# socom20/speech-cloner

Measured on AMD Instinct MI355X. Metric: mel frames/sec, higher is better.
Workload: dtype bf16; 1 GPU; full: STFT+mel front-end on batch 32 x 4 s @ 16 kHz (configs[1] input) -> 64 windows of 400 frames -> encoder (enc_14 weights) + decoder (hp/decoder_cfg_d.json sizes, random init), 64 windows per launch, independent steps pipelined over 10 HIP streams; batch=32, samples=64000, windows=64, model_dtype=bfloat16, streams=10, parallelism=utterance-sharded x1, no collective

## Files before the change

### include/vc_hip.h

```cpp
#ifndef VC_HIP_H
#define VC_HIP_H

#include <stddef.h>
#include <stdint.h>

#ifdef __cplusplus
extern "C" {
#endif

#define VC_OK 0
#define VC_ERR_INVALID 1
#define VC_ERR_HIP 2
#define VC_ERR_WORKSPACE 3
#define VC_ERR_UNSUPPORTED 4

#define VC_ABI_VERSION 7

int vc_version(void);
const char* vc_last_error(void);
const char* vc_target_arch(void);

int vc_set_option(const char* name, int value);
int vc_get_option(const char* name, int* value);
int vc_ablate_build(void);

typedef struct vc_frontend_cfg {
    int32_t sample_rate;
    int32_t hop_length;
    int32_t win_length;
    int32_t n_fft;
    int32_t n_mels;
    int32_t n_mfcc;
    float pre_emphasis;
    float mean_abs_amp_norm;
    float mfcc_norm_factor;
    float M_dB_norm_factor;
    float P_dB_norm_factor;
    int32_t mfcc_normaleze_first_mfcc;
    int32_t calc_mfcc_derivate;
    int32_t clip_output;
} vc_frontend_cfg;

typedef struct vc_frontend_plan vc_frontend_plan;

int vc_frontend_host_tables(const vc_frontend_cfg* cfg, double* h_mel, double* h_dct);

int vc_frontend_plan_create(const vc_frontend_cfg* cfg, const double* h_window,
                            vc_frontend_plan** out_plan);
void vc_frontend_plan_destroy(vc_frontend_plan* plan);

int32_t vc_frontend_num_frames(const vc_frontend_plan* plan, int32_t n_samples);
int32_t vc_frontend_mfcc_width(const vc_frontend_plan* plan);
int32_t vc_frontend_power_width(const vc_frontend_plan* plan);
int vc_frontend_get_mel(const vc_frontend_plan* plan, double* h_out);
int vc_frontend_get_dct(const vc_frontend_plan* plan, double* h_out);

size_t vc_frontend_workspace_bytes(const vc_frontend_plan* plan, int32_t batch, int32_t max_samples);

int vc_frontend_f32(const vc_frontend_plan* plan, const float* d_wav, const int32_t* d_lens,
                    int32_t batch, int32_t max_samples, int32_t wav_stride, int32_t out_rows,
                    float* d_mfcc, float* d_mel_db, float* d_pow_db,
                    void* d_workspace, size_t workspace_bytes, void* stream);

int vc_frontend_stages_f32(const vc_frontend_plan* plan, const float* d_wav, const int32_t* d_lens,
                           int32_t batch, int32_t max_samples, int32_t wav_stride, int32_t out_rows,
                           float* d_mfcc, float* d_mel_db, float* d_pow_db,
                           void* d_workspace, size_t workspace_bytes, void* stream,
                           int32_t stage_mask);

#define VC_F32 0
#define VC_BF16 1
#define VC_ACT_NONE 0
#define VC_ACT_RELU 1
#define VC_ACT_SIGMOID 2
#define VC_ACT_TANH 3
#define VC_GEMM_PLAIN 0
#define VC_GEMM_HIGHWAY 1
#define VC_GEMM_MAX_GROUPS 32

typedef struct vc_gemm_group {
    const void* d_Bt;
    int32_t K;
    int32_t taps;
    int32_t pad_l;
    int32_t c_off;
} vc_gemm_group;

typedef struct vc_gemm_desc {
    int32_t dtype;
    int32_t mode;
    const void* d_X;
    int32_t M, T, Cin, ldx;
    int32_t N;
    int32_t n_groups;
    vc_gemm_group groups[VC_GEMM_MAX_GROUPS];
    const float* d_pro_scale;
    const float* d_pro_shift;
    int32_t pro_relu, pro_pool;
    const float* d_epi_scale;
    const float* d_epi_shift;
    int32_t act;
    const void* d_R;
    int32_t ldr;
    void* d_C;
    int32_t ldc;
    int32_t out_f32;
    float drop_keep;
    unsigned long long drop_seed;
    int32_t sum_groups;
    int32_t epi_pool;
    void* d_workspace;
    size_t workspace_bytes;
} vc_gemm_desc;

int vc_conv_gemm(const vc_gemm_desc* desc, void* stream);
size_t vc_conv_gemm_workspace_bytes(const vc_gemm_desc* desc);
int vc_conv_gemm_epi_pool_supported(const vc_gemm_desc* desc);

int vc_lstm_bidir(const float* d_xproj, const void* d_Wh_fw, const void* d_Wh_bw, int32_t w_dtype, int32_t n_seq, int32_t T,
                  int32_t H, void* d_out, int32_t out_dtype, void* stream);

int vc_softmax_argmax(const float* d_logits, int32_t M, int32_t N, int32_t ldl,
                      void* d_prob, int32_t ldp, int32_t out_dtype, int32_t* d_class, void* stream);
int vc_softmax_argmax_dual(const float* d_logits, int32_t M, int32_t N, int32_t ldl, float* d_prob, int32_t ldp,
                           void* d_prob_bf16, int32_t ldp_bf16, int32_t* d_class, void* stream);

size_t vc_gru_workspace_bytes(int32_t H, int32_t w_dtype);
int vc_gru_bidir(const float* d_xproj, const void* d_Wh_fw, const void* d_Wh_bw, int32_t w_dtype,
                 int32_t n_seq, int32_t T, int32_t H, void* d_out, int32_t out_dtype,
                 void* d_workspace, size_t workspace_bytes, void* stream);


typedef struct vc_wgrad_group {
    const void* d_dYT;
    void* d_dW;
    int32_t N, taps, shift0;
    int32_t ldw;
} vc_wgrad_group;
typedef struct vc_wgrad_desc {
    const void* d_XT;
    int32_t ldxt, ldyt, Cin, M, T, margin, n_groups;
    int32_t splits_allowed;
    vc_wgrad_group groups[VC_GEMM_MAX_GROUPS];
} vc_wgrad_desc;
int vc_conv_wgrad(const vc_wgrad_desc* desc, void* stream);

int vc_transpose_pad(const float* d_X, int32_t M, int32_t C, int32_t ld, int32_t T, const float* d_scale,
                     const float* d_shift, int32_t relu, int32_t pool, int32_t row_shift, float* d_XT,
                     int32_t ldt, int32_t pad, int32_t slack_row, void* stream);

int vc_split16(const float* d_X, int32_t M, int32_t C, int32_t ldx, int32_t T, const float* d_scale, const float* d_shift,
               int32_t relu, int32_t pool, void* d_out16, float* d_row_scale, void* stream);
typedef struct vc_w16_item {
    const float* src;
    void* dst;
    float* scale_dst;
    int32_t k, cin, cout, mode;
    int32_t row_len, tap_stride, plane_stride, base;
    int32_t group, scale_n;
} vc_w16_item;
int vc_weights16(const vc_w16_item* d_items, int32_t n_items, uint32_t* d_gmax, int32_t n_groups, void* stream);
typedef struct vc_gemm16_pair {
    const void* d_Bt0;
    const void* d_Bt1;
    int32_t taps0, extra, pad_l, c_off0, c_off1;
    int32_t row0;
    int32_t nrows0, nrows1;
    int32_t s_off0, s_off1;
} vc_gemm16_pair;
typedef struct vc_gemm16_desc {
    const void* d_X16;
    const float* d_row_scale;
    int32_t M, T, C, ldx;
    int32_t n_pairs, ragged;
    vc_gemm16_pair pairs[16];
    const float* d_col_scale;
    const float* d_col_shift;
    float* d_C;
    int32_t ldc;
    int32_t accumulate;
    int32_t act;
    int32_t atomic_splits;
    void* d_workspace;
    size_t workspace_bytes;
} vc_gemm16_desc;
size_t vc_gemm16_workspace_bytes(int32_t M, int32_t C, int32_t n_pairs);
int vc_transpose_split16(const float* d_X, int32_t M, int32_t C, int32_t ldx, int32_t T, const float* d_scale,
                         const float* d_shift, int32_t relu, int32_t pool, int32_t shift0, int32_t n_shifts, void* d_out16,
                         float* d_row_scale, void* stream);
int vc_gemm16(const vc_gemm16_desc* desc, void* stream);

int vc_mx8_quantize(const void* d_X, int32_t x_dtype, int32_t M, int32_t C, int32_t ldx, void* d_Q, void* d_S, void* stream);
#define VC_MX8_MAX_GROUPS 32
#define VC_MX8_OUT_MX 0
#define VC_MX8_OUT_BF16 1
#define VC_MX8_OUT_F32 2
typedef struct vc_mx8_group {
    const void* d_W;
    const void* d_Ws;
    int32_t taps, pad_l, c_off, reserved;
} vc_mx8_group;
typedef struct vc_mx8_conv_desc {
    const void* d_X;
    const void* d_Xs;
    int32_t M, T, Cin, n_groups;
    vc_mx8_group groups[VC_MX8_MAX_GROUPS];
    const float* d_epi_scale;
    const float* d_epi_shift;
    int32_t act, pool, out_mode, n_out;
    void* d_C;
    void* d_Cs;
    void* d_workspace;
    size_t workspace_bytes;
} vc_mx8_conv_desc;
size_t vc_mx8_conv_workspace_bytes(const vc_mx8_conv_desc* desc);
int vc_mx8_conv(const vc_mx8_conv_desc* desc, void* stream);

size_t vc_stats_workspace_floats(int32_t M, int32_t C);
int vc_bn_train_stats(const float* d_X, int32_t M, int32_t C, int32_t ld, const float* d_gamma,
                      const float* d_beta, float* d_moving_mean, float* d_moving_var, float decay, float eps,
                      float* d_scale, float* d_shift, float* d_mean, float* d_rstd, float* d_workspace,
                      void* stream);
int vc_affine_act(const float* d_X, const float* d_scale, const float* d_shift, int32_t relu, const float* d_R,
                  float* d_out, size_t n, int32_t C, void* stream);
int vc_bn_backward(const float* d_G, const float* d_X, int32_t M, int32_t C, int32_t ld, int32_t T,
                   const float* d_gamma, const float* d_scale, const float* d_shift, const float* d_mean,
                   const float* d_rstd, int32_t mode, float* d_dX, float* d_dgamma, float* d_dbeta,
                   float* d_workspace, void* stream);
int vc_bn_post_routing(const float* d_X, int32_t M, int32_t C, int32_t ld, int32_t T, const float* d_scale,
                       const float* d_shift, uint8_t* d_bits, void* stream);
int vc_relu_dropout_backward(const float* d_dY, const float* d_Y, float inv_keep, float* d_dZ, size_t n, void* stream);
int vc_highway_backward(const float* d_pre, int32_t NP, const float* d_X, const float* d_dO, int32_t M, int32_t H,
                        float* d_dpre, float* d_dXd, void* stream);
int vc_col_sum(const float* d_X, int32_t M, int32_t C, int32_t ld, float* d_out, int32_t accumulate,
               float* d_workspace, void* stream);
int vc_fill(float* d_p, float value, size_t n, void* stream);
typedef struct vc_layout_item {
    const float* src;
    float* dst;
    int32_t k, cin, cout, mode;
} vc_layout_item;
int vc_weight_layouts(const vc_layout_item* d_items, int32_t n_items, void* stream);
int vc_axpby(const float* d_X, int32_t ldx, float a, const float* d_Y, int32_t ldy, float b, float* d_out, int32_t ldo,
             int32_t M, int32_t C, void* stream);
int vc_mse_loss(const float* d_y, const float* d_t, size_t n, float weight, float* d_dY, int32_t C, int32_t ld_dy,
                float* d_loss, float* d_workspace, void* stream);
int vc_lstm_train_forward(const float* d_xproj, const float* d_Wh_fw, const float* d_Wh_bw, int32_t n_seq, int32_t T,
                          int32_t H, float* d_out, float* d_gates, float* d_cstate, void* stream);
int vc_lstm_backward(const float* d_dout, const float* d_gates, const float* d_cstate, const float* d_WhT_fw,
                     const float* d_WhT_bw, int32_t n_seq, int32_t T, int32_t H, float* d_dpre, void* stream);
int vc_softmax_ce(const float* d_logits, const float* d_target, int32_t M, int32_t C, int32_t ldl, float* d_dlogits,
                  int32_t ldd, float* d_out3, float* d_workspace, void* stream);
int vc_adam_step(float* d_param, const float* d_grad, float* d_m, float* d_v, size_t n, float lr_t, float beta1,
                 float beta2, float epsilon, float grad_scale, void* stream);
int vc_gru_train_forward(const float* d_xproj, const float* d_Wh_fw, const float* d_Wh_bw, int32_t n_seq,
                         int32_t T, int32_t H, float* d_out, float* d_gates, float* d_rh, void* stream);
int vc_gru_backward(const float* d_dout, const float* d_out, const float* d_gates, const float* d_Wh_fw,
                    const float* d_Wh_bw, const float* d_WhT_fw, const float* d_WhT_bw, int32_t n_seq,
                    int32_t T, int32_t H, float* d_dpre, void* stream);

typedef struct vc_vocoder_plan vc_vocoder_plan;

int vc_vocoder_plan_create(int32_t win_length, int32_t hop_length, int32_t n_fft, const double* h_window,
                           vc_vocoder_plan** out_plan);
void vc_vocoder_plan_destroy(vc_vocoder_plan* plan);
int32_t vc_vocoder_num_samples(const vc_vocoder_plan* plan, int32_t n_frames);
size_t vc_vocoder_workspace_bytes(const vc_vocoder_plan* plan, int32_t batch, int32_t max_frames, int32_t trace);

int vc_power_to_amp(const float* d_P, const int32_t* d_n_frames, int32_t batch, int32_t max_frames, int32_t n_bins,
                    float P_dB_norm_factor, float realse, float* d_amp, void* stream);

int vc_griffin_lim_f32(const vc_vocoder_plan* plan, const float* d_amp, const float* d_phase0,
                       const int32_t* d_n_frames, int32_t batch, int32_t max_frames, int32_t num_iters,
                       float* d_wav, int32_t wav_stride, float* d_trace, void* d_workspace, size_t workspace_bytes,
                       void* stream);

size_t vc_vocoder_workspace_bytes_momentum(const vc_vocoder_plan* plan, int32_t batch, int32_t max_frames,
                                           int32_t trace);
int vc_griffin_lim_momentum_f32(const vc_vocoder_plan* plan, const float* d_amp, const float* d_phase0,
                                const int32_t* d_n_frames, int32_t batch, int32_t max_frames, int32_t num_iters,
                                float momentum, float* d_wav, int32_t wav_stride, float* d_trace, void* d_workspace,
                                size_t workspace_bytes, void* stream);

int vc_inv_preemphasis_normalize(const vc_vocoder_plan* plan, float* d_wav, const int32_t* d_n_frames, int32_t batch,
                                 int32_t max_frames, int32_t wav_stride, float coeff, float mean_abs_amp_norm,
                                 void* stream);

int vc_highway_pack(const void* d_Bt, int32_t n_cols, int32_t H, void* d_packed, void* stream);
int vc_highway_chain(const void* d_X, int32_t M, int32_t H, int32_t ldx, int32_t n_layers,
                     const void* const* d_packed, const float* const* d_bias, void* d_Y, int32_t ldy,
                     const void* d_proj_packed, const float* d_proj_bias, int32_t n_proj, float* d_P, int32_t ldp,
                     void* stream);

#define VC_CBHG_FRONT_MAX_HIGHWAY 4
typedef struct vc_cbhg_front_desc {
    const void* d_x;
    int32_t x_f32, ldx;
    int32_t n_windows, T;
    int32_t n_features, prenet_units, width, n_banks, bank_filters, n_highway, gru_units;
    const void *d_pk_dense1, *d_pk_dense2, *d_pk_bank, *d_pk_proj1, *d_pk_proj2, *d_pk_gru;
    const void* d_pk_highway[VC_CBHG_FRONT_MAX_HIGHWAY];
    const float* d_coef;
    float* d_xproj;
    int32_t ldp;
} vc_cbhg_front_desc;
int vc_mfma_pack(const void* d_W, int32_t rows, int32_t K, int32_t ldw, int32_t chained, void* d_packed, void* stream);
int32_t vc_cbhg_front_coef_floats(void);
int vc_cbhg_front_supported(int32_t n_features, int32_t prenet_units, int32_t width, int32_t n_banks,
                            int32_t bank_filters, int32_t n_highway, int32_t gru_units, int32_t T);
int vc_cbhg_front(const vc_cbhg_front_desc* desc, void* stream);

int vc_prenet_chain_supported(int32_t cin_padded, int32_t units1, int32_t units2);
int vc_prenet_chain(const void* d_X, int32_t x_f32, int32_t M, int32_t ldx, int32_t cin_padded, int32_t units1, int32_t units2,
                    const void* d_pk1, const float* d_b1, const void* d_pk2, const float* d_b2, void* d_Y, int32_t ldy,
                    void* stream);

int vc_gather_rows(const void* d_src, const int64_t* d_index, const void* d_pad_row, int64_t n_rows,
                   int32_t row_bytes, void* d_dst, void* stream);

int vc_convert(const void* d_src, int32_t src_dtype, void* d_dst, int32_t dst_dtype, size_t n, void* stream);

int vc_cut_windows(const float* d_src, const int32_t* d_win_tab, const int32_t* d_n_frames, int32_t batch,
                   int32_t max_frames, int32_t n_windows, int32_t T, int32_t C, float* d_dst, void* stream);

int vc_compound_stitch(const void* d_src, int32_t src_dtype, const int32_t* d_utt_tab, int32_t batch, int32_t n_windows,
                       int32_t T, int32_t C, int32_t out_frames, float* d_dst, float* d_amp, float P_dB_norm_factor,
                       void* stream);

int vc_phase_init(const int32_t* d_n_frames, const int32_t* d_utt_id, int32_t batch, int32_t max_frames, int32_t n_bins,
                  int64_t seed, float* d_phase, void* stream);

typedef struct vc_resample_plan vc_resample_plan;
int vc_resample_plan_create(int32_t up, int32_t down, int32_t half, const double* h_taps, vc_resample_plan** out_plan);
void vc_resample_plan_destroy(vc_resample_plan* plan);
int vc_resample_f32(const vc_resample_plan* plan, const float* d_in, const int32_t* d_lens_in, int32_t batch, int32_t max_in,
                    int32_t ld_in, float* d_out, int32_t max_out, int32_t ld_out, void* stream);

int vc_mel_cepstra(const void* d_mel, int32_t mel_dtype, int32_t rows, int32_t n_mels, const float* d_dct, int32_t n_coef,
                   float* d_cep, void* stream);
size_t vc_dtw_workspace_size(int32_t batch, int32_t max_a, int32_t max_b, int32_t want_path);
int vc_dtw_f32(const float* d_ca, const float* d_cb, const int32_t* d_len_a, const int32_t* d_len_b, int32_t batch,
               int32_t max_a, int32_t max_b, int32_t n_coef, float scale, int32_t band, int32_t want_path, float* d_total,
               int32_t* d_path_len, float* d_mcd, void* d_workspace, size_t workspace_bytes, void* stream);
int vc_dtw_backtrack(const void* d_workspace, size_t workspace_bytes, const int32_t* d_len_a, const int32_t* d_len_b,
                     const float* d_total, const int32_t* d_path_len, int32_t batch, int32_t max_a, int32_t max_b, int32_t* d_path,
                     void* stream);
int vc_frame_mcd_f32(const float* d_ca, const float* d_cb, const int32_t* d_len_a, const int32_t* d_len_b, int32_t batch,
                     int32_t max_a, int32_t max_b, int32_t n_coef, float scale, float* d_mcd, void* stream);

int vc_f0_yin_f32(const float* d_wav, const int32_t* d_lens, int32_t batch, int32_t max_len, int32_t ld, float sample_rate,
                  int32_t hop, int32_t frame_length, int32_t tau_min, int32_t tau_max, float threshold, float* d_f0,
                  float* d_aperiodicity, int32_t max_frames, void* stream);
int vc_f0_metrics_f32(const float* d_f0_a, const float* d_f0_b, const int32_t* d_len_a, const int32_t* d_len_b, int32_t batch,
                      int32_t max_a, int32_t max_b, const int32_t* d_path, const int32_t* d_path_len, int32_t max_path,
                      int32_t* d_counts, float* d_values, void* stream);

int vc_frame_energy_tile(int32_t hop, int32_t frame_length);
int vc_frame_energy_f32(const float* d_wav, const int32_t* d_lens, int32_t batch, int32_t max_len, int32_t ld, int32_t hop,
                        int32_t frame_length, float* d_energy, int32_t max_frames, void* stream);
int vc_activity_mask(const float* d_energy, const float* d_f0, const int32_t* d_n_frames, int32_t batch, int32_t max_frames,
                     int32_t mode, float ratio, int32_t max_gap, int32_t min_run, uint8_t* d_mask, void* stream);
int vc_mask_compact(const uint8_t* d_mask_a, const int32_t* d_frames_a, int32_t max_a, const uint8_t* d_mask_b,
                    const int32_t* d_frames_b, int32_t max_b, int32_t batch, int32_t* d_index, int32_t* d_n_active, int32_t* d_n_kept,
                    int32_t* d_intervals, int32_t* d_n_intervals, void* stream);
int vc_compact_rows_f32(const float* d_src, int32_t src_frames, const int32_t* d_index, int32_t index_frames, const int32_t* d_n_kept,
                        int32_t batch, int32_t n_cols, float* d_dst, int32_t dst_frames, void* stream);
int vc_path_map(const int32_t* d_path_in, const int32_t* d_path_len, int32_t batch, int32_t max_path, const int32_t* d_index_a,
                int32_t max_a, const int32_t* d_index_b, int32_t max_b, int32_t* d_path_out, void* stream);
int vc_speech_gain_f32(const float* d_wav, const int32_t* d_lens, int32_t batch, int32_t max_len, int32_t ld, int32_t hop,
                       const uint8_t* d_mask, const int32_t* d_n_active, int32_t max_frames, float target, float* d_gain,
                       void* stream);
int vc_scale_rows_f32(const float* d_wav, const int32_t* d_lens, int32_t batch, int32_t max_len, int32_t ld, const float* d_gain,
                      float* d_out, void* stream);

#ifdef __cplusplus
}
#endif
#endif
```

### speech-cloner_amd/_vc.py

```python
import contextlib
import ctypes as C
import os
import threading


_HERE = os.path.dirname(os.path.abspath(__file__))
LIB_PATH = os.environ.get('VC_LIB_PATH', os.path.join(_HERE, 'libvc_hip.so'))

VC_OK = 0
VC_ABI_VERSION = 7


class VCError(RuntimeError):
    pass


class FrontendCfg(C.Structure):
    _fields_ = [('sample_rate', C.c_int32), ('hop_length', C.c_int32), ('win_length', C.c_int32),
                ('n_fft', C.c_int32), ('n_mels', C.c_int32), ('n_mfcc', C.c_int32),
                ('pre_emphasis', C.c_float), ('mean_abs_amp_norm', C.c_float),
                ('mfcc_norm_factor', C.c_float), ('M_dB_norm_factor', C.c_float),
                ('P_dB_norm_factor', C.c_float),
                ('mfcc_normaleze_first_mfcc', C.c_int32), ('calc_mfcc_derivate', C.c_int32),
                ('clip_output', C.c_int32)]


VC_F32, VC_BF16 = 0, 1
ACT_NONE, ACT_RELU, ACT_SIGMOID, ACT_TANH = 0, 1, 2, 3
GEMM_PLAIN, GEMM_HIGHWAY = 0, 1
GEMM_MAX_GROUPS = 32


class GemmGroup(C.Structure):
    _fields_ = [('d_Bt', C.c_void_p), ('K', C.c_int32), ('taps', C.c_int32), ('pad_l', C.c_int32),
                ('c_off', C.c_int32)]


class GemmDesc(C.Structure):
    _fields_ = [('dtype', C.c_int32), ('mode', C.c_int32), ('d_X', C.c_void_p),
                ('M', C.c_int32), ('T', C.c_int32), ('Cin', C.c_int32), ('ldx', C.c_int32),
                ('N', C.c_int32), ('n_groups', C.c_int32),
                ('groups', GemmGroup * GEMM_MAX_GROUPS),
                ('d_pro_scale', C.c_void_p), ('d_pro_shift', C.c_void_p),
                ('pro_relu', C.c_int32), ('pro_pool', C.c_int32),
                ('d_epi_scale', C.c_void_p), ('d_epi_shift', C.c_void_p), ('act', C.c_int32),
                ('d_R', C.c_void_p), ('ldr', C.c_int32), ('d_C', C.c_void_p), ('ldc', C.c_int32),
                ('out_f32', C.c_int32), ('drop_keep', C.c_float), ('drop_seed', C.c_ulonglong),
                ('sum_groups', C.c_int32), ('epi_pool', C.c_int32),
                ('d_workspace', C.c_void_p), ('workspace_bytes', C.c_size_t)]


CBHG_FRONT_MAX_HIGHWAY = 4


class CbhgFrontDesc(C.Structure):
    _fields_ = [('d_x', C.c_void_p), ('x_f32', C.c_int32), ('ldx', C.c_int32), ('n_windows', C.c_int32), ('T', C.c_int32),
                ('n_features', C.c_int32), ('prenet_units', C.c_int32), ('width', C.c_int32), ('n_banks', C.c_int32),
                ('bank_filters', C.c_int32), ('n_highway', C.c_int32), ('gru_units', C.c_int32),
                ('d_pk_dense1', C.c_void_p), ('d_pk_dense2', C.c_void_p), ('d_pk_bank', C.c_void_p),
                ('d_pk_proj1', C.c_void_p), ('d_pk_proj2', C.c_void_p), ('d_pk_gru', C.c_void_p),
                ('d_pk_highway', C.c_void_p * CBHG_FRONT_MAX_HIGHWAY),
                ('d_coef', C.c_void_p),
                ('d_xproj', C.c_void_p), ('ldp', C.c_int32)]


class LayoutItem(C.Structure):
    _fields_ = [('src', C.c_void_p), ('dst', C.c_void_p), ('k', C.c_int32), ('cin', C.c_int32), ('cout', C.c_int32),
                ('mode', C.c_int32)]


class W16Item(C.Structure):
    _fields_ = [('src', C.c_void_p), ('dst', C.c_void_p), ('scale_dst', C.c_void_p), ('k', C.c_int32), ('cin', C.c_int32),
                ('cout', C.c_int32), ('mode', C.c_int32), ('row_len', C.c_int32), ('tap_stride', C.c_int32),
                ('plane_stride', C.c_int32), ('base', C.c_int32), ('group', C.c_int32), ('scale_n', C.c_int32)]


class Gemm16Pair(C.Structure):
    _fields_ = [('d_Bt0', C.c_void_p), ('d_Bt1', C.c_void_p), ('taps0', C.c_int32), ('extra', C.c_int32),
                ('pad_l', C.c_int32), ('c_off0', C.c_int32), ('c_off1', C.c_int32), ('row0', C.c_int32),
                ('nrows0', C.c_int32), ('nrows1', C.c_int32), ('s_off0', C.c_int32), ('s_off1', C.c_int32)]


class Gemm16Desc(C.Structure):
    _fields_ = [('d_X16', C.c_void_p), ('d_row_scale', C.c_void_p), ('M', C.c_int32), ('T', C.c_int32), ('C', C.c_int32),
                ('ldx', C.c_int32), ('n_pairs', C.c_int32), ('ragged', C.c_int32), ('pairs', Gemm16Pair * 16),
                ('d_col_scale', C.c_void_p), ('d_col_shift', C.c_void_p), ('d_C', C.c_void_p), ('ldc', C.c_int32),
                ('accumulate', C.c_int32), ('act', C.c_int32), ('atomic_splits', C.c_int32), ('d_workspace', C.c_void_p),
                ('workspace_bytes', C.c_size_t)]


MX8_MAX_GROUPS = 32
MX8_OUT_MX, MX8_OUT_BF16, MX8_OUT_F32 = 0, 1, 2


class Mx8Group(C.Structure):
    _fields_ = [('d_W', C.c_void_p), ('d_Ws', C.c_void_p), ('taps', C.c_int32), ('pad_l', C.c_int32),
                ('c_off', C.c_int32), ('reserved', C.c_int32)]


class Mx8ConvDesc(C.Structure):
    _fields_ = [('d_X', C.c_void_p), ('d_Xs', C.c_void_p), ('M', C.c_int32), ('T', C.c_int32), ('Cin', C.c_int32),
                ('n_groups', C.c_int32), ('groups', Mx8Group * MX8_MAX_GROUPS), ('d_epi_scale', C.c_void_p),
                ('d_epi_shift', C.c_void_p), ('act', C.c_int32), ('pool', C.c_int32), ('out_mode', C.c_int32),
                ('n_out', C.c_int32), ('d_C', C.c_void_p), ('d_Cs', C.c_void_p), ('d_workspace', C.c_void_p),
                ('workspace_bytes', C.c_size_t)]


class WgradGroup(C.Structure):
    _fields_ = [('d_dYT', C.c_void_p), ('d_dW', C.c_void_p), ('N', C.c_int32), ('taps', C.c_int32),
                ('shift0', C.c_int32), ('ldw', C.c_int32)]


class WgradDesc(C.Structure):
    _fields_ = [('d_XT', C.c_void_p), ('ldxt', C.c_int32), ('ldyt', C.c_int32), ('Cin', C.c_int32),
                ('M', C.c_int32), ('T', C.c_int32), ('margin', C.c_int32), ('n_groups', C.c_int32),
                ('splits_allowed', C.c_int32), ('groups', WgradGroup * GEMM_MAX_GROUPS)]


_lib = None
_lock = threading.Lock()

_P = C.c_void_p
_SIGS = {
    'vc_version': (C.c_int, []),
    'vc_last_error': (C.c_char_p, []),
    'vc_target_arch': (C.c_char_p, []),
    'vc_set_option': (C.c_int, [C.c_char_p, C.c_int]),
    'vc_get_option': (C.c_int, [C.c_char_p, C.POINTER(C.c_int)]),
    'vc_ablate_build': (C.c_int, []),
    'vc_frontend_host_tables': (C.c_int, [C.POINTER(FrontendCfg), _P, _P]),
    'vc_frontend_plan_create': (C.c_int, [C.POINTER(FrontendCfg), _P, C.POINTER(_P)]),
    'vc_frontend_plan_destroy': (None, [_P]),
    'vc_frontend_num_frames': (C.c_int32, [_P, C.c_int32]),
    'vc_frontend_mfcc_width': (C.c_int32, [_P]),
    'vc_frontend_power_width': (C.c_int32, [_P]),
    'vc_frontend_get_mel': (C.c_int, [_P, _P]),
    'vc_frontend_get_dct': (C.c_int, [_P, _P]),
    'vc_frontend_workspace_bytes': (C.c_size_t, [_P, C.c_int32, C.c_int32]),
    'vc_frontend_f32': (C.c_int, [_P, _P, _P, C.c_int32, C.c_int32, C.c_int32, C.c_int32, _P, _P, _P, _P,
                                  C.c_size_t, _P]),
    'vc_frontend_stages_f32': (C.c_int, [_P, _P, _P, C.c_int32, C.c_int32, C.c_int32, C.c_int32, _P, _P, _P, _P,
                                         C.c_size_t, _P, C.c_int32]),
    'vc_conv_gemm_workspace_bytes': (C.c_size_t, [C.POINTER(GemmDesc)]),
    'vc_conv_gemm': (C.c_int, [C.POINTER(GemmDesc), _P]),
    'vc_softmax_argmax': (C.c_int, [_P, C.c_int32, C.c_int32, C.c_int32, _P, C.c_int32, C.c_int32, _P, _P]),
    'vc_softmax_argmax_dual': (C.c_int, [_P, C.c_int32, C.c_int32, C.c_int32, _P, C.c_int32, _P, C.c_int32, _P, _P]),
    'vc_gru_workspace_bytes': (C.c_size_t, [C.c_int32, C.c_int32]),
    'vc_gru_bidir': (C.c_int, [_P, _P, _P, C.c_int32, C.c_int32, C.c_int32, C.c_int32, _P, C.c_int32, _P,
                               C.c_size_t, _P]),
    'vc_lstm_bidir': (C.c_int, [_P, _P, _P, C.c_int32, C.c_int32, C.c_int32, C.c_int32, _P, C.c_int32, _P]),
    'vc_convert': (C.c_int, [_P, C.c_int32, _P, C.c_int32, C.c_size_t, _P]),
    'vc_conv_wgrad': (C.c_int, [C.POINTER(WgradDesc), _P]),
    'vc_transpose_pad': (C.c_int, [_P, C.c_int32, C.c_int32, C.c_int32, C.c_int32, _P, _P, C.c_int32, C.c_int32,
                                   C.c_int32, _P, C.c_int32, C.c_int32, C.c_int32, _P]),
    'vc_stats_workspace_floats': (C.c_size_t, [C.c_int32, C.c_int32]),
    'vc_bn_train_stats': (C.c_int, [_P, C.c_int32, C.c_int32, C.c_int32, _P, _P, _P, _P, C.c_float, C.c_float,
                                    _P, _P, _P, _P, _P, _P]),
    'vc_affine_act': (C.c_int, [_P, _P, _P, C.c_int32, _P, _P, C.c_size_t, C.c_int32, _P]),
    'vc_bn_backward': (C.c_int, [_P, _P, C.c_int32, C.c_int32, C.c_int32, C.c_int32, _P, _P, _P, _P, _P,
                                 C.c_int32, _P, _P, _P, _P, _P]),
    'vc_lstm_train_forward': (C.c_int, [_P, _P, _P, C.c_int32, C.c_int32, C.c_int32, _P, _P, _P, _P]),
    'vc_lstm_backward': (C.c_int, [_P, _P, _P, _P, _P, C.c_int32, C.c_int32, C.c_int32, _P, _P]),
    'vc_bn_post_routing': (C.c_int, [_P, C.c_int32, C.c_int32, C.c_int32, C.c_int32, _P, _P, _P, _P]),
    'vc_relu_dropout_backward': (C.c_int, [_P, _P, C.c_float, _P, C.c_size_t, _P]),
    'vc_highway_backward': (C.c_int, [_P, C.c_int32, _P, _P, C.c_int32, C.c_int32, _P, _P, _P]),
    'vc_col_sum': (C.c_int, [_P, C.c_int32, C.c_int32, C.c_int32, _P, C.c_int32, _P, _P]),
    'vc_fill': (C.c_int, [_P, C.c_float, C.c_size_t, _P]),
    'vc_weight_layouts': (C.c_int, [_P, C.c_int32, _P]),
    'vc_split16': (C.c_int, [_P, C.c_int32, C.c_int32, C.c_int32, C.c_int32, _P, _P, C.c_int32, C.c_int32, _P, _P, _P]),
    'vc_weights16': (C.c_int, [_P, C.c_int32, _P, C.c_int32, _P]),
    'vc_transpose_split16': (C.c_int, [_P, C.c_int32, C.c_int32, C.c_int32, C.c_int32, _P, _P, C.c_int32, C.c_int32, C.c_int32,
                                       C.c_int32, _P, _P, _P]),
    'vc_gemm16_workspace_bytes': (C.c_size_t, [C.c_int32, C.c_int32, C.c_int32]),
    'vc_gemm16': (C.c_int, [C.POINTER(Gemm16Desc), _P]),
    'vc_mx8_quantize': (C.c_int, [_P, C.c_int32, C.c_int32, C.c_int32, C.c_int32, _P, _P, _P]),
    'vc_mx8_conv_workspace_bytes': (C.c_size_t, [C.POINTER(Mx8ConvDesc)]),
    'vc_mx8_conv': (C.c_int, [C.POINTER(Mx8ConvDesc), _P]),
    'vc_axpby': (C.c_int, [_P, C.c_int32, C.c_float, _P, C.c_int32, C.c_float, _P, C.c_int32, C.c_int32, C.c_int32, _P]),
    'vc_mse_loss': (C.c_int, [_P, _P, C.c_size_t, C.c_float, _P, C.c_int32, C.c_int32, _P, _P, _P]),
    'vc_softmax_ce': (C.c_int, [_P, _P, C.c_int32, C.c_int32, C.c_int32, _P, C.c_int32, _P, _P, _P]),
    'vc_adam_step': (C.c_int, [_P, _P, _P, _P, C.c_size_t, C.c_float, C.c_float, C.c_float, C.c_float,
                               C.c_float, _P]),
    'vc_gru_train_forward': (C.c_int, [_P, _P, _P, C.c_int32, C.c_int32, C.c_int32, _P, _P, _P, _P]),
    'vc_gru_backward': (C.c_int, [_P, _P, _P, _P, _P, _P, _P, C.c_int32, C.c_int32, C.c_int32, _P, _P]),
    'vc_conv_gemm_epi_pool_supported': (C.c_int, [C.POINTER(GemmDesc)]),
    'vc_highway_pack': (C.c_int, [_P, C.c_int32, C.c_int32, _P, _P]),
    'vc_highway_chain': (C.c_int, [_P, C.c_int32, C.c_int32, C.c_int32, C.c_int32, C.POINTER(_P), C.POINTER(_P), _P, C.c_int32,
                                   _P, _P, C.c_int32, _P, C.c_int32, _P]),
    'vc_mfma_pack': (C.c_int, [_P, C.c_int32, C.c_int32, C.c_int32, C.c_int32, _P, _P]),
    'vc_prenet_chain_supported': (C.c_int, [C.c_int32] * 3),
    'vc_prenet_chain': (C.c_int, [_P, C.c_int32, C.c_int32, C.c_int32, C.c_int32, C.c_int32, C.c_int32, _P, _P, _P, _P, _P, C.c_int32, _P]),
    'vc_cbhg_front_coef_floats': (C.c_int32, []),
    'vc_cbhg_front_supported': (C.c_int, [C.c_int32] * 8),
    'vc_cbhg_front': (C.c_int, [C.POINTER(CbhgFrontDesc), _P]),
    'vc_gather_rows': (C.c_int, [_P, _P, _P, C.c_int64, C.c_int32, _P, _P]),
    'vc_vocoder_plan_create': (C.c_int, [C.c_int32, C.c_int32, C.c_int32, _P, C.POINTER(_P)]),
    'vc_vocoder_plan_destroy': (None, [_P]),
    'vc_vocoder_num_samples': (C.c_int32, [_P, C.c_int32]),
    'vc_vocoder_workspace_bytes': (C.c_size_t, [_P, C.c_int32, C.c_int32, C.c_int32]),
    'vc_power_to_amp': (C.c_int, [_P, _P, C.c_int32, C.c_int32, C.c_int32, C.c_float, C.c_float, _P, _P]),
    'vc_griffin_lim_f32': (C.c_int, [_P, _P, _P, _P, C.c_int32, C.c_int32, C.c_int32, _P, C.c_int32, _P, _P,
                                     C.c_size_t, _P]),
    'vc_vocoder_workspace_bytes_momentum': (C.c_size_t, [_P, C.c_int32, C.c_int32, C.c_int32]),
    'vc_griffin_lim_momentum_f32': (C.c_int, [_P, _P, _P, _P, C.c_int32, C.c_int32, C.c_int32, C.c_float, _P, C.c_int32,
                                              _P, _P, C.c_size_t, _P]),
    'vc_inv_preemphasis_normalize': (C.c_int, [_P, _P, _P, C.c_int32, C.c_int32, C.c_int32, C.c_float, C.c_float, _P]),
    'vc_cut_windows': (C.c_int, [_P, _P, _P, C.c_int32, C.c_int32, C.c_int32, C.c_int32, C.c_int32, _P, _P]),
    'vc_compound_stitch': (C.c_int, [_P, C.c_int32, _P, C.c_int32, C.c_int32, C.c_int32, C.c_int32, C.c_int32, _P, _P,
                                     C.c_float, _P]),
    'vc_phase_init': (C.c_int, [_P, _P, C.c_int32, C.c_int32, C.c_int32, C.c_int64, _P, _P]),
    'vc_resample_plan_create': (C.c_int, [C.c_int32, C.c_int32, C.c_int32, _P, C.POINTER(_P)]),
    'vc_resample_plan_destroy': (None, [_P]),
    'vc_resample_f32': (C.c_int, [_P, _P, _P, C.c_int32, C.c_int32, C.c_int32, _P, C.c_int32, C.c_int32, _P]),
    'vc_mel_cepstra': (C.c_int, [_P, C.c_int32, C.c_int32, C.c_int32, _P, C.c_int32, _P, _P]),
    'vc_dtw_workspace_size': (C.c_size_t, [C.c_int32] * 4),
    'vc_dtw_f32': (C.c_int, [_P, _P, _P, _P, C.c_int32, C.c_int32, C.c_int32, C.c_int32, C.c_float, C.c_int32, C.c_int32, _P, _P, _P,
                             _P, C.c_size_t, _P]),
    'vc_dtw_backtrack': (C.c_int, [_P, C.c_size_t, _P, _P, _P, _P, C.c_int32, C.c_int32, C.c_int32, _P, _P]),
    'vc_frame_mcd_f32': (C.c_int, [_P, _P, _P, _P, C.c_int32, C.c_int32, C.c_int32, C.c_int32, C.c_float, _P, _P]),
    'vc_frame_energy_tile': (C.c_int, [C.c_int32, C.c_int32]),
    'vc_frame_energy_f32': (C.c_int, [_P, _P, C.c_int32, C.c_int32, C.c_int32, C.c_int32, C.c_int32, _P, C.c_int32, _P]),
    'vc_activity_mask': (C.c_int, [_P, _P, _P, C.c_int32, C.c_int32, C.c_int32, C.c_float, C.c_int32, C.c_int32, _P, _P]),
    'vc_mask_compact': (C.c_int, [_P, _P, C.c_int32, _P, _P, C.c_int32, C.c_int32, _P, _P, _P, _P, _P, _P]),
    'vc_compact_rows_f32': (C.c_int, [_P, C.c_int32, _P, C.c_int32, _P, C.c_int32, C.c_int32, _P, C.c_int32, _P]),
    'vc_path_map': (C.c_int, [_P, _P, C.c_int32, C.c_int32, _P, C.c_int32, _P, C.c_int32, _P, _P]),
    'vc_speech_gain_f32': (C.c_int, [_P, _P, C.c_int32, C.c_int32, C.c_int32, C.c_int32, _P, _P, C.c_int32, C.c_float, _P, _P]),
    'vc_scale_rows_f32': (C.c_int, [_P, _P, C.c_int32, C.c_int32, C.c_int32, _P, _P, _P]),
    'vc_f0_yin_f32': (C.c_int, [_P, _P, C.c_int32, C.c_int32, C.c_int32, C.c_float, C.c_int32, C.c_int32, C.c_int32, C.c_int32,
                                C.c_float, _P, _P, C.c_int32, _P]),
    'vc_f0_metrics_f32': (C.c_int, [_P, _P, _P, _P, C.c_int32, C.c_int32, C.c_int32, _P, _P, C.c_int32, _P, _P, _P]),
}


def lib():
    global _lib
    if _lib is not None:
        return _lib
    with _lock:
        if _lib is not None:
            return _lib
        if not os.path.exists(LIB_PATH):
            raise VCError('native library %s not found -- run `python -c "import __graft_entry__ as g; '
                          'g.build()"` (or make -C speech-cloner_amd/csrc); there is no CPU fallback'
                          % LIB_PATH)
        import torch
        h = C.CDLL(LIB_PATH)
        h.vc_version.restype, h.vc_version.argtypes = C.c_int, []
        got = h.vc_version()
        if got != VC_ABI_VERSION:
            raise VCError('native library %s reports ABI version %d, this binding is written for %d -- rebuild it '
                          '(make -C speech-cloner_amd/csrc)' % (LIB_PATH, got, VC_ABI_VERSION))
        for name, (res, args) in _SIGS.items():
            try:
                fn = getattr(h, name)
            except AttributeError:
                raise VCError('native library %s does not export %s -- it was built from older sources, rebuild it '
                              '(make -C speech-cloner_amd/csrc)' % (LIB_PATH, name)) from None
            fn.restype = res
            fn.argtypes = args
        _lib = h
    return _lib


def set_option(name, value):
    check(lib().vc_set_option(name.encode(), int(value)))


def get_option(name):
    v = C.c_int(0)
    check(lib().vc_get_option(name.encode(), C.byref(v)))
    return v.value


@contextlib.contextmanager
def options(**kw):
    old = {k: get_option(k) for k in kw}
    try:
        for k, v in kw.items():
            set_option(k, v)
        yield
    finally:
        for k, v in old.items():
            set_option(k, v)


THROUGHPUT_OPTIONS = {'proj256_split': 0, 'fe_fused': 0}


def throughput_mode():
    return options(**THROUGHPUT_OPTIONS)


def check(rc):
    if rc != VC_OK:
        msg = lib().vc_last_error()
        raise VCError('libvc_hip error %d: %s' % (rc, msg.decode('utf-8', 'replace') if msg else '?'))


def ptr(t):
    if t is None:
        return None
    if hasattr(t, 'data_ptr'):
        return C.c_void_p(t.data_ptr())
    return C.c_void_p(t.ctypes.data)


def current_stream():
    import torch
    return C.c_void_p(torch.cuda.current_stream().cuda_stream)
```

### speech-cloner_amd/csrc/vc_api.hip

```cpp
#include <cstdarg>
#include <atomic>
#include <cstdio>
#include <cstring>
#include "vc_common.h"

namespace vc {

static thread_local char g_err[512] = "";

char* last_error_buf() { return g_err; }

int set_error(int code, const char* fmt, ...) {
    va_list ap;
    va_start(ap, fmt);
    vsnprintf(g_err, sizeof(g_err), fmt, ap);
    va_end(ap);
    return code;
}

static std::atomic<int> g_opt[OPT_COUNT];
static const struct { const char* name; Option id; bool ablate; } k_opts[] = {
    {"bank256", OPT_BANK256, false}, {"bank256_xcd", OPT_BANK256_XCD, false}, {"conv256", OPT_CONV256, false},
    {"conv256_min_k", OPT_CONV256_MINK, false}, {"conv256_wm", OPT_CONV256_WM, false}, {"proj256", OPT_PROJ256, false}, {"proj256_split", OPT_PROJ256_SPLIT, false},
    {"wgrad_xcd", OPT_WGRAD_XCD, false}, {"gru_mfma", OPT_GRU_MFMA, false}, {"gru_mfma4", OPT_GRU_MFMA4, false}, {"gru_small_mfma", OPT_GRU_SMALL_MFMA, false}, {"fe_fused", OPT_FE_FUSED, false}, {"fe_fused_spin", OPT_FE_FUSED_SPIN, false}, {"gru_train_resident", OPT_GRU_TRAIN_RESIDENT, false}, {"prenet_lds", OPT_PRENET_LDS, false}, {"cbhg_front_mi", OPT_CBHG_FRONT_MI, false}, {"gemm16_split", OPT_GEMM16_SPLIT, false}, {"f32_f16x3", OPT_F32_F16X3, false}, {"gru_f32_wide", OPT_GRU_F32_WIDE, false},
    {"ablate_bank256", OPT_ABLATE_BANK256, true}, {"ablate_bank256_only", OPT_ABLATE_BANK256_ONLY, true},
    {"ablate_cbhg_front", OPT_ABLATE_CBHG_FRONT, true},
};
static struct OptInit { OptInit() { for (auto& o : g_opt) o.store(-1); } } g_opt_init;

int opt(Option o) { return g_opt[o].load(std::memory_order_relaxed); }

static __global__ void zero_words_kernel(unsigned* __restrict__ p, size_t n) {
    for (size_t i = (size_t)blockIdx.x * blockDim.x + threadIdx.x; i < n; i += (size_t)gridDim.x * blockDim.x) p[i] = 0u;
}

hipError_t zero_async(void* d_p, size_t bytes, hipStream_t st) {
    if (bytes % 4) return hipErrorInvalidValue;
    const size_t n = bytes / 4;
    if (n == 0) return hipSuccess;
    const size_t blocks = (n + 255) / 256;
    hipLaunchKernelGGL(zero_words_kernel, dim3((unsigned)(blocks < 1024 ? blocks : 1024)), dim3(256), 0, st,
                       static_cast<unsigned*>(d_p), n);
    return hipGetLastError();
}

}

extern "C" {

int vc_set_option(const char* name, int value) {
    VC_REQUIRE(name, "vc_set_option: NULL name");
    for (const auto& o : vc::k_opts)
        if (!std::strcmp(o.name, name)) {
#ifndef VC_ABLATE
            VC_REQUIRE(!o.ablate, "vc_set_option: %s exists only in -DVC_ABLATE builds (tools/build_ablate.sh)", name);
#endif
            vc::g_opt[o.id].store(value);
            return VC_OK;
        }
    return vc::set_error(VC_ERR_INVALID, "vc_set_option: unknown option %s", name);
}

int vc_get_option(const char* name, int* value) {
    VC_REQUIRE(name && value, "vc_get_option: NULL argument");
    for (const auto& o : vc::k_opts)
        if (!std::strcmp(o.name, name)) { *value = vc::g_opt[o.id].load(); return VC_OK; }
    return vc::set_error(VC_ERR_INVALID, "vc_get_option: unknown option %s", name);
}

int vc_ablate_build(void) {
#ifdef VC_ABLATE
    return 1;
#else
    return 0;
#endif
}

int vc_version(void) { return VC_ABI_VERSION; }
const char* vc_last_error(void) { return vc::last_error_buf(); }
const char* vc_target_arch(void) { return "gfx950"; }

}
```

### speech-cloner_amd/csrc/vc_common.h

```cpp
#pragma once
#include <hip/hip_runtime.h>
#include <cstdarg>
#include <cstdio>
#include "vc_hip.h"

namespace vc {

char* last_error_buf();
int set_error(int code, const char* fmt, ...);

#define VC_HIP_CHECK(expr)                                                                   \
    do {                                                                                     \
        hipError_t _e = (expr);                                                              \
        if (_e != hipSuccess)                                                                \
            return vc::set_error(VC_ERR_HIP, "%s failed: %s (%s:%d)", #expr,                 \
                                 hipGetErrorString(_e), __FILE__, __LINE__);                 \
    } while (0)

#define VC_REQUIRE(cond, ...)                                                                \
    do {                                                                                     \
        if (!(cond)) return vc::set_error(VC_ERR_INVALID, __VA_ARGS__);                      \
    } while (0)

constexpr int WAVE = 64;

enum Option {
    OPT_BANK256 = 0,
    OPT_BANK256_XCD,
    OPT_CONV256,
    OPT_CONV256_MINK,
    OPT_CONV256_WM,
    OPT_PROJ256,
    OPT_PROJ256_SPLIT,
    OPT_WGRAD_XCD,
    OPT_GRU_MFMA,
    OPT_FE_FUSED,
    OPT_FE_FUSED_SPIN,
    OPT_GRU_SMALL_MFMA,
    OPT_GRU_MFMA4,
    OPT_PRENET_LDS,
    OPT_GRU_TRAIN_RESIDENT,
    OPT_CBHG_FRONT_MI,
    OPT_GRU_F32_WIDE,
    OPT_F32_F16X3,
    OPT_GEMM16_SPLIT,
    OPT_ABLATE_BANK256,
    OPT_ABLATE_BANK256_ONLY,
    OPT_ABLATE_CBHG_FRONT,
    OPT_COUNT
};
int opt(Option o);

hipError_t zero_async(void* d_p, size_t bytes, hipStream_t st);

#if defined(__HIPCC__)
template <int CTRL, int ROW_MASK>
__device__ __forceinline__ float dpp_move(float identity, float v) {
    return __int_as_float(__builtin_amdgcn_update_dpp(__float_as_int(identity), __float_as_int(v), CTRL, ROW_MASK, 0xF, false));
}
#define VC_WAVE_REDUCE(OP, ID)                                                                  \
    v = OP(v, dpp_move<0xB1, 0xF>(ID, v));                             \
    v = OP(v, dpp_move<0x4E, 0xF>(ID, v));                             \
    v = OP(v, dpp_move<0x141, 0xF>(ID, v));                                \
    v = OP(v, dpp_move<0x140, 0xF>(ID, v));          \
    v = OP(v, dpp_move<0x142, 0xA>(ID, v));                 \
    v = OP(v, dpp_move<0x143, 0xC>(ID, v));                 \
    return __int_as_float(__builtin_amdgcn_readlane(__float_as_int(v), 63));
__device__ __forceinline__ float vc_addf(float a, float b) { return a + b; }
__device__ __forceinline__ float wave_sum(float v) { VC_WAVE_REDUCE(vc_addf, 0.0f) }
__device__ __forceinline__ float wave_max(float v) { VC_WAVE_REDUCE(fmaxf, -3.402823466e38f) }
__device__ __forceinline__ float highway_gate(float hpre, float tpre, float x) {
    const float hv = fmaxf(hpre, 0.0f);
    const float e = __builtin_amdgcn_exp2f(tpre * -1.4426950408889634f);
    const float tv = __builtin_amdgcn_rcpf(1.0f + e);
    return fmaf(tv, hv - x, x);
}
__device__ __forceinline__ float wave_min(float v) { VC_WAVE_REDUCE(fminf, 3.402823466e38f) }
#undef VC_WAVE_REDUCE
#endif

}
```

### speech-cloner_amd/csrc/vc_conv256.h

```cpp
#pragma once
#include <hip/hip_runtime.h>
#include <cstdint>

struct Conv256Args {
    const void* X;
    int32_t M, T, Cin, ldx, N;
    const void* Bt;
    int32_t K, taps, pad_l, c_off;
    int32_t pool;
    const float* epi_scale;
    const float* epi_shift;
    int32_t act;
    const void* R;
    int32_t ldr;
    void* C;
    int32_t ldc;
};

int vc_launch_conv256(const Conv256Args& a, hipStream_t st);
```

### speech-cloner_amd/csrc/vc_conv256.hip

```cpp
#include "vc_common.h"
#include "vc_conv256.h"
#include <cstdlib>

namespace {

typedef float f32x16 __attribute__((ext_vector_type(16)));
typedef __bf16 bf16x8 __attribute__((ext_vector_type(8)));
typedef __bf16 bf16x4 __attribute__((ext_vector_type(4)));
typedef unsigned short u16x8 __attribute__((ext_vector_type(8)));

constexpr int a_rows(int wm) { return 64 * wm + 8; }

__device__ __forceinline__ void glds16(const void* g, void* l) {
    __builtin_amdgcn_global_load_lds((const __attribute__((address_space(1))) void*)(uintptr_t)g,
                                     (__attribute__((address_space(3))) void*)(uintptr_t)(uint32_t)(uintptr_t)l, 16, 0, 0);
}

__device__ __forceinline__ bf16x8 max_nonneg(bf16x8 x, bf16x8 y) {
    return __builtin_bit_cast(bf16x8, __builtin_elementwise_max(__builtin_bit_cast(u16x8, x), __builtin_bit_cast(u16x8, y)));
}

__device__ __forceinline__ float act_fn(float v, int act) {
    switch (act) {
        case VC_ACT_RELU: return fmaxf(v, 0.0f);
        case VC_ACT_SIGMOID: return 1.0f / (1.0f + __expf(-v));
        case VC_ACT_TANH: return tanhf(v);
        default: return v;
    }
}

__device__ __forceinline__ void wait_loads_but(int n) {
    if (n >= 8) asm volatile("s_waitcnt vmcnt(8) lgkmcnt(0)" ::: "memory");
    else if (n >= 6) asm volatile("s_waitcnt vmcnt(6) lgkmcnt(0)" ::: "memory");
    else if (n >= 4) asm volatile("s_waitcnt vmcnt(4) lgkmcnt(0)" ::: "memory");
    else if (n >= 2) asm volatile("s_waitcnt vmcnt(2) lgkmcnt(0)" ::: "memory");
    else asm volatile("s_waitcnt vmcnt(0) lgkmcnt(0)" ::: "memory");
}

template <int WN, bool POOL, int NBUF, int WM>
__global__ void __launch_bounds__(64 * WM * WN, 1)
conv256_kernel(Conv256Args a) {
    constexpr int BM = 64 * WM, A_ROWS = a_rows(WM), A_BYTES = A_ROWS * 128;
    constexpr int BN = 64 * WN, NWAVE = WM * WN, NTHR = 64 * NWAVE;
    constexpr int BQ = (BN / 8) / NWAVE;
    static_assert(BQ * NWAVE * 8 == BN && (BQ == 2 || BQ == 4), "weight tile split");
    constexpr int DIST = NBUF - 1;
    constexpr int B_BYTES = BN * 128;
    constexpr int AQ = (A_ROWS / 8 + NWAVE - 1) / NWAVE;
    extern __shared__ __attribute__((aligned(16))) char smem[];
    char* const As = smem;
    char* const Bs = smem + 2 * A_BYTES;

    const int tid = threadIdx.x, lane = tid & 63;
    const int wid = __builtin_amdgcn_readfirstlane(tid >> 6);
    const int wr = wid / WN, wc = wid % WN;
    const int m0 = blockIdx.x * BM, n0 = blockIdx.y * BN;
    const int ntap = a.taps, nslab = a.Cin >> 6, ntiles = nslab * ntap, pad_l = a.pad_l;
    const __bf16* X = reinterpret_cast<const __bf16*>(a.X);
    const __bf16* Bt = reinterpret_cast<const __bf16*>(a.Bt);

    const int srow = lane >> 3, pslot = lane & 7;
    const __bf16* a_src[AQ];
#pragma unroll
    for (int q = 0; q < AQ; ++q) {
        const int rho = (q * NWAVE + wid) * 8 + srow;
        const int g = min(max(m0 - pad_l + rho, 0), a.M - 1);
        a_src[q] = X + (size_t)g * a.ldx + (pslot ^ ((rho >> 1) & 7)) * 8;
    }
    const int a_rows_needed = BM + ntap - 1 + (POOL ? 1 : 0);
    const __bf16* b_src[BQ];
#pragma unroll
    for (int q = 0; q < BQ; ++q) {
        const int n = (q * NWAVE + wid) * 8 + srow;
        b_src[q] = Bt + (size_t)min(n0 + n, a.N - 1) * a.K + (pslot ^ ((n >> 1) & 7)) * 8;
    }
    auto stageA = [&](int cs, int buf) {
        char* dst = As + buf * A_BYTES + wid * 1024;
#pragma unroll
        for (int q = 0; q < AQ; ++q) {
            const int rb = q * NWAVE + wid;
            if (rb * 8 < a_rows_needed && rb < A_ROWS / 8) glds16(a_src[q] + cs * 64, dst + q * NWAVE * 1024);
        }
    };
    auto stageB = [&](int n, int buf) {
        const int cs = n / ntap, j = n - cs * ntap;
        const int koff = j * a.Cin + cs * 64;
        char* dst = Bs + buf * B_BYTES + wid * 1024;
#pragma unroll
        for (int q = 0; q < BQ; ++q) glds16(b_src[q] + koff, dst + q * NWAVE * 1024);
    };

    const int li = lane & 31, lh = lane >> 5;
    const int a_row0 = wr * 64 + li;
    const int xb = (li >> 1) & 7;
    int b_off[4];
#pragma unroll
    for (int s = 0; s < 4; ++s) b_off[s] = (wc * 64 + li) * 128 + (((2 * s + lh) ^ xb) << 4);
    int jlo[2], jhi[2];
#pragma unroll
    for (int i = 0; i < 2; ++i) {
        const int m = min(m0 + wr * 64 + i * 32 + li, a.M - 1);
        const int t = m % a.T;
        jlo[i] = max(0, pad_l - t);
        jhi[i] = a.T - t + pad_l;
    }
    int J_lo = max(jlo[0], jlo[1]);
    int J_hi = min(jhi[0], jhi[1]) - (POOL ? 1 : 0);
#pragma unroll
    for (int o = 32; o > 0; o >>= 1) {
        J_lo = max(J_lo, __shfl_xor(J_lo, o, 64));
        J_hi = min(J_hi, __shfl_xor(J_hi, o, 64));
    }
    J_lo = __builtin_amdgcn_readfirstlane(J_lo);
    J_hi = __builtin_amdgcn_readfirstlane(J_hi);

    f32x16 acc[2][2];
#pragma unroll
    for (int i = 0; i < 2; ++i)
#pragma unroll
        for (int c = 0; c < 2; ++c)
#pragma unroll
            for (int r = 0; r < 16; ++r) acc[i][c][r] = 0.0f;

    bf16x8 fa[2][2], fp[2][2], fb[2][2];
    int a_base = 0, a_o[4], p_base = 0, p_o[4];
    int j = 0;
    auto tap_setup = [&](int n) {
        const int cs = n / ntap, jj = n - cs * ntap;
        const int rho = a_row0 + jj;
        a_base = (cs & 1) * A_BYTES + rho * 128;
        p_base = a_base + 128;
        const int x = (rho >> 1) & 7, xp = ((rho + 1) >> 1) & 7;
#pragma unroll
        for (int s = 0; s < 4; ++s) {
            a_o[s] = ((2 * s + lh) ^ x) << 4;
            p_o[s] = ((2 * s + lh) ^ xp) << 4;
        }
        return jj;
    };

    const int keep = ntap == 1 ? DIST - 2 : DIST - 1;
    const int tail0 = ntap == 1 ? ntiles - DIST : ntiles - 2;
    static_assert(DIST == 2 || DIST == 3, "the taps >= DIST - 1 argument above assumes 3 or 4 weight buffers");
    stageA(0, 0);
    stageB(0, 0);
#pragma unroll
    for (int d = 1; d < DIST; ++d)
        if (d < ntiles) stageB(d, d);
    wait_loads_but(BQ * min(DIST - 1, ntiles - 1));
    __builtin_amdgcn_s_barrier();
    asm volatile("" ::: "memory");
    if (nslab > 1) stageA(1, 1);
    if (DIST < ntiles) stageB(DIST, DIST);
    int bcur = 0;
    j = tap_setup(0);
    {
        const char* ap = As + a_base + a_o[0];
        fa[0][0] = *reinterpret_cast<const bf16x8*>(ap);
        fa[0][1] = *reinterpret_cast<const bf16x8*>(ap + 4096);
        if constexpr (POOL) {
            const char* pp = As + p_base + p_o[0];
            fp[0][0] = *reinterpret_cast<const bf16x8*>(pp);
            fp[0][1] = *reinterpret_cast<const bf16x8*>(pp + 4096);
        }
        const char* bp = Bs + b_off[0];
        fb[0][0] = *reinterpret_cast<const bf16x8*>(bp);
        fb[0][1] = *reinterpret_cast<const bf16x8*>(bp + 4096);
    }

    for (int n = 0; n < ntiles; ++n) {
        const bool need_mask = !(j >= J_lo && j < J_hi);
        bool v[2], hn[2];
#pragma unroll
        for (int i = 0; i < 2; ++i) {
            v[i] = j >= jlo[i] && j < jhi[i];
            hn[i] = j < jhi[i] - 1;
        }
        const bf16x8 zero = {};
        int jn = j;
#pragma unroll
        for (int s = 0; s < 4; ++s) {
            const int cur = s & 1, nxt = cur ^ 1;
            bool have_next = true;
            int nb = bcur;
            if (s == 3) {
                wait_loads_but(BQ * max(0, min(keep, tail0 - n)));
                __builtin_amdgcn_s_barrier();
                asm volatile("" ::: "memory");
                have_next = n + 1 < ntiles;
                if (have_next) {
                    const int cs1 = (n + 1) / ntap;
                    if ((n + 1) - cs1 * ntap == 0 && cs1 + 1 < nslab) stageA(cs1 + 1, (cs1 + 1) & 1);
                    jn = tap_setup(n + 1);
                }
                if (n + 1 + DIST < ntiles) stageB(n + 1 + DIST, bcur);
                nb = bcur + 1 == NBUF ? 0 : bcur + 1;
            }
            const int sn = (s + 1) & 3;
            const char* ap = As + a_base + a_o[sn];
            const char* pp = As + p_base + p_o[sn];
            const char* bp = Bs + nb * B_BYTES + b_off[sn];
            bf16x8 av[2];
#pragma unroll
            for (int i = 0; i < 2; ++i) {
                if constexpr (POOL) av[i] = max_nonneg(fa[cur][i], fp[cur][i]);
                else av[i] = fa[cur][i];
            }
            if (need_mask) {
#pragma unroll
                for (int i = 0; i < 2; ++i) {
                    if constexpr (POOL) av[i] = hn[i] ? av[i] : fa[cur][i];
                    av[i] = v[i] ? av[i] : zero;
                }
            }
            __builtin_amdgcn_s_setprio(1);
            acc[0][0] = __builtin_amdgcn_mfma_f32_32x32x16_bf16(fb[cur][0], av[0], acc[0][0], 0, 0, 0);
            acc[0][1] = __builtin_amdgcn_mfma_f32_32x32x16_bf16(fb[cur][1], av[0], acc[0][1], 0, 0, 0);
            if (have_next) {
                fa[nxt][0] = *reinterpret_cast<const bf16x8*>(ap);
                fa[nxt][1] = *reinterpret_cast<const bf16x8*>(ap + 4096);
                if constexpr (POOL) {
                    fp[nxt][0] = *reinterpret_cast<const bf16x8*>(pp);
                    fp[nxt][1] = *reinterpret_cast<const bf16x8*>(pp + 4096);
                }
                fb[nxt][0] = *reinterpret_cast<const bf16x8*>(bp);
                fb[nxt][1] = *reinterpret_cast<const bf16x8*>(bp + 4096);
            }
            acc[1][0] = __builtin_amdgcn_mfma_f32_32x32x16_bf16(fb[cur][0], av[1], acc[1][0], 0, 0, 0);
            acc[1][1] = __builtin_amdgcn_mfma_f32_32x32x16_bf16(fb[cur][1], av[1], acc[1][1], 0, 0, 0);
            __builtin_amdgcn_s_setprio(0);
        }
        j = jn;
        bcur = bcur + 1 == NBUF ? 0 : bcur + 1;
    }

    constexpr int EP = BN * 2 + 16;
    __syncthreads();
    {
#pragma unroll
        for (int c = 0; c < 2; ++c) {
#pragma unroll
            for (int q = 0; q < 4; ++q) {
                const int col = wc * 64 + c * 32 + 8 * q + 4 * lh;
                const int gn = min(n0 + col, a.N - 4);
                float4 sv = make_float4(1.0f, 1.0f, 1.0f, 1.0f), bv = make_float4(0.0f, 0.0f, 0.0f, 0.0f);
                if (a.epi_scale) sv = *reinterpret_cast<const float4*>(a.epi_scale + a.c_off + gn);
                if (a.epi_shift) bv = *reinterpret_cast<const float4*>(a.epi_shift + a.c_off + gn);
                const float svv[4] = {sv.x, sv.y, sv.z, sv.w}, bvv[4] = {bv.x, bv.y, bv.z, bv.w};
#pragma unroll
                for (int i = 0; i < 2; ++i) {
                    const int row = wr * 64 + i * 32 + li;
                    bf16x4 rr = {};
                    if (a.R) {
                        const int gm = min(m0 + row, a.M - 1);
                        rr = *reinterpret_cast<const bf16x4*>(reinterpret_cast<const __bf16*>(a.R) + (size_t)gm * a.ldr + gn);
                    }
                    bf16x4 o;
#pragma unroll
                    for (int e = 0; e < 4; ++e) {
                        float val = act_fn(acc[i][c][4 * q + e] * svv[e] + bvv[e], a.act);
                        if (a.R) val += (float)rr[e];
                        o[e] = (__bf16)val;
                    }
                    *reinterpret_cast<bf16x4*>(smem + row * EP + col * 2) = o;
                }
            }
        }
    }
    __syncthreads();
    {
        constexpr int CPR = BN / 8;
        __bf16* C = reinterpret_cast<__bf16*>(a.C);
        for (int idx = tid; idx < BM * CPR; idx += NTHR) {
            const int row = idx / CPR, ch = idx - row * CPR;
            const int gm = m0 + row, gn = n0 + ch * 8;
            if (gm < a.M && gn < a.N)
                *reinterpret_cast<bf16x8*>(C + (size_t)gm * a.ldc + a.c_off + gn) =
                    *reinterpret_cast<const bf16x8*>(smem + row * EP + ch * 16);
        }
    }
}

template <int WN, bool POOL, int WM> int launch(const Conv256Args& a, hipStream_t st) {
    constexpr int NBUF = WN == 4 ? 3 : 4;
    constexpr int BM = 64 * WM;
    constexpr int LDS = 2 * a_rows(WM) * 128 + NBUF * 64 * WN * 128;
    static_assert(LDS <= 160 * 1024 && BM * (64 * WN * 2 + 16) <= LDS, "LDS budget (K loop, epilogue tile)");
    static bool attr_done = false;
    if (!attr_done) {
        VC_HIP_CHECK(hipFuncSetAttribute(reinterpret_cast<const void*>(conv256_kernel<WN, POOL, NBUF, WM>),
                                         hipFuncAttributeMaxDynamicSharedMemorySize, LDS));
        attr_done = true;
    }
    hipLaunchKernelGGL((conv256_kernel<WN, POOL, NBUF, WM>), dim3((a.M + BM - 1) / BM, a.N / (64 * WN)), dim3(64 * WM * WN), LDS, st, a);
    VC_HIP_CHECK(hipGetLastError());
    return VC_OK;
}

}

int vc_launch_conv256(const Conv256Args& a, hipStream_t st) {
    const bool wide = (a.N % 256) == 0;
    const bool tall = !wide && a.M >= 2048 && vc::opt(vc::OPT_CONV256_WM) != 2;
    if (a.pool) return wide ? launch<4, true, 2>(a, st) : (tall ? launch<2, true, 4>(a, st) : launch<2, true, 2>(a, st));
    return wide ? launch<4, false, 2>(a, st) : (tall ? launch<2, false, 4>(a, st) : launch<2, false, 2>(a, st));
}
```

### speech-cloner_amd/csrc/vc_rnn.hip

```cpp
#include <hip/hip_runtime.h>
#include <cstdlib>

#include "vc_common.h"

namespace {

typedef __bf16 bf16x2 __attribute__((ext_vector_type(2)));

__device__ __forceinline__ float ld_w(const float* p) { return *p; }
__device__ __forceinline__ float ld_w(const __bf16* p) { return (float)*p; }
__device__ __forceinline__ float sigmoidf_(float v) { return 1.0f / (1.0f + __expf(-v)); }
__device__ __forceinline__ float fast_sigmoid(float v) { return __builtin_amdgcn_rcpf(1.0f + __expf(-v)); }
__device__ __forceinline__ float fast_tanh(float v) { return 1.0f - 2.0f * __builtin_amdgcn_rcpf(__expf(2.0f * v) + 1.0f); }

struct GruArgs {
    const float* xproj;
    const void* Wh[2];
    void* out;
    int32_t n_seq, T, H, out_bf16, w_in_lds;
};

template <typename T> __device__ __forceinline__ void st_out(void* o, size_t i, float v, int bf) {
    if (bf) reinterpret_cast<__bf16*>(o)[i] = (__bf16)v;
    else reinterpret_cast<float*>(o)[i] = v;
}

template <typename WT>
__global__ void __launch_bounds__(512)
gru_generic_kernel(GruArgs a) {
    extern __shared__ __attribute__((aligned(16))) char smem[];
    const int H = a.H, H3 = 3 * H, NT = blockDim.x, tid = threadIdx.x;
    float* h = reinterpret_cast<float*>(smem);
    float* rh = h + H;
    float* u = rh + H;
    WT* wl = reinterpret_cast<WT*>(u + H);
    const int seq = blockIdx.x, dir = blockIdx.y;
    const WT* Wg = reinterpret_cast<const WT*>(a.Wh[dir]);
    if (a.w_in_lds) {
        for (int i = tid; i < H * H3; i += NT) wl[i] = Wg[i];
        Wg = wl;
    }
    for (int i = tid; i < H; i += NT) h[i] = 0.0f;

    int KS1 = 1, KS2 = 1;
    while (KS1 * 2 <= 64 && KS1 * 2 * 2 * H <= NT) KS1 *= 2;
    while (KS2 * 2 <= 64 && KS2 * 2 * H <= NT) KS2 *= 2;
    const int col1 = tid / KS1, ks1 = tid % KS1;
    const int col2 = tid / KS2, ks2 = tid % KS2;
    const bool act1 = col1 < 2 * H, act2 = col2 < H;
    const size_t xrow = 6 * (size_t)H;
    const float* xbase = a.xproj + (size_t)seq * a.T * xrow + (size_t)dir * H3;
    __syncthreads();

    int t = dir ? a.T - 1 : 0;
    const int dt = dir ? -1 : 1;
    float xg = (act1 && ks1 == 0) ? xbase[(size_t)t * xrow + col1] : 0.0f;
    float xc = (act2 && ks2 == 0) ? xbase[(size_t)t * xrow + 2 * H + col2] : 0.0f;
    for (int step = 0; step < a.T; ++step, t += dt) {
        float xg_n = 0.0f, xc_n = 0.0f;
        if (step + 1 < a.T) {
            if (act1 && ks1 == 0) xg_n = xbase[(size_t)(t + dt) * xrow + col1];
            if (act2 && ks2 == 0) xc_n = xbase[(size_t)(t + dt) * xrow + 2 * H + col2];
        }
        float acc = 0.0f;
        if (act1) {
            const WT* w = Wg + col1;
            for (int k = ks1; k < H; k += KS1) acc = fmaf(h[k], ld_w(w + (size_t)k * H3), acc);
        }
        for (int o = KS1 >> 1; o > 0; o >>= 1) acc += __shfl_xor(acc, o, 64);
        if (act1 && ks1 == 0) {
            const float g = sigmoidf_(acc + xg);
            if (col1 < H) rh[col1] = g * h[col1];
            else u[col1 - H] = g;
        }
        __syncthreads();
        float acc2 = 0.0f;
        if (act2) {
            const WT* w = Wg + 2 * H + col2;
            for (int k = ks2; k < H; k += KS2) acc2 = fmaf(rh[k], ld_w(w + (size_t)k * H3), acc2);
        }
        for (int o = KS2 >> 1; o > 0; o >>= 1) acc2 += __shfl_xor(acc2, o, 64);
        float hn = 0.0f;
        if (act2 && ks2 == 0) {
            const float c = tanhf(acc2 + xc);
            const float uu = u[col2];
            hn = uu * h[col2] + (1.0f - uu) * c;
        }
        __syncthreads();
        if (act2 && ks2 == 0) {
            h[col2] = hn;
            st_out<WT>(a.out, ((size_t)seq * a.T + t) * 2 * H + (size_t)dir * H + col2, hn, a.out_bf16);
        }
        __syncthreads();
        xg = xg_n;
        xc = xc_n;
    }
}


struct LstmArgs {
    const float* xproj;
    const void* Wh[2];
    int32_t n_seq, T, H;
    void* out;
    int32_t out_bf16, w_in_lds;
};

template <typename WT>
__global__ void __launch_bounds__(512)
lstm_generic_kernel(LstmArgs a) {
    extern __shared__ __attribute__((aligned(16))) char smem[];
    const int H = a.H, H4 = 4 * H, NT = blockDim.x, tid = threadIdx.x;
    float* h = reinterpret_cast<float*>(smem);
    float* z = h + H;
    WT* wl = reinterpret_cast<WT*>(z + H4);
    const int seq = blockIdx.x, dir = blockIdx.y;
    const WT* W = reinterpret_cast<const WT*>(a.Wh[dir]);
    if (a.w_in_lds) {
        for (int i = tid; i < H * H4; i += NT) wl[i] = W[i];
        W = wl;
    }
    for (int i = tid; i < H; i += NT) h[i] = 0.0f;
    float c = 0.0f;
    const size_t xrow = 8 * (size_t)H;
    const float* xbase = a.xproj + (size_t)seq * a.T * xrow + (size_t)dir * H4;
    __syncthreads();
    int t = dir ? a.T - 1 : 0;
    const int dt = dir ? -1 : 1;
    for (int step = 0; step < a.T; ++step, t += dt) {
        const float* xr = xbase + (size_t)t * xrow;
        for (int col = tid; col < H4; col += NT) {
            float acc = xr[col];
            const WT* w = W + col;
#pragma unroll 4
            for (int k = 0; k < H; ++k) acc = fmaf(h[k], ld_w(w + (size_t)k * H4), acc);
            z[col] = acc;
        }
        __syncthreads();
        if (tid < H) {
            const float gi = sigmoidf_(z[tid]), gj = tanhf(z[H + tid]);
            const float gf = sigmoidf_(z[2 * H + tid] + 1.0f), go = sigmoidf_(z[3 * H + tid]);
            c = gf * c + gi * gj;
            const float hn = go * tanhf(c);
            h[tid] = hn;
            st_out<WT>(a.out, ((size_t)seq * a.T + t) * 2 * H + (size_t)dir * H + tid, hn, a.out_bf16);
        }
        __syncthreads();
    }
}

typedef __bf16 bf16x8v __attribute__((ext_vector_type(8)));
typedef float f32x4v __attribute__((ext_vector_type(4)));

template <typename WT> struct Res;
template <> struct Res<__bf16> {
    static constexpr int EPC = 8;
    typedef __bf16 hstore_t;
    typedef bf16x8v chunk_t;
    static __device__ __forceinline__ void dot(const chunk_t& w, const __bf16* hs, float& a0, float& a1) {
        const bf16x8v hv = *reinterpret_cast<const bf16x8v*>(hs);
        const bf16x2 w0 = {w[0], w[1]}, w1 = {w[2], w[3]}, w2 = {w[4], w[5]}, w3 = {w[6], w[7]};
        const bf16x2 h0 = {hv[0], hv[1]}, h1 = {hv[2], hv[3]}, h2 = {hv[4], hv[5]}, h3 = {hv[6], hv[7]};
        a0 = __builtin_amdgcn_fdot2_f32_bf16(w0, h0, a0, false);
        a1 = __builtin_amdgcn_fdot2_f32_bf16(w1, h1, a1, false);
        a0 = __builtin_amdgcn_fdot2_f32_bf16(w2, h2, a0, false);
        a1 = __builtin_amdgcn_fdot2_f32_bf16(w3, h3, a1, false);
    }
};
template <> struct Res<float> {
    static constexpr int EPC = 4;
    typedef float hstore_t;
    typedef f32x4v chunk_t;
    static __device__ __forceinline__ void dot(const chunk_t& w, const float* hs, float& a0, float& a1) {
        const f32x4v hv = *reinterpret_cast<const f32x4v*>(hs);
        a0 = fmaf(w[0], hv[0], a0);
        a1 = fmaf(w[1], hv[1], a1);
        a0 = fmaf(w[2], hv[2], a0);
        a1 = fmaf(w[3], hv[3], a1);
    }
};

template <int H, int NT> struct ResGeom {
    static constexpr int KS1 = NT / (2 * H), KL1 = H / KS1, KS2 = NT / H, KL2 = H / KS2;
};

template <int H, typename WT, int NT>
__global__ void __launch_bounds__(256)
gru_pack_kernel(const WT* W0, const WT* W1, WT* packed) {
    typedef ResGeom<H, NT> G;
    constexpr int EPC = Res<WT>::EPC, PER = G::KL1 + G::KL2, H3 = 3 * H;
    const int total = 2 * NT * PER;
    for (int idx = blockIdx.x * 256 + threadIdx.x; idx < total; idx += gridDim.x * 256) {
        const int dir = idx / (NT * PER);
        int r = idx - dir * NT * PER;
        const int c = r / (NT * EPC);
        r -= c * NT * EPC;
        const int tid = r / EPC, e = r - tid * EPC;
        const int j = c * EPC + e;
        const WT* W = dir ? W1 : W0;
        WT v;
        if (j < G::KL1) {
            const int col1 = tid / G::KS1, ks1 = tid % G::KS1;
            v = W[(size_t)(ks1 * G::KL1 + j) * H3 + col1];
        } else {
            const int col2 = tid / G::KS2, ks2 = tid % G::KS2;
            v = W[(size_t)(ks2 * G::KL2 + (j - G::KL1)) * H3 + 2 * H + col2];
        }
        packed[idx] = v;
    }
}

template <int H, typename WT, int NT>
__global__ void __launch_bounds__(NT, NT / 256)
gru_resident_kernel(GruArgs a, const WT* packed) {
    typedef Res<WT> R;
    typedef ResGeom<H, NT> G;
    typedef typename R::hstore_t hs_t;
    typedef typename R::chunk_t chunk_t;
    constexpr int H3 = 3 * H, EPC = R::EPC;
    constexpr int KS1 = G::KS1, KL1 = G::KL1, KS2 = G::KS2, KL2 = G::KL2;
    constexpr int NC1 = KL1 / EPC, NC2 = KL2 / EPC;
    constexpr int P = EPC;
    static_assert(KS1 >= 1 && KS2 <= 64 && KL1 % EPC == 0 && KL2 % EPC == 0, "unsupported H");
    static_assert(2 * H <= NT, "one thread per gate column at least");
    __shared__ __attribute__((aligned(16))) hs_t hb[KS1 * (KL1 + P)];
    __shared__ __attribute__((aligned(16))) hs_t rhb[KS2 * (KL2 + P)];
    __shared__ float hf[H];
    __shared__ float ul[H];

    const int tid = threadIdx.x;
    const int seq = blockIdx.x, dir = blockIdx.y;
    const int col1 = tid / KS1, ks1 = tid % KS1;
    const int col2 = tid / KS2, ks2 = tid % KS2;
    chunk_t w1[NC1], w2[NC2];
    {
        const chunk_t* pk = reinterpret_cast<const chunk_t*>(packed) + (size_t)dir * NT * (NC1 + NC2) + tid;
#pragma unroll
        for (int c = 0; c < NC1; ++c) w1[c] = pk[(size_t)c * NT];
#pragma unroll
        for (int c = 0; c < NC2; ++c) w2[c] = pk[(size_t)(NC1 + c) * NT];
    }
    for (int i = tid; i < KS1 * (KL1 + P); i += NT) hb[i] = (hs_t)0.0f;
    for (int i = tid; i < KS2 * (KL2 + P); i += NT) rhb[i] = (hs_t)0.0f;
    if (tid < H) hf[tid] = 0.0f;
    const size_t xrow = 6 * (size_t)H;
    const float* xbase = a.xproj + (size_t)seq * a.T * xrow + (size_t)dir * H3;
    int t = dir ? a.T - 1 : 0;
    const int dt = dir ? -1 : 1;
    float xg = (ks1 == 0) ? xbase[(size_t)t * xrow + col1] : 0.0f;
    float xc = (ks2 == 0) ? xbase[(size_t)t * xrow + 2 * H + col2] : 0.0f;
    float hreg = 0.0f;
    const hs_t* hs1 = hb + ks1 * (KL1 + P);
    const hs_t* hs2 = rhb + ks2 * (KL2 + P);
    __syncthreads();

    for (int step = 0; step < a.T; ++step, t += dt) {
        float xg_n = 0.0f, xc_n = 0.0f;
        if (step + 1 < a.T) {
            if (ks1 == 0) xg_n = xbase[(size_t)(t + dt) * xrow + col1];
            if (ks2 == 0) xc_n = xbase[(size_t)(t + dt) * xrow + 2 * H + col2];
        }
        float a0 = 0.0f, a1 = 0.0f;
#pragma unroll
        for (int c = 0; c < NC1; ++c) R::dot(w1[c], hs1 + c * EPC, a0, a1);
        float acc = a0 + a1;
#pragma unroll
        for (int o = KS1 >> 1; o > 0; o >>= 1) acc += __shfl_xor(acc, o, 64);
        if (ks1 == 0) {
            const float g = (sizeof(WT) == 2) ? fast_sigmoid(acc + xg) : sigmoidf_(acc + xg);
            if (col1 < H) {
                const int s = col1 / KL2, off = col1 - s * KL2;
                rhb[s * (KL2 + P) + off] = (hs_t)(g * hf[col1]);
            } else {
                ul[col1 - H] = g;
            }
        }
        __syncthreads();
        float b0 = 0.0f, b1 = 0.0f;
#pragma unroll
        for (int c = 0; c < NC2; ++c) R::dot(w2[c], hs2 + c * EPC, b0, b1);
        float acc2 = b0 + b1;
#pragma unroll
        for (int o = KS2 >> 1; o > 0; o >>= 1) acc2 += __shfl_xor(acc2, o, 64);
        if (ks2 == 0) {
            const float c = (sizeof(WT) == 2) ? fast_tanh(acc2 + xc) : tanhf(acc2 + xc);
            const float uu = ul[col2];
            const float hn = uu * hreg + (1.0f - uu) * c;
            hreg = hn;
            const int s = col2 / KL1, off = col2 - s * KL1;
            hb[s * (KL1 + P) + off] = (hs_t)hn;
            hf[col2] = hn;
            st_out<WT>(a.out, ((size_t)seq * a.T + t) * 2 * H + (size_t)dir * H + col2, hn, a.out_bf16);
        }
        __syncthreads();
        xg = xg_n;
        xc = xc_n;
    }
}

template <int H, typename WT, int NT>
int launch_resident(const GruArgs& a, void* ws, size_t ws_bytes, hipStream_t st) {
    const size_t need = 2 * (size_t)3 * H * H * sizeof(WT);
    if (ws == nullptr || ws_bytes < need)
        return vc::set_error(VC_ERR_WORKSPACE, "vc_gru_bidir: workspace too small (%zu < %zu)", ws_bytes, need);
    WT* packed = static_cast<WT*>(ws);
    hipLaunchKernelGGL((gru_pack_kernel<H, WT, NT>), dim3(256), dim3(256), 0, st,
                       static_cast<const WT*>(a.Wh[0]), static_cast<const WT*>(a.Wh[1]), packed);
    hipLaunchKernelGGL((gru_resident_kernel<H, WT, NT>), dim3(a.n_seq, 2), dim3(NT), 0, st, a,
                       static_cast<const WT*>(packed));
    VC_HIP_CHECK(hipGetLastError());
    return VC_OK;
}


typedef float f32x4m __attribute__((ext_vector_type(4)));

template <int H> struct MfGeom {
    static constexpr int NW = 8, UW = H / NW, TPW = UW / 16, KSN = H / 32;
    static constexpr int NF_G = 2 * TPW * KSN, NF_C = TPW * KSN, NF = NF_G + NF_C;
    static constexpr int PITCH = H + 8;
    static constexpr bool CAND_LDS = (H >= 256);
};

template <int H>
__global__ void __launch_bounds__(256)
gru_mfma_pack_kernel(const __bf16* W0, const __bf16* W1, __bf16* packed) {
    typedef MfGeom<H> G;
    const int total = 2 * G::NW * G::NF * 64 * 8;
    for (int idx = blockIdx.x * 256 + threadIdx.x; idx < total; idx += gridDim.x * 256) {
        int r = idx;
        const int j = r & 7; r >>= 3;
        const int lane = r & 63; r >>= 6;
        const int f = r % G::NF; r /= G::NF;
        const int wave = r % G::NW;
        const int dir = r / G::NW;
        int g, rem;
        if (f < G::NF_G) { g = f / (G::TPW * G::KSN); rem = f % (G::TPW * G::KSN); }
        else { g = 2; rem = f - G::NF_G; }
        const int tl = rem / G::KSN, ks = rem % G::KSN;
        const int k = ks * 32 + 8 * (lane >> 4) + j;
        const int col = g * H + wave * G::UW + tl * 16 + (lane & 15);
        const __bf16* W = dir ? W1 : W0;
        packed[idx] = W[(size_t)k * 3 * H + col];
    }
}

#ifdef VC_ABLATE
__device__ unsigned long long g_gru_stamps[16];
#define GRU_T(i) do { if (stamp) { const unsigned long long t_ = __builtin_amdgcn_s_memtime(); acc_t[i] += t_ - t_prev; t_prev = t_; } } while (0)
#else
#define GRU_T(i) do { } while (0)
#endif

#define GRU_LDS_BARRIER() asm volatile("s_waitcnt lgkmcnt(0)\n\ts_barrier" ::: "memory")

template <int H>
__global__ void __launch_bounds__(512, 2)
gru_mfma_kernel(GruArgs a, const __bf16* packed) {
    typedef MfGeom<H> G;
    constexpr int TPW = G::TPW, KSN = G::KSN, PITCH = G::PITCH, UW = G::UW;
    extern __shared__ __attribute__((aligned(16))) char smem[];
    __bf16* hb = reinterpret_cast<__bf16*>(smem);
    __bf16* rhb = hb + 16 * PITCH;
    bf16x8v* candL = reinterpret_cast<bf16x8v*>(rhb + 16 * PITCH);

    const int tid = threadIdx.x, lane = tid & 63, wave = tid >> 6;
    const int dir = blockIdx.y, seq0 = blockIdx.x * 16;
    const int n = lane & 15, q = lane >> 4;
    const int seq = min(seq0 + n, a.n_seq - 1);
    const bool seq_ok = (seq0 + n) < a.n_seq;
    const bf16x8v* pk = reinterpret_cast<const bf16x8v*>(packed) + ((size_t)(dir * G::NW + wave) * G::NF) * 64 + lane;

    bf16x8v wg[G::NF_G];
#pragma unroll
    for (int f = 0; f < G::NF_G; ++f) wg[f] = pk[(size_t)f * 64];
    bf16x8v wc[G::CAND_LDS ? 1 : G::NF_C];
    if (G::CAND_LDS) {
#pragma unroll
        for (int f = 0; f < G::NF_C; ++f) candL[(wave * G::NF_C + f) * 64 + lane] = pk[(size_t)(G::NF_G + f) * 64];
    } else {
#pragma unroll
        for (int f = 0; f < G::NF_C; ++f) wc[f] = pk[(size_t)(G::NF_G + f) * 64];
    }
    for (int i = tid; i < 2 * 16 * PITCH; i += 512) hb[i] = (__bf16)0.0f;
    float hreg[TPW][4];
#pragma unroll
    for (int tl = 0; tl < TPW; ++tl)
#pragma unroll
        for (int e = 0; e < 4; ++e) hreg[tl][e] = 0.0f;

    const int H3 = 3 * H;
    const size_t xrow = 6 * (size_t)H;
    const int ucol = wave * UW + q * 4;
    const float* xbase = a.xproj + (size_t)seq * a.T * xrow + (size_t)dir * H3 + ucol;
    int t = dir ? a.T - 1 : 0;
    const int dt = dir ? -1 : 1;
    f32x4m xr[TPW], xu[TPW], xc[TPW];
#pragma unroll
    for (int tl = 0; tl < TPW; ++tl) {
        const float* xp = xbase + (size_t)t * xrow + tl * 16;
        xr[tl] = *reinterpret_cast<const f32x4m*>(xp);
        xu[tl] = *reinterpret_cast<const f32x4m*>(xp + H);
        xc[tl] = *reinterpret_cast<const f32x4m*>(xp + 2 * H);
    }
    __syncthreads();

    const __bf16* hrow = hb + n * PITCH + 8 * q;
    const __bf16* rrow = rhb + n * PITCH + 8 * q;
#ifdef VC_ABLATE
    const bool stamp = blockIdx.x == 0 && blockIdx.y == 0 && tid == 0;
    unsigned long long acc_t[8] = {0, 0, 0, 0, 0, 0, 0, 0}, t_prev = __builtin_amdgcn_s_memtime();
#endif
    for (int step = 0; step < a.T; ++step, t += dt) {
        const bool more = step + 1 < a.T;
        const float* xn = xbase + (size_t)(more ? t + dt : t) * xrow;
        bf16x8v bfr[KSN];
#pragma unroll
        for (int ks = 0; ks < KSN; ++ks) bfr[ks] = *reinterpret_cast<const bf16x8v*>(hrow + ks * 32);
        f32x4m ar[TPW], au[TPW];
#pragma unroll
        for (int tl = 0; tl < TPW; ++tl) {
            ar[tl] = xr[tl];
            au[tl] = xu[tl];
            xr[tl] = *reinterpret_cast<const f32x4m*>(xn + tl * 16);
            xu[tl] = *reinterpret_cast<const f32x4m*>(xn + tl * 16 + H);
        }
#pragma unroll
        for (int ks = 0; ks < KSN; ++ks) {
#pragma unroll
            for (int tl = 0; tl < TPW; ++tl) {
                ar[tl] = __builtin_amdgcn_mfma_f32_16x16x32_bf16(wg[(0 * TPW + tl) * KSN + ks], bfr[ks], ar[tl], 0, 0, 0);
                au[tl] = __builtin_amdgcn_mfma_f32_16x16x32_bf16(wg[(1 * TPW + tl) * KSN + ks], bfr[ks], au[tl], 0, 0, 0);
            }
        }
        GRU_T(0);
        float uu[TPW][4];
#pragma unroll
        for (int tl = 0; tl < TPW; ++tl) {
            typedef __bf16 bf16x4v __attribute__((ext_vector_type(4)));
            bf16x4v o;
#pragma unroll
            for (int e = 0; e < 4; ++e) {
                const float r = fast_sigmoid(ar[tl][e]);
                uu[tl][e] = fast_sigmoid(au[tl][e]);
                o[e] = (__bf16)(r * hreg[tl][e]);
            }
            *reinterpret_cast<bf16x4v*>(rhb + n * PITCH + ucol + tl * 16) = o;
        }
        GRU_T(1);
        GRU_LDS_BARRIER();
        GRU_T(2);
#pragma unroll
        for (int ks = 0; ks < KSN; ++ks) bfr[ks] = *reinterpret_cast<const bf16x8v*>(rrow + ks * 32);
        f32x4m ac[TPW];
#pragma unroll
        for (int tl = 0; tl < TPW; ++tl) {
            ac[tl] = xc[tl];
            xc[tl] = *reinterpret_cast<const f32x4m*>(xn + tl * 16 + 2 * H);
        }
#pragma unroll
        for (int ks = 0; ks < KSN; ++ks) {
#pragma unroll
            for (int tl = 0; tl < TPW; ++tl) {
                const bf16x8v w = G::CAND_LDS ? candL[(wave * G::NF_C + tl * KSN + ks) * 64 + lane] : wc[G::CAND_LDS ? 0 : tl * KSN + ks];
                ac[tl] = __builtin_amdgcn_mfma_f32_16x16x32_bf16(w, bfr[ks], ac[tl], 0, 0, 0);
            }
        }
        GRU_T(3);
#pragma unroll
        for (int tl = 0; tl < TPW; ++tl) {
            typedef __bf16 bf16x4v __attribute__((ext_vector_type(4)));
            bf16x4v o;
            f32x4m hv;
#pragma unroll
            for (int e = 0; e < 4; ++e) {
                const float c = fast_tanh(ac[tl][e]);
                const float hn = uu[tl][e] * hreg[tl][e] + (1.0f - uu[tl][e]) * c;
                hreg[tl][e] = hn;
                hv[e] = hn;
                o[e] = (__bf16)hn;
            }
            *reinterpret_cast<bf16x4v*>(hb + n * PITCH + ucol + tl * 16) = o;
            if (seq_ok) {
                const size_t oi = ((size_t)seq * a.T + t) * 2 * H + (size_t)dir * H + ucol + tl * 16;
                if (a.out_bf16) *reinterpret_cast<bf16x4v*>(reinterpret_cast<__bf16*>(a.out) + oi) = o;
                else *reinterpret_cast<f32x4m*>(reinterpret_cast<float*>(a.out) + oi) = hv;
            }
        }
        GRU_T(4);
        GRU_LDS_BARRIER();
        GRU_T(5);
    }
#ifdef VC_ABLATE
    if (stamp) {
#pragma unroll
        for (int i = 0; i < 8; ++i) g_gru_stamps[i] = acc_t[i];
    }
#endif
}

template <int H>
int launch_mfma(const GruArgs& a, void* ws, size_t ws_bytes, hipStream_t st) {
    typedef MfGeom<H> G;
    const size_t need = 2 * (size_t)3 * H * H * sizeof(__bf16);
    if (ws == nullptr || ws_bytes < need)
        return vc::set_error(VC_ERR_WORKSPACE, "vc_gru_bidir: workspace too small (%zu < %zu)", ws_bytes, need);
    __bf16* packed = static_cast<__bf16*>(ws);
    hipLaunchKernelGGL((gru_mfma_pack_kernel<H>), dim3(256), dim3(256), 0, st, static_cast<const __bf16*>(a.Wh[0]),
                       static_cast<const __bf16*>(a.Wh[1]), packed);
    const size_t lds = 2 * 16 * (size_t)G::PITCH * 2 + (G::CAND_LDS ? (size_t)G::NW * G::NF_C * 64 * 16 : 0);
    static bool attr_done = false;
    if (!attr_done) {
        VC_HIP_CHECK(hipFuncSetAttribute(reinterpret_cast<const void*>(gru_mfma_kernel<H>),
                                         hipFuncAttributeMaxDynamicSharedMemorySize, (int)lds));
        attr_done = true;
    }
    hipLaunchKernelGGL((gru_mfma_kernel<H>), dim3((a.n_seq + 15) / 16, 2), dim3(512), lds, st, a,
                       static_cast<const __bf16*>(packed));
    VC_HIP_CHECK(hipGetLastError());
    return VC_OK;
}

template <int H> struct Mf4Geom {
    static constexpr int NW = 4, UW = H / NW, TPW = UW / 16, KSN = H / 32;
    static constexpr int NF_G = 2 * TPW * KSN, NF_C = TPW * KSN, NF = NF_G + NF_C;
    static constexpr int PITCH = H + 8;
    static constexpr int KL = (H >= 256) ? 4 : 0;
    static constexpr int KR = KSN - KL;
    static constexpr size_t LDS = 2 * 16 * (size_t)PITCH * 2 + (size_t)NW * TPW * KL * 64 * 16;
};

template <int H>
__global__ void __launch_bounds__(256)
gru_mfma4_pack_kernel(const __bf16* W0, const __bf16* W1, __bf16* packed) {
    typedef Mf4Geom<H> G;
    const int total = 2 * G::NW * G::NF * 64 * 8;
    for (int idx = blockIdx.x * 256 + threadIdx.x; idx < total; idx += gridDim.x * 256) {
        int r = idx;
        const int j = r & 7; r >>= 3;
        const int lane = r & 63; r >>= 6;
        const int f = r % G::NF; r /= G::NF;
        const int wave = r % G::NW;
        const int dir = r / G::NW;
        int g, rem;
        if (f < G::NF_G) { g = f / (G::TPW * G::KSN); rem = f % (G::TPW * G::KSN); }
        else { g = 2; rem = f - G::NF_G; }
        const int tl = rem / G::KSN, ks = rem % G::KSN;
        const int k = ks * 32 + 8 * (lane >> 4) + j;
        const int col = g * H + wave * G::UW + tl * 16 + (lane & 15);
        const __bf16* W = dir ? W1 : W0;
        packed[idx] = W[(size_t)k * 3 * H + col];
    }
}

template <int H>
__global__ void __launch_bounds__(256, 1)
gru_mfma4_kernel(GruArgs a, const __bf16* packed) {
    typedef Mf4Geom<H> G;
    constexpr int TPW = G::TPW, KSN = G::KSN, PITCH = G::PITCH, UW = G::UW, KL = G::KL, KR = G::KR;
    typedef __bf16 bf16x4v __attribute__((ext_vector_type(4)));
    extern __shared__ __attribute__((aligned(16))) char smem[];
    __bf16* hb = reinterpret_cast<__bf16*>(smem);
    __bf16* rhb = hb + 16 * PITCH;
    bf16x8v* candL = reinterpret_cast<bf16x8v*>(rhb + 16 * PITCH);

    const int tid = threadIdx.x, lane = tid & 63;
    const int wave = __builtin_amdgcn_readfirstlane(tid >> 6);
    const int dir = blockIdx.y, seq0 = blockIdx.x * 16;
    const int n = lane & 15, q = lane >> 4;
    const int seq = min(seq0 + n, a.n_seq - 1);
    const bool seq_ok = (seq0 + n) < a.n_seq;
    const bf16x8v* pk = reinterpret_cast<const bf16x8v*>(packed) + ((size_t)(dir * G::NW + wave) * G::NF) * 64 + lane;

    bf16x8v wr[TPW][KSN], wu[TPW][KSN], wc[TPW][KR];
#pragma unroll
    for (int tl = 0; tl < TPW; ++tl)
#pragma unroll
        for (int ks = 0; ks < KSN; ++ks) {
            wr[tl][ks] = pk[(size_t)((0 * TPW + tl) * KSN + ks) * 64];
            wu[tl][ks] = pk[(size_t)((1 * TPW + tl) * KSN + ks) * 64];
            const bf16x8v c = pk[(size_t)(G::NF_G + tl * KSN + ks) * 64];
            if (ks < KR) wc[tl][ks < KR ? ks : 0] = c;
            else candL[((wave * TPW + tl) * KL + (ks - KR)) * 64 + lane] = c;
        }
    for (int i = tid; i < 2 * 16 * PITCH; i += 256) hb[i] = (__bf16)0.0f;
    float hreg[TPW][4];
#pragma unroll
    for (int tl = 0; tl < TPW; ++tl)
#pragma unroll
        for (int e = 0; e < 4; ++e) hreg[tl][e] = 0.0f;

    const int H3 = 3 * H;
    const size_t xrow = 6 * (size_t)H;
    const int ucol = wave * UW + q * 4;
    const float* xbase = a.xproj + (size_t)seq * a.T * xrow + (size_t)dir * H3 + ucol;
    int t = dir ? a.T - 1 : 0;
    const int dt = dir ? -1 : 1;
    f32x4m xr[TPW], xu[TPW], xc[TPW];
#pragma unroll
    for (int tl = 0; tl < TPW; ++tl) {
        const float* xp = xbase + (size_t)t * xrow + tl * 16;
        xr[tl] = *reinterpret_cast<const f32x4m*>(xp);
        xu[tl] = *reinterpret_cast<const f32x4m*>(xp + H);
        xc[tl] = *reinterpret_cast<const f32x4m*>(xp + 2 * H);
    }
    __syncthreads();

    const __bf16* hrow = hb + n * PITCH + 8 * q;
    const __bf16* rrow = rhb + n * PITCH + 8 * q;
#define GRU4_BARRIER() asm volatile("s_waitcnt lgkmcnt(0)\n\ts_barrier" ::: "memory")
#define GRU4_MFMA(acc, w, b, in_acc)                                                                                   \
    do {                                                                                                               \
        if (in_acc) asm volatile("s_nop 1\n\tv_mfma_f32_16x16x32_bf16 %0, %1, %2, %0" : "+v"(acc) : "a"(w), "v"(b));   \
        else asm volatile("s_nop 1\n\tv_mfma_f32_16x16x32_bf16 %0, %1, %2, %0" : "+v"(acc) : "v"(w), "v"(b));         \
    } while (0)
#ifdef VC_ABLATE
    const bool stamp = blockIdx.x == 0 && blockIdx.y == 0 && tid == 0;
    unsigned long long acc_t[8] = {0, 0, 0, 0, 0, 0, 0, 0}, t_prev = __builtin_amdgcn_s_memtime();
#endif
    for (int step = 0; step < a.T; ++step, t += dt) {
        const float* xn = xbase + (size_t)(step + 1 < a.T ? t + dt : t) * xrow;
        bf16x8v bfr[KSN];
#pragma unroll
        for (int ks = 0; ks < KSN; ++ks) bfr[ks] = *reinterpret_cast<const bf16x8v*>(hrow + ks * 32);
        f32x4m ar[TPW], au[TPW];
#pragma unroll
        for (int tl = 0; tl < TPW; ++tl) {
            ar[tl] = xr[tl];
            au[tl] = xu[tl];
            xr[tl] = *reinterpret_cast<const f32x4m*>(xn + tl * 16);
            xu[tl] = *reinterpret_cast<const f32x4m*>(xn + tl * 16 + H);
        }
        GRU_T(0);
#pragma unroll
        for (int ks = 0; ks < KSN; ++ks)
#pragma unroll
            for (int tl = 0; tl < TPW; ++tl) GRU4_MFMA(ar[tl], wr[tl][ks], bfr[ks], true);
        float rhf[TPW][4];
#pragma unroll
        for (int ks = 0; ks < KSN; ++ks) {
#pragma unroll
            for (int tl = 0; tl < TPW; ++tl) GRU4_MFMA(au[tl], wu[tl][ks], bfr[ks], !(H >= 256 && tl == TPW - 1 && ks >= KSN - 4));
            constexpr int PER = (TPW * 4 + KSN - 2) / (KSN - 1);
            if (ks >= 1) {
#pragma unroll
                for (int v = (ks - 1) * PER; v < ks * PER && v < TPW * 4; ++v) {
                    const int tl = v >> 2, e = v & 3;
                    if (e == 0 || v == (ks - 1) * PER) asm volatile("" : "+v"(ar[tl]));
                    rhf[tl][e] = fast_sigmoid(ar[tl][e]) * hreg[tl][e];
                    asm volatile("" : "+v"(rhf[tl][e]));
                }
            }
        }
        GRU_T(1);
#pragma unroll
        for (int tl = 0; tl < TPW; ++tl) {
            bf16x4v o;
#pragma unroll
            for (int e = 0; e < 4; ++e) o[e] = (__bf16)rhf[tl][e];
            *reinterpret_cast<bf16x4v*>(rhb + n * PITCH + ucol + tl * 16) = o;
        }
        GRU_T(2);
        GRU4_BARRIER();
        GRU_T(3);
#pragma unroll
        for (int tl = 0; tl < TPW; ++tl) asm volatile("" : "+v"(au[tl]));
#pragma unroll
        for (int ks = 0; ks < KSN; ++ks) bfr[ks] = *reinterpret_cast<const bf16x8v*>(rrow + ks * 32);
        f32x4m ac[TPW];
#pragma unroll
        for (int tl = 0; tl < TPW; ++tl) {
            ac[tl] = xc[tl];
            xc[tl] = *reinterpret_cast<const f32x4m*>(xn + tl * 16 + 2 * H);
        }
#pragma unroll
        for (int ks = 0; ks < KSN; ++ks)
#pragma unroll
            for (int tl = 0; tl < TPW; ++tl) {
                const bf16x8v w = ks < KR ? wc[tl][ks < KR ? ks : 0] : candL[((wave * TPW + tl) * KL + (ks < KR ? 0 : ks - KR)) * 64 + lane];
                ac[tl] = __builtin_amdgcn_mfma_f32_16x16x32_bf16(w, bfr[ks], ac[tl], 0, 0, 0);
            }
        float uu[TPW][4];
#pragma unroll
        for (int tl = 0; tl < TPW; ++tl)
#pragma unroll
            for (int e = 0; e < 4; ++e) uu[tl][e] = fast_sigmoid(au[tl][e]);
        bf16x4v ob[TPW];
        f32x4m hv[TPW];
#pragma unroll
        for (int tl = 0; tl < TPW; ++tl) {
#pragma unroll
            for (int e = 0; e < 4; ++e) {
                const float c = fast_tanh(ac[tl][e]);
                const float hn = uu[tl][e] * hreg[tl][e] + (1.0f - uu[tl][e]) * c;
                hreg[tl][e] = hn;
                hv[tl][e] = hn;
                ob[tl][e] = (__bf16)hn;
            }
            *reinterpret_cast<bf16x4v*>(hb + n * PITCH + ucol + tl * 16) = ob[tl];
        }
        GRU_T(4);
        if (seq_ok) {
            if (a.out_bf16) {
#pragma unroll
                for (int tl = 0; tl < TPW; ++tl)
                    *reinterpret_cast<bf16x4v*>(reinterpret_cast<__bf16*>(a.out) + ((size_t)seq * a.T + t) * 2 * H + (size_t)dir * H + ucol + tl * 16) = ob[tl];
            } else {
#pragma unroll
                for (int tl = 0; tl < TPW; ++tl)
                    *reinterpret_cast<f32x4m*>(reinterpret_cast<float*>(a.out) + ((size_t)seq * a.T + t) * 2 * H + (size_t)dir * H + ucol + tl * 16) = hv[tl];
            }
        }
        GRU_T(5);
        GRU4_BARRIER();
        GRU_T(6);
    }
#undef GRU4_MFMA
#undef GRU4_BARRIER
#ifdef VC_ABLATE
    if (stamp) {
#pragma unroll
        for (int i = 0; i < 8; ++i) g_gru_stamps[i] = acc_t[i];
    }
#endif
}

template <int H>
int launch_mfma4(const GruArgs& a, void* ws, size_t ws_bytes, hipStream_t st) {
    typedef Mf4Geom<H> G;
    const size_t need = 2 * (size_t)3 * H * H * sizeof(__bf16);
    if (ws == nullptr || ws_bytes < need)
        return vc::set_error(VC_ERR_WORKSPACE, "vc_gru_bidir: workspace too small (%zu < %zu)", ws_bytes, need);
    __bf16* packed = static_cast<__bf16*>(ws);
    hipLaunchKernelGGL((gru_mfma4_pack_kernel<H>), dim3(256), dim3(256), 0, st, static_cast<const __bf16*>(a.Wh[0]),
                       static_cast<const __bf16*>(a.Wh[1]), packed);
    static bool attr_done = false;
    if (!attr_done) {
        VC_HIP_CHECK(hipFuncSetAttribute(reinterpret_cast<const void*>(gru_mfma4_kernel<H>),
                                         hipFuncAttributeMaxDynamicSharedMemorySize, (int)G::LDS));
        attr_done = true;
    }
    hipLaunchKernelGGL((gru_mfma4_kernel<H>), dim3((a.n_seq + 15) / 16, 2), dim3(256), G::LDS, st, a,
                       static_cast<const __bf16*>(packed));
    VC_HIP_CHECK(hipGetLastError());
    return VC_OK;
}

template <int H> struct MfsGeom {
    static constexpr int HP = (H + 15) / 16 * 16, KP = (H + 31) / 32 * 32;
    static constexpr int TPW = HP / 16, KSN = KP / 32, NF = 3 * TPW * KSN;
    static constexpr int PITCH = KP + 8;
    static constexpr int WPB = 4;
    static constexpr size_t LDS = (size_t)WPB * 2 * 16 * PITCH * 2;
};

template <int H>
__global__ void __launch_bounds__(256)
gru_mfma_small_pack_kernel(const __bf16* W0, const __bf16* W1, __bf16* packed) {
    typedef MfsGeom<H> G;
    const int total = 2 * G::NF * 64 * 8;
    for (int idx = blockIdx.x * 256 + threadIdx.x; idx < total; idx += gridDim.x * 256) {
        int r = idx;
        const int j = r & 7; r >>= 3;
        const int lane = r & 63; r >>= 6;
        const int f = r % G::NF;
        const int dir = r / G::NF;
        const int g = f / (G::TPW * G::KSN), rem = f % (G::TPW * G::KSN);
        const int tl = rem / G::KSN, ks = rem % G::KSN;
        const int k = ks * 32 + 8 * (lane >> 4) + j;
        const int unit = tl * 16 + (lane & 15);
        const __bf16* W = dir ? W1 : W0;
        packed[idx] = (k < H && unit < H) ? W[(size_t)k * 3 * H + g * H + unit] : (__bf16)0.0f;
    }
}

template <int H>
__global__ void __launch_bounds__(64 * MfsGeom<H>::WPB)
gru_mfma_small_kernel(GruArgs a, const __bf16* packed) {
    typedef MfsGeom<H> G;
    constexpr int TPW = G::TPW, KSN = G::KSN, PITCH = G::PITCH;
    typedef __bf16 bf16x4v __attribute__((ext_vector_type(4)));
    extern __shared__ __attribute__((aligned(16))) char smem[];
    const int lane = threadIdx.x & 63;
    const int wave = __builtin_amdgcn_readfirstlane((int)(threadIdx.x >> 6));
    const int dir = blockIdx.y, seq0 = (blockIdx.x * G::WPB + wave) * 16;
    if (seq0 >= a.n_seq) return;
    __bf16* hb = reinterpret_cast<__bf16*>(smem) + (size_t)wave * 2 * 16 * PITCH;
    __bf16* rhb = hb + 16 * PITCH;
    const int n = lane & 15, q = lane >> 4;
    const int seq = min(seq0 + n, a.n_seq - 1);
    const bool seq_ok = (seq0 + n) < a.n_seq;
    const bf16x8v* pk = reinterpret_cast<const bf16x8v*>(packed) + (size_t)dir * G::NF * 64 + lane;
    bf16x8v w[3][TPW][KSN];
#pragma unroll
    for (int g = 0; g < 3; ++g)
#pragma unroll
        for (int tl = 0; tl < TPW; ++tl)
#pragma unroll
            for (int ks = 0; ks < KSN; ++ks) w[g][tl][ks] = pk[(size_t)((g * TPW + tl) * KSN + ks) * 64];
    for (int i = lane; i < 2 * 16 * PITCH; i += 64) hb[i] = (__bf16)0.0f;
    float hreg[TPW][4];
#pragma unroll
    for (int tl = 0; tl < TPW; ++tl)
#pragma unroll
        for (int e = 0; e < 4; ++e) hreg[tl][e] = 0.0f;

    const int H3 = 3 * H;
    const size_t xrow = 6 * (size_t)H;
    const float* xbase = a.xproj + (size_t)seq * a.T * xrow + (size_t)dir * H3 + q * 4;
    bool uok[TPW];
#pragma unroll
    for (int tl = 0; tl < TPW; ++tl) uok[tl] = tl * 16 + q * 4 < H;
    int t = dir ? a.T - 1 : 0;
    const int dt = dir ? -1 : 1;
    const f32x4m zero4 = {0.0f, 0.0f, 0.0f, 0.0f};
    f32x4m xr[TPW], xu[TPW], xc[TPW];
#pragma unroll
    for (int tl = 0; tl < TPW; ++tl) {
        const float* xp = xbase + (size_t)t * xrow + tl * 16;
        xr[tl] = uok[tl] ? *reinterpret_cast<const f32x4m*>(xp) : zero4;
        xu[tl] = uok[tl] ? *reinterpret_cast<const f32x4m*>(xp + H) : zero4;
        xc[tl] = uok[tl] ? *reinterpret_cast<const f32x4m*>(xp + 2 * H) : zero4;
    }
    const __bf16* hrow = hb + n * PITCH + 8 * q;
    const __bf16* rrow = rhb + n * PITCH + 8 * q;
    for (int step = 0; step < a.T; ++step, t += dt) {
        const float* xn = xbase + (size_t)(step + 1 < a.T ? t + dt : t) * xrow;
        bf16x8v bfr[KSN];
#pragma unroll
        for (int ks = 0; ks < KSN; ++ks) bfr[ks] = *reinterpret_cast<const bf16x8v*>(hrow + ks * 32);
        f32x4m ar[TPW], au[TPW];
#pragma unroll
        for (int tl = 0; tl < TPW; ++tl) {
            ar[tl] = xr[tl];
            au[tl] = xu[tl];
            xr[tl] = uok[tl] ? *reinterpret_cast<const f32x4m*>(xn + tl * 16) : zero4;
            xu[tl] = uok[tl] ? *reinterpret_cast<const f32x4m*>(xn + tl * 16 + H) : zero4;
        }
#pragma unroll
        for (int ks = 0; ks < KSN; ++ks)
#pragma unroll
            for (int tl = 0; tl < TPW; ++tl) {
                ar[tl] = __builtin_amdgcn_mfma_f32_16x16x32_bf16(w[0][tl][ks], bfr[ks], ar[tl], 0, 0, 0);
                au[tl] = __builtin_amdgcn_mfma_f32_16x16x32_bf16(w[1][tl][ks], bfr[ks], au[tl], 0, 0, 0);
            }
#pragma unroll
        for (int tl = 0; tl < TPW; ++tl) {
            bf16x4v o;
#pragma unroll
            for (int e = 0; e < 4; ++e) o[e] = (__bf16)(fast_sigmoid(ar[tl][e]) * hreg[tl][e]);
            if (uok[tl]) *reinterpret_cast<bf16x4v*>(rhb + n * PITCH + tl * 16 + q * 4) = o;
        }
#pragma unroll
        for (int ks = 0; ks < KSN; ++ks) bfr[ks] = *reinterpret_cast<const bf16x8v*>(rrow + ks * 32);
        f32x4m ac[TPW];
#pragma unroll
        for (int tl = 0; tl < TPW; ++tl) {
            ac[tl] = xc[tl];
            xc[tl] = uok[tl] ? *reinterpret_cast<const f32x4m*>(xn + tl * 16 + 2 * H) : zero4;
        }
#pragma unroll
        for (int ks = 0; ks < KSN; ++ks)
#pragma unroll
            for (int tl = 0; tl < TPW; ++tl)
                ac[tl] = __builtin_amdgcn_mfma_f32_16x16x32_bf16(w[2][tl][ks], bfr[ks], ac[tl], 0, 0, 0);
#pragma unroll
        for (int tl = 0; tl < TPW; ++tl) {
            bf16x4v o;
            f32x4m hv;
#pragma unroll
            for (int e = 0; e < 4; ++e) {
                const float u = fast_sigmoid(au[tl][e]);
                const float c = fast_tanh(ac[tl][e]);
                const float hn = u * hreg[tl][e] + (1.0f - u) * c;
                hreg[tl][e] = hn;
                hv[e] = hn;
                o[e] = (__bf16)hn;
            }
            if (uok[tl]) {
                *reinterpret_cast<bf16x4v*>(hb + n * PITCH + tl * 16 + q * 4) = o;
                if (seq_ok) {
                    const size_t oi = ((size_t)seq * a.T + t) * 2 * H + (size_t)dir * H + tl * 16 + q * 4;
                    if (a.out_bf16) *reinterpret_cast<bf16x4v*>(reinterpret_cast<__bf16*>(a.out) + oi) = o;
                    else *reinterpret_cast<f32x4m*>(reinterpret_cast<float*>(a.out) + oi) = hv;
                }
            }
        }
    }
}

template <int H>
int launch_mfma_small(const GruArgs& a, void* ws, size_t ws_bytes, hipStream_t st) {
    typedef MfsGeom<H> G;
    const size_t need = 2 * (size_t)G::NF * 64 * 16;
    if (ws == nullptr || ws_bytes < need)
        return vc::set_error(VC_ERR_WORKSPACE, "vc_gru_bidir: workspace too small (%zu < %zu)", ws_bytes, need);
    __bf16* packed = static_cast<__bf16*>(ws);
    hipLaunchKernelGGL((gru_mfma_small_pack_kernel<H>), dim3(16), dim3(256), 0, st, static_cast<const __bf16*>(a.Wh[0]),
                       static_cast<const __bf16*>(a.Wh[1]), packed);
    const int groups = (a.n_seq + 15) / 16;
    hipLaunchKernelGGL((gru_mfma_small_kernel<H>), dim3((groups + G::WPB - 1) / G::WPB, 2), dim3(64 * G::WPB), G::LDS, st, a,
                       static_cast<const __bf16*>(packed));
    VC_HIP_CHECK(hipGetLastError());
    return VC_OK;
}

constexpr int GRU_WAVE_WPB = 4;
template <int H, typename WT>
__global__ void __launch_bounds__(64 * GRU_WAVE_WPB)
gru_wave_kernel(GruArgs a) {
    static_assert(H <= 64 && H % 4 == 0, "one lane per hidden unit, unrolled by 4");
    constexpr int H3 = 3 * H;
    const int lane = threadIdx.x & 63;
    const int seq = blockIdx.x * GRU_WAVE_WPB + (threadIdx.x >> 6), dir = blockIdx.y;
    if (seq >= a.n_seq) return;
    const bool act = lane < H;
    const int j = act ? lane : 0;
    const WT* W = reinterpret_cast<const WT*>(a.Wh[dir]);
    float wr[H], wu[H], wc[H];
#pragma unroll
    for (int k = 0; k < H; ++k) {
        wr[k] = act ? ld_w(W + (size_t)k * H3 + j) : 0.0f;
        wu[k] = act ? ld_w(W + (size_t)k * H3 + H + j) : 0.0f;
        wc[k] = act ? ld_w(W + (size_t)k * H3 + 2 * H + j) : 0.0f;
    }
    const size_t xrow = 6 * (size_t)H;
    const float* xbase = a.xproj + (size_t)seq * a.T * xrow + (size_t)dir * H3 + j;
    int t = dir ? a.T - 1 : 0;
    const int dt = dir ? -1 : 1;
    float xr = xbase[(size_t)t * xrow], xu = xbase[(size_t)t * xrow + H], xc = xbase[(size_t)t * xrow + 2 * H];
    float h = 0.0f;
    for (int step = 0; step < a.T; ++step, t += dt) {
        float xr_n = 0.0f, xu_n = 0.0f, xc_n = 0.0f;
        if (step + 1 < a.T) {
            const float* xn = xbase + (size_t)(t + dt) * xrow;
            xr_n = xn[0]; xu_n = xn[H]; xc_n = xn[2 * H];
        }
        float ar0 = xr, ar1 = 0.0f, au0 = xu, au1 = 0.0f;
#pragma unroll
        for (int k = 0; k < H; k += 2) {
            const float h0 = __int_as_float(__builtin_amdgcn_readlane(__float_as_int(h), k));
            const float h1 = __int_as_float(__builtin_amdgcn_readlane(__float_as_int(h), k + 1));
            ar0 = fmaf(h0, wr[k], ar0);
            au0 = fmaf(h0, wu[k], au0);
            ar1 = fmaf(h1, wr[k + 1], ar1);
            au1 = fmaf(h1, wu[k + 1], au1);
        }
        constexpr bool FAST = sizeof(WT) == 2;
        const float r = FAST ? fast_sigmoid(ar0 + ar1) : sigmoidf_(ar0 + ar1);
        const float u = FAST ? fast_sigmoid(au0 + au1) : sigmoidf_(au0 + au1);
        const float rh = r * h;
        float ac0 = xc, ac1 = 0.0f, ac2 = 0.0f, ac3 = 0.0f;
#pragma unroll
        for (int k = 0; k < H; k += 4) {
            const float r0 = __int_as_float(__builtin_amdgcn_readlane(__float_as_int(rh), k));
            const float r1 = __int_as_float(__builtin_amdgcn_readlane(__float_as_int(rh), k + 1));
            const float r2 = __int_as_float(__builtin_amdgcn_readlane(__float_as_int(rh), k + 2));
            const float r3 = __int_as_float(__builtin_amdgcn_readlane(__float_as_int(rh), k + 3));
            ac0 = fmaf(r0, wc[k], ac0);
            ac1 = fmaf(r1, wc[k + 1], ac1);
            ac2 = fmaf(r2, wc[k + 2], ac2);
            ac3 = fmaf(r3, wc[k + 3], ac3);
        }
        const float acs = (ac0 + ac1) + (ac2 + ac3);
        const float c = FAST ? fast_tanh(acs) : tanhf(acs);
        h = act ? (u * h + (1.0f - u) * c) : 0.0f;
        if (act) st_out<WT>(a.out, ((size_t)seq * a.T + t) * 2 * H + (size_t)dir * H + j, h, a.out_bf16);
        xr = xr_n; xu = xu_n; xc = xc_n;
    }
}

__global__ void __launch_bounds__(256)
softmax_argmax_kernel(const float* logits, int M, int N, int ldl, void* prob, int ldp, int out_bf16, int32_t* cls,
                      __bf16* prob2, int ldp2) {
    const int lane = threadIdx.x & 63;
    const int row = blockIdx.x * 4 + (threadIdx.x >> 6);
    if (row >= M) return;
    const float* x = logits + (size_t)row * ldl;
    float mx = -3.402823466e38f;
    int mi = 0x7fffffff;
    for (int c = lane; c < N; c += 64) {
        const float v = x[c];
        if (v > mx) { mx = v; mi = c; }
    }
#pragma unroll
    for (int o = 32; o > 0; o >>= 1) {
        const float ov = __shfl_xor(mx, o, 64);
        const int oi = __shfl_xor(mi, o, 64);
        if (ov > mx || (ov == mx && oi < mi)) { mx = ov; mi = oi; }
    }
    float s = 0.0f;
    for (int c = lane; c < N; c += 64) s += expf(x[c] - mx);
    s = vc::wave_sum(s);
    const float inv = 1.0f / s;
    const int wmax = ldp > ldp2 ? ldp : ldp2;
    for (int c = lane; c < wmax; c += 64) {
        const float p = c < N ? expf(x[c] - mx) * inv : 0.0f;
        if (c < ldp) {
            if (out_bf16) reinterpret_cast<__bf16*>(prob)[(size_t)row * ldp + c] = (__bf16)p;
            else reinterpret_cast<float*>(prob)[(size_t)row * ldp + c] = p;
        }
        if (prob2 && c < ldp2) prob2[(size_t)row * ldp2 + c] = (__bf16)p;
    }
    if (cls && lane == 0) cls[row] = mi;
}

__global__ void __launch_bounds__(256)
convert_kernel(const void* src, int sdt, void* dst, int ddt, size_t n) {
    size_t i = (size_t)blockIdx.x * 256 + threadIdx.x;
    const size_t stride = (size_t)gridDim.x * 256;
    for (; i < n; i += stride) {
        const float v = sdt == VC_F32 ? reinterpret_cast<const float*>(src)[i]
                                      : (float)reinterpret_cast<const __bf16*>(src)[i];
        if (ddt == VC_F32) reinterpret_cast<float*>(dst)[i] = v;
        else reinterpret_cast<__bf16*>(dst)[i] = (__bf16)v;
    }
}

}

extern "C" {

size_t vc_gru_workspace_bytes(int32_t H, int32_t w_dtype) {
    if (H <= 0) return 0;
    if (H == 40 && w_dtype == VC_BF16) return 2 * (size_t)MfsGeom<40>::NF * 64 * 16;
    return 2 * (size_t)3 * H * H * (w_dtype == VC_F32 ? 4 : 2);
}

int vc_gru_bidir(const float* d_xproj, const void* d_Wh_fw, const void* d_Wh_bw, int32_t w_dtype, int32_t n_seq,
                 int32_t T, int32_t H, void* d_out, int32_t out_dtype, void* d_workspace, size_t workspace_bytes,
                 void* stream) {
    VC_REQUIRE(d_xproj && d_Wh_fw && d_Wh_bw && d_out, "NULL argument");
    VC_REQUIRE(n_seq > 0 && T > 0 && H > 0 && H <= 1024, "bad shape n_seq=%d T=%d H=%d", n_seq, T, H);
    VC_REQUIRE(w_dtype == VC_F32 || w_dtype == VC_BF16, "bad w_dtype %d", w_dtype);
    VC_REQUIRE(out_dtype == VC_F32 || out_dtype == VC_BF16, "bad out_dtype %d", out_dtype);
    GruArgs a;
    a.xproj = d_xproj; a.Wh[0] = d_Wh_fw; a.Wh[1] = d_Wh_bw; a.out = d_out;
    a.n_seq = n_seq; a.T = T; a.H = H; a.out_bf16 = out_dtype == VC_BF16;
    const size_t wbytes = (size_t)H * 3 * H * (w_dtype == VC_F32 ? 4 : 2);
    const size_t base = 3 * (size_t)H * 4;
    a.w_in_lds = (base + wbytes <= 150 * 1024);
    const size_t lds = base + (a.w_in_lds ? wbytes : 0);
    int nt = 256;
    while (nt < 512 && nt < 2 * H) nt *= 2;
    hipStream_t st = static_cast<hipStream_t>(stream);
    dim3 grid(n_seq, 2);
    const int gm = vc::opt(vc::OPT_GRU_MFMA);
    const bool use_valu = gm >= 0 ? (gm != 1) : (n_seq < 32);
    const bool four = vc::opt(vc::OPT_GRU_MFMA4) == 1;
    if (w_dtype == VC_BF16 && H == 256) return use_valu ? launch_resident<256, __bf16, 512>(a, d_workspace, workspace_bytes, st)
                                               : four ? launch_mfma4<256>(a, d_workspace, workspace_bytes, st)
                                                      : launch_mfma<256>(a, d_workspace, workspace_bytes, st);
    if (w_dtype == VC_BF16 && H == 128) return use_valu ? launch_resident<128, __bf16, 256>(a, d_workspace, workspace_bytes, st)
                                               : four ? launch_mfma4<128>(a, d_workspace, workspace_bytes, st)
                                                      : launch_mfma<128>(a, d_workspace, workspace_bytes, st);
    if (w_dtype == VC_F32 && H == 128) return launch_resident<128, float, 1024>(a, d_workspace, workspace_bytes, st);
    if (H == 40 && w_dtype == VC_BF16) {
        const int sm = vc::opt(vc::OPT_GRU_SMALL_MFMA);
        if (sm == 1) return launch_mfma_small<40>(a, d_workspace, workspace_bytes, st);
    }
    if (H == 40) {
        const dim3 gw((n_seq + GRU_WAVE_WPB - 1) / GRU_WAVE_WPB, 2);
        if (w_dtype == VC_F32) hipLaunchKernelGGL((gru_wave_kernel<40, float>), gw, dim3(64 * GRU_WAVE_WPB), 0, st, a);
        else hipLaunchKernelGGL((gru_wave_kernel<40, __bf16>), gw, dim3(64 * GRU_WAVE_WPB), 0, st, a);
        VC_HIP_CHECK(hipGetLastError());
        return VC_OK;
    }
    if (w_dtype == VC_F32) {
        VC_HIP_CHECK(hipFuncSetAttribute(reinterpret_cast<const void*>(gru_generic_kernel<float>),
                                         hipFuncAttributeMaxDynamicSharedMemorySize, (int)lds));
        hipLaunchKernelGGL(gru_generic_kernel<float>, grid, dim3(nt), lds, st, a);
    } else {
        VC_HIP_CHECK(hipFuncSetAttribute(reinterpret_cast<const void*>(gru_generic_kernel<__bf16>),
                                         hipFuncAttributeMaxDynamicSharedMemorySize, (int)lds));
        hipLaunchKernelGGL(gru_generic_kernel<__bf16>, grid, dim3(nt), lds, st, a);
    }
    VC_HIP_CHECK(hipGetLastError());
    return VC_OK;
}

#ifdef VC_ABLATE
int vc_ablate_read_gru_stamps(unsigned long long* h_out) {
    VC_HIP_CHECK(hipDeviceSynchronize());
    VC_HIP_CHECK(hipMemcpyFromSymbol(h_out, HIP_SYMBOL(g_gru_stamps), sizeof(unsigned long long) * 16));
    return VC_OK;
}
#endif

int vc_lstm_bidir(const float* d_xproj, const void* d_Wh_fw, const void* d_Wh_bw, int32_t w_dtype, int32_t n_seq, int32_t T,
                  int32_t H, void* d_out, int32_t out_dtype, void* stream) {
    VC_REQUIRE(d_xproj && d_Wh_fw && d_Wh_bw && d_out, "NULL argument");
    VC_REQUIRE(n_seq > 0 && T > 0 && H > 0 && H <= 512 && n_seq <= 65535, "vc_lstm_bidir: bad shape n_seq=%d T=%d H=%d (H <= 512)", n_seq, T, H);
    VC_REQUIRE((w_dtype == VC_F32 || w_dtype == VC_BF16) && (out_dtype == VC_F32 || out_dtype == VC_BF16), "bad dtype");
    LstmArgs a;
    a.xproj = d_xproj; a.Wh[0] = d_Wh_fw; a.Wh[1] = d_Wh_bw; a.n_seq = n_seq; a.T = T; a.H = H;
    a.out = d_out; a.out_bf16 = out_dtype == VC_BF16;
    const size_t base = (size_t)5 * H * sizeof(float);
    const size_t wbytes = (size_t)4 * H * H * (w_dtype == VC_F32 ? 4 : 2);
    a.w_in_lds = (base + wbytes <= 150 * 1024);
    const size_t lds = base + (a.w_in_lds ? wbytes : 0);
    hipStream_t st = static_cast<hipStream_t>(stream);
    if (w_dtype == VC_F32) {
        VC_HIP_CHECK(hipFuncSetAttribute(reinterpret_cast<const void*>(lstm_generic_kernel<float>),
                                         hipFuncAttributeMaxDynamicSharedMemorySize, (int)lds));
        hipLaunchKernelGGL(lstm_generic_kernel<float>, dim3(n_seq, 2), dim3(512), lds, st, a);
    } else {
        VC_HIP_CHECK(hipFuncSetAttribute(reinterpret_cast<const void*>(lstm_generic_kernel<__bf16>),
                                         hipFuncAttributeMaxDynamicSharedMemorySize, (int)lds));
        hipLaunchKernelGGL(lstm_generic_kernel<__bf16>, dim3(n_seq, 2), dim3(512), lds, st, a);
    }
    VC_HIP_CHECK(hipGetLastError());
    return VC_OK;
}

int vc_softmax_argmax(const float* d_logits, int32_t M, int32_t N, int32_t ldl, void* d_prob, int32_t ldp,
                      int32_t out_dtype, int32_t* d_class, void* stream) {
    VC_REQUIRE(d_logits && d_prob, "NULL argument");
    VC_REQUIRE(M > 0 && N > 0 && ldl >= N && ldp >= N, "bad shape M=%d N=%d ldl=%d ldp=%d", M, N, ldl, ldp);
    VC_REQUIRE(out_dtype == VC_F32 || out_dtype == VC_BF16, "bad out_dtype %d", out_dtype);
    hipLaunchKernelGGL(softmax_argmax_kernel, dim3((M + 3) / 4), dim3(256), 0, static_cast<hipStream_t>(stream),
                       d_logits, M, N, ldl, d_prob, ldp, out_dtype == VC_BF16, d_class, static_cast<__bf16*>(nullptr), 0);
    VC_HIP_CHECK(hipGetLastError());
    return VC_OK;
}

int vc_softmax_argmax_dual(const float* d_logits, int32_t M, int32_t N, int32_t ldl, float* d_prob, int32_t ldp,
                           void* d_prob_bf16, int32_t ldp_bf16, int32_t* d_class, void* stream) {
    VC_REQUIRE(d_logits && d_prob && d_prob_bf16, "NULL argument");
    VC_REQUIRE(M > 0 && N > 0 && ldl >= N && ldp >= N && ldp_bf16 >= N, "bad shape M=%d N=%d ldl=%d ldp=%d/%d", M, N, ldl, ldp, ldp_bf16);
    hipLaunchKernelGGL(softmax_argmax_kernel, dim3((M + 3) / 4), dim3(256), 0, static_cast<hipStream_t>(stream),
                       d_logits, M, N, ldl, static_cast<void*>(d_prob), ldp, 0, d_class, static_cast<__bf16*>(d_prob_bf16), ldp_bf16);
    VC_HIP_CHECK(hipGetLastError());
    return VC_OK;
}

int vc_convert(const void* d_src, int32_t src_dtype, void* d_dst, int32_t dst_dtype, size_t n, void* stream) {
    VC_REQUIRE(d_src && d_dst, "NULL argument");
    VC_REQUIRE((src_dtype == VC_F32 || src_dtype == VC_BF16) && (dst_dtype == VC_F32 || dst_dtype == VC_BF16), "bad dtype");
    if (n == 0) return VC_OK;
    const int blocks = (int)((n + 255) / 256 < 4096 ? (n + 255) / 256 : 4096);
    hipLaunchKernelGGL(convert_kernel, dim3(blocks), dim3(256), 0, static_cast<hipStream_t>(stream), d_src, src_dtype,
                       d_dst, dst_dtype, n);
    VC_HIP_CHECK(hipGetLastError());
    return VC_OK;
}

}
```

### speech-cloner_amd/modules.py

```python
import contextlib
import ctypes as C
import math
import threading

import numpy as np

import _vc
import mx8

OPTIONS = {'prenet_chain': True,
           'highway_chain': True,
           'cbhg_front': True}


def apply_options(d):
    for k, v in (d or {}).items():
        if k in OPTIONS:
            OPTIONS[k] = bool(v)
        else:
            _vc.set_option(k, int(v))

BN_EPS = 1e-3
BN_DECAY = 0.999
BANK_FILTERS = 128


def _torch():
    import torch
    return torch


class VariableStore:

    def __init__(self, compute_dtype='float32', device='cuda', seed=0):
        torch = _torch()
        self.mx8 = False
        if compute_dtype in ('float32', 'f32', torch.float32):
            self.dtype, self.vc_dtype = torch.float32, _vc.VC_F32
        elif compute_dtype in ('bfloat16', 'bf16', torch.bfloat16):
            self.dtype, self.vc_dtype = torch.bfloat16, _vc.VC_BF16
        elif compute_dtype == 'mxfp8':
            self.dtype, self.vc_dtype, self.mx8 = torch.bfloat16, _vc.VC_BF16, True
        else:
            raise ValueError(' - ERROR, compute_dtype {} not understood'.format(compute_dtype))
        self.device = torch.device(device)
        self.vars = {}
        self.order = []
        self.non_trainable = set()
        self._cache = {}
        self._rng = np.random.RandomState(seed)

    def get(self, name, shape, init):
        v = self.vars.get(name)
        if v is not None:
            if tuple(v.shape) != tuple(shape):
                raise ValueError(' - ERROR, variable {} has shape {}, requested {}'.format(name, tuple(v.shape), shape))
            return v
        torch = _torch()
        if init == 'glorot':
            if len(shape) == 2:
                fan_in, fan_out = shape
            else:
                rf = int(np.prod(shape[:-2]))
                fan_in, fan_out = shape[-2] * rf, shape[-1] * rf
            lim = math.sqrt(6.0 / (fan_in + fan_out))
            a = self._rng.uniform(-lim, lim, size=shape).astype(np.float32)
        elif isinstance(init, (int, float)):
            a = np.full(shape, float(init), dtype=np.float32)
        else:
            raise ValueError(init)
        v = torch.from_numpy(a).to(self.device)
        self.vars[name] = v
        self.order.append(name)
        if name.endswith('/moving_mean') or name.endswith('/moving_variance'):
            self.non_trainable.add(name)
        return v

    def assign(self, name, value):
        torch = _torch()
        t = value if torch.is_tensor(value) else torch.from_numpy(np.ascontiguousarray(value, dtype=np.float32))
        if name not in self.vars:
            raise KeyError(name)
        if tuple(t.shape) != tuple(self.vars[name].shape):
            raise ValueError(' - ERROR, assign {}: shape {} != {}'.format(name, tuple(t.shape), tuple(self.vars[name].shape)))
        self.vars[name].copy_(t.to(self.device, dtype=torch.float32))
        self.invalidate()

    def load_dict(self, d, strict=True):
        missing = [n for n in self.vars if n not in d]
        if strict and missing:
            raise KeyError('variables missing from checkpoint: {}'.format(missing[:4]))
        torch = _torch()
        for n, v in self.vars.items():
            if n in d:
                a = np.asarray(d[n], dtype=np.float32)
                if v.dim() == 0 and a.size == 1:
                    a = a.reshape(())
                a = np.ascontiguousarray(a) if a.ndim else a
                if tuple(a.shape) != tuple(v.shape):
                    raise ValueError(' - ERROR, checkpoint tensor {} has shape {}, model wants {}'.format(n, a.shape, tuple(v.shape)))
                v.copy_(torch.from_numpy(np.array(a)) if a.ndim == 0 else torch.from_numpy(a))
        self.invalidate()

    def to_numpy(self):
        return {n: v.detach().cpu().numpy() for n, v in self.vars.items()}

    def trainable_names(self, prefix=''):
        return [n for n in self.order if n.startswith(prefix) and n not in self.non_trainable]

    def invalidate(self, prefix=None):
        if prefix is None:
            self._cache.clear()
        else:
            pre = prefix.rstrip('/')
            for k in [k for k in self._cache if isinstance(k, tuple) and any(
                    isinstance(e, str) and (e == pre or e.startswith(pre + '/')) for e in k[1:])]:
                del self._cache[k]
        self.version = getattr(self, 'version', 0) + 1

    def cached(self, key, fn):
        v = self._cache.get(key)
        if v is None:
            v = fn()
            self._cache[key] = v
            torch = _torch()
            if torch.cuda.is_available():
                cur = torch.cuda.current_stream()
                if cur != torch.cuda.default_stream():
                    cur.synchronize()
        return v


_CTX = threading.local()


def _ctx():
    if not hasattr(_CTX, 'stack'):
        _CTX.stack = []
        _CTX.store = None
    return _CTX


@contextlib.contextmanager
def variable_store(store):
    c = _ctx()
    prev = c.store
    c.store = store
    try:
        yield store
    finally:
        c.store = prev


@contextlib.contextmanager
def variable_scope(name, reuse=None):
    c = _ctx()
    c.stack.append(name)
    try:
        yield '/'.join(c.stack)
    finally:
        c.stack.pop()


def _scope(*names):
    return '/'.join(list(_ctx().stack) + [n for n in names if n])


def _store():
    s = _ctx().store
    if s is None:
        raise RuntimeError(' - ERROR, no current VariableStore (use `with variable_store(store):`)')
    return s


def _pad8(n):
    return (n + 7) // 8 * 8


def _as3(x):
    if x.dim() != 3:
        raise ValueError(' - ERROR, expected a [N, T, C] tensor, got shape {}'.format(tuple(x.shape)))
    return x


def gemm_desc(X, M, T, Cin, ldx, N, groups, Cout, ldc, vc_dtype, mode=_vc.GEMM_PLAIN,
              pro_scale=None, pro_shift=None, pro_relu=0, pro_pool=0,
              epi_scale=None, epi_shift=None, act=_vc.ACT_NONE, R=None, ldr=0, out_f32=False, epi_pool=0, sum_groups=False):
    d = _vc.GemmDesc()
    d.dtype, d.mode = vc_dtype, mode
    d.d_X = X.data_ptr()
    d.M, d.T, d.Cin, d.ldx, d.N, d.n_groups = M, T, Cin, ldx, N, len(groups)
    for i, (Bt, K, taps, pad_l, c_off) in enumerate(groups):
        g = d.groups[i]
        g.d_Bt, g.K, g.taps, g.pad_l, g.c_off = Bt.data_ptr(), K, taps, pad_l, c_off
    d.d_pro_scale = pro_scale.data_ptr() if pro_scale is not None else None
    d.d_pro_shift = pro_shift.data_ptr() if pro_shift is not None else None
    d.pro_relu, d.pro_pool = int(pro_relu), int(pro_pool)
    d.d_epi_scale = epi_scale.data_ptr() if epi_scale is not None else None
    d.d_epi_shift = epi_shift.data_ptr() if epi_shift is not None else None
    d.act = act
    d.d_R = R.data_ptr() if R is not None else None
    d.ldr = ldr
    d.d_C, d.ldc, d.out_f32 = Cout.data_ptr(), ldc, int(bool(out_f32))
    d.epi_pool = int(epi_pool)
    d.sum_groups = int(sum_groups)
    return d


def gemm_launch(X, M, T, Cin, ldx, N, groups, Cout, ldc, vc_dtype, **kw):
    d = gemm_desc(X, M, T, Cin, ldx, N, groups, Cout, ldc, vc_dtype, **kw)
    if vc_dtype == _vc.VC_BF16 and len(groups) == 1 and N == 256:
        nbytes = _vc.lib().vc_conv_gemm_workspace_bytes(C.byref(d))
        if nbytes:
            ws = _torch().empty(nbytes, dtype=_torch().uint8, device=Cout.device)
            d.d_workspace, d.workspace_bytes = ws.data_ptr(), nbytes
    _vc.check(_vc.lib().vc_conv_gemm(C.byref(d), _vc.current_stream()))
    return Cout


def convert(x, dtype):
    torch = _torch()
    if x.dtype == dtype:
        return x
    y = torch.empty(x.shape, dtype=dtype, device=x.device)
    code = {torch.float32: _vc.VC_F32, torch.bfloat16: _vc.VC_BF16}
    _vc.check(_vc.lib().vc_convert(x.data_ptr(), code[x.dtype], y.data_ptr(), code[dtype], x.numel(),
                                   _vc.current_stream()))
    return y


def axpby(x, a, y, b, out=None):
    torch = _torch()
    if x.dtype != torch.float32 or y.dtype != torch.float32 or x.shape != y.shape:
        raise ValueError(' - ERROR, axpby wants two float32 tensors of one shape')
    x, y = x.contiguous(), y.contiguous()
    if out is None:
        out = torch.empty_like(x)
    Cn = x.shape[-1]
    _vc.check(_vc.lib().vc_axpby(x.data_ptr(), Cn, float(a), y.data_ptr(), Cn, float(b), out.data_ptr(), Cn,
                                 x.numel() // Cn, Cn, _vc.current_stream()))
    return out


def _prep_dense(store, scope, cin, units, bias_init=0.0):
    k = store.get(scope + '/kernel', (cin, units), 'glorot')
    b = store.get(scope + '/bias', (units,), bias_init)

    def build():
        torch = _torch()
        cp = _pad8(cin)
        bt = torch.zeros((units, cp), dtype=torch.float32, device=store.device)
        bt[:, :cin] = k.t()
        return bt.to(store.dtype).contiguous(), b.clone()
    return store.cached(('dense', scope), build)


def _prep_conv(store, scope, size, cin, filters):
    k = store.get(scope + '/conv1d/kernel', (size, cin, filters), 'glorot')

    def build():
        return k.reshape(size * cin, filters).t().contiguous().to(store.dtype)
    return store.cached(('conv', scope), build)


def _bn_vars(store, scope, C_):
    return (store.get(scope + '/beta', (C_,), 0.0), store.get(scope + '/gamma', (C_,), 1.0),
            store.get(scope + '/moving_mean', (C_,), 0.0), store.get(scope + '/moving_variance', (C_,), 1.0))


def _prep_bn(store, scope, C_):
    beta, gamma, mean, var = _bn_vars(store, scope, C_)

    def build():
        torch = _torch()
        s = gamma * torch.rsqrt(var + BN_EPS)
        return s.contiguous(), (beta - mean * s).contiguous()
    return store.cached(('bn', scope), build)


def _prep_highway(store, scope, H):
    k1 = store.get(scope + '/dense1/kernel', (H, H), 'glorot')
    b1 = store.get(scope + '/dense1/bias', (H,), 0.0)
    k2 = store.get(scope + '/dense2/kernel', (H, H), 'glorot')
    b2 = store.get(scope + '/dense2/bias', (H,), -1.0)

    def build():
        torch = _torch()
        nb = (H + 31) // 32
        if H % 32 == 0:
            bt = torch.stack([k1.t().reshape(nb, 32, H), k2.t().reshape(nb, 32, H)], dim=1).reshape(64 * nb, H)
            bias = torch.stack([b1.view(nb, 32), b2.view(nb, 32)], dim=1).reshape(64 * nb)
            return bt.to(store.dtype).contiguous(), bias
        bt = torch.zeros((64 * nb, H), dtype=torch.float32, device=store.device)
        bias = torch.zeros((64 * nb,), dtype=torch.float32, device=store.device)
        for q in range(nb):
            lo, hi = 32 * q, min(H, 32 * q + 32)
            bt[64 * q:64 * q + (hi - lo)] = k1[:, lo:hi].t()
            bt[64 * q + 32:64 * q + 32 + (hi - lo)] = k2[:, lo:hi].t()
            bias[64 * q:64 * q + (hi - lo)] = b1[lo:hi]
            bias[64 * q + 32:64 * q + 32 + (hi - lo)] = b2[lo:hi]
        return bt.to(store.dtype).contiguous(), bias
    return store.cached(('highway', scope), build)


def _prep_gru(store, scope, cin, H):
    w = {}
    for d in ('fw', 'bw'):
        s = '{}/bidirectional_rnn/{}/gru_cell'.format(scope, d)
        w[d] = (store.get(s + '/gates/kernel', (cin + H, 2 * H), 'glorot'),
                store.get(s + '/gates/bias', (2 * H,), 1.0),
                store.get(s + '/candidate/kernel', (cin + H, H), 'glorot'),
                store.get(s + '/candidate/bias', (H,), 0.0))

    def build():
        torch = _torch()
        btx = torch.cat([torch.cat([w[d][0][:cin].t(), w[d][2][:cin].t()], 0) for d in ('fw', 'bw')], 0)
        bx = torch.cat([torch.cat([w[d][1], w[d][3]], 0) for d in ('fw', 'bw')], 0)
        wh = [torch.cat([w[d][0][cin:], w[d][2][cin:]], 1).contiguous().to(store.dtype) for d in ('fw', 'bw')]
        return btx.contiguous().to(store.dtype), bx.contiguous(), wh[0], wh[1]
    return store.cached(('gru', scope), build)


def _prep_gru_uni(store, scope, cin, H):
    s = '{}/rnn/gru_cell'.format(scope)
    wg = store.get(s + '/gates/kernel', (cin + H, 2 * H), 'glorot')
    bg = store.get(s + '/gates/bias', (2 * H,), 1.0)
    wc = store.get(s + '/candidate/kernel', (cin + H, H), 'glorot')
    bc = store.get(s + '/candidate/bias', (H,), 0.0)

    def build():
        torch = _torch()
        one = torch.cat([wg[:cin].t(), wc[:cin].t()], 0)
        b1 = torch.cat([bg, bc], 0)
        wh = torch.cat([wg[cin:], wc[cin:]], 1).contiguous().to(store.dtype)
        return torch.cat([one, one], 0).contiguous().to(store.dtype), torch.cat([b1, b1], 0).contiguous(), wh
    return store.cached(('gru_uni', scope), build)


def dense(inputs, units, activation_fn=None, name='dense', bias_init=0.0, out_f32=False, in_features=None):
    torch = _torch()
    store = _store()
    x = _as3(inputs)
    N_, T_, Cx = x.shape
    scope = _scope(name)
    cin = Cx if in_features is None else in_features
    kname = scope + '/kernel'
    if kname in store.vars:
        cin = store.vars[kname].shape[0]
    bt, b = _prep_dense(store, scope, cin, units, bias_init)
    if Cx != _pad8(cin):
        raise ValueError(' - ERROR, dense {}: input width {} does not match kernel rows {}'.format(scope, Cx, cin))
    out = torch.empty((N_, T_, units), dtype=torch.float32 if out_f32 else store.dtype, device=x.device)
    act = {None: _vc.ACT_NONE, 'relu': _vc.ACT_RELU, 'sigmoid': _vc.ACT_SIGMOID, 'tanh': _vc.ACT_TANH}[activation_fn]
    gemm_launch(x, N_ * T_, T_, Cx, Cx, units, [(bt, Cx, 1, 0, 0)], out, units, store.vc_dtype,
                epi_shift=b, act=act, out_f32=out_f32)
    return out


def bn(inputs, is_training=True, activation_fn=None, scope="bn", reuse=None):
    if is_training:
        raise NotImplementedError(' - ERROR, bn: training-mode batch statistics are fused into the training step')
    torch = _torch()
    store = _store()
    x = _as3(inputs)
    N_, T_, C_ = x.shape
    s, sh = _prep_bn(store, _scope(scope), C_)
    eye = store.cached(('eye', C_), lambda: torch.eye(C_, dtype=store.dtype, device=store.device))
    out = torch.empty_like(x)
    act = {None: _vc.ACT_NONE, 'relu': _vc.ACT_RELU}[activation_fn]
    gemm_launch(x, N_ * T_, T_, C_, C_, C_, [(eye, C_, 1, 0, 0)], out, C_, store.vc_dtype,
                epi_scale=s, epi_shift=sh, act=act)
    return out


def _f32_split_ok(store):
    return store.dtype == _torch().float32 and _vc.get_option('f32_f16x3') != 0


def _mx8_ok(store):
    return getattr(store, 'mx8', False)


def conv1d(inputs, filters=None, size=1, rate=1, padding="SAME", use_bias=False, activation_fn=None,
           scope="conv1d", reuse=None, bn_scope=None, residual=None, pool_input=False):
    if rate != 1 or padding.upper() != "SAME" or use_bias:
        raise NotImplementedError(' - ERROR, conv1d: only rate=1, padding=SAME, use_bias=False are used by the reference')
    torch = _torch()
    store = _store()
    if isinstance(inputs, mx8.MxTensor):
        N_, T_, Cin = inputs.shape
        filters = Cin if filters is None else filters
        if not (_mx8_ok(store) and mx8.conv_supported(Cin, filters, size) and residual is None and not pool_input):
            raise ValueError(' - ERROR, conv1d {}: an MX-FP8 input needs mxfp8 mode, a multiple of 128 filters, no '
                             'residual and no input pooling'.format(_scope(scope)))
        with variable_scope(scope):
            kscope = _scope()
            store.get(kscope + '/conv1d/kernel', (size, Cin, filters), 'glorot')
        if bn_scope is not None:
            s, sh = _prep_bn(store, _scope(bn_scope), filters)
        else:
            s = store.cached(('ones', filters), lambda: torch.ones(filters, dtype=torch.float32, device=store.device))
            sh = store.cached(('zeros', filters), lambda: torch.zeros(filters, dtype=torch.float32, device=store.device))
        packed = store.cached(('mx8conv', kscope, bn_scope), lambda: mx8.pack_kernel(store.vars[kscope + '/conv1d/kernel']))
        act = {None: _vc.ACT_NONE, 'relu': _vc.ACT_RELU}[activation_fn]
        return mx8.conv(inputs, packed, size, filters, s, sh, act)
    x = _as3(inputs)
    N_, T_, Cin = x.shape
    if filters is None:
        filters = Cin
    with variable_scope(scope):
        bt = _prep_conv(store, _scope(), size, Cin, filters)
    s = sh = None
    if bn_scope is not None:
        s, sh = _prep_bn(store, _scope(bn_scope), filters)
    out = torch.empty((N_, T_, filters), dtype=store.dtype, device=x.device)
    act = {None: _vc.ACT_NONE, 'relu': _vc.ACT_RELU}[activation_fn]
    if _f32_split_ok(store) and residual is None and filters in (128, 256) and Cin % 64 == 0 and 1024 <= Cin <= 4096 and size <= 33:
        import gemm16
        kscope = _scope(scope)

        def build():
            w16 = gemm16.Weights16(x.device)
            pairs, cs = gemm16.conv_forward_operands(w16, store.vars[kscope + '/conv1d/kernel'])
            w16.refresh()
            return w16, pairs, (cs * s if s is not None else cs)
        w16, pairs, scale = store.cached(('g16conv', kscope, bn_scope), build)
        M = N_ * T_
        x16, rs = gemm16.split16(x.contiguous().view(M, Cin), M, Cin, Cin, T_, pool=1 if pool_input else 0)
        gemm16.gemm16(x16, rs, M, T_, Cin, pairs, out, filters, col_scale=scale, col_shift=sh, act=act)
        return out
    gemm_launch(x, N_ * T_, T_, Cin, Cin, filters, [(bt, size * Cin, size, (size - 1) // 2, 0)], out, filters,
                store.vc_dtype, pro_pool=int(pool_input), epi_scale=s, epi_shift=sh, act=act,
                R=residual, ldr=filters if residual is not None else 0)
    return out


def conv1d_banks(inputs, K=16, embed_size=256, is_training=True, scope="conv1d_banks", reuse=None, pool_output=None,
                 mx8_out=False):
    if is_training:
        raise NotImplementedError(' - ERROR, conv1d_banks: training mode runs through the fused training step')
    torch = _torch()
    store = _store()
    x = _as3(inputs)
    N_, T_, Cin = x.shape
    F_ = embed_size // 2
    if K > _vc.GEMM_MAX_GROUPS:
        raise ValueError(' - ERROR, conv1d_banks: K={} > {}'.format(K, _vc.GEMM_MAX_GROUPS))
    use_mx8 = mx8_out and pool_output == 'auto' and _mx8_ok(store) and mx8.bank_supported(K, Cin, F_)
    groups = []
    with variable_scope(scope):
        for k in range(1, K + 1):
            sub = 'conv1d' if k == 1 else 'num_{}/conv1d'.format(k)
            with variable_scope(sub):
                if use_mx8:
                    store.get(_scope() + '/conv1d/kernel', (k, Cin, F_), 'glorot')
                else:
                    bt = _prep_conv(store, _scope(), k, Cin, F_)
                    groups.append((bt, k * Cin, k, (k - 1) // 2, F_ * (k - 1)))
        s, sh = _prep_bn(store, _scope('bn'), F_ * K)
    if use_mx8:
        bscope = _scope(scope)
        packed = store.cached(('mx8bank', bscope), lambda: [mx8.pack_kernel(store.vars[
            bscope + ('/conv1d' if k == 1 else '/num_{}/conv1d'.format(k)) + '/conv1d/kernel']) for k in range(1, K + 1)])
        return mx8.bank(x, packed, K, s, sh), True
    out = torch.empty((N_, T_, F_ * K), dtype=store.dtype, device=x.device)
    if _f32_split_ok(store) and K % 2 == 0 and K <= 32 and Cin % 64 == 0 and F_ == BANK_FILTERS == 128:
        import gemm16
        bscope = _scope(scope)

        def build():
            w16 = gemm16.Weights16(x.device)
            kern = [store.vars[bscope + ('/conv1d' if k == 1 else '/num_{}/conv1d'.format(k)) + '/conv1d/kernel'] for k in range(1, K + 1)]
            pairs, cs = gemm16.bank_forward_operands(w16, kern, Cin)
            w16.refresh()
            return w16, pairs, cs * s
        w16, pairs, scale = store.cached(('g16bank', bscope), build)
        M = N_ * T_
        x16, rs = gemm16.split16(x.contiguous().view(M, Cin), M, Cin, Cin, T_)
        gemm16.gemm16(x16, rs, M, T_, Cin, pairs, out, F_ * K, col_scale=scale, col_shift=sh, act=_vc.ACT_RELU)
        return (out, False) if pool_output == 'auto' else out
    d = gemm_desc(x, N_ * T_, T_, Cin, Cin, F_, groups, out, F_ * K, store.vc_dtype,
                  epi_scale=s, epi_shift=sh, act=_vc.ACT_RELU, epi_pool=1 if pool_output == 'auto' else 0)
    pooled = False
    if pool_output == 'auto':
        pooled = bool(_vc.lib().vc_conv_gemm_epi_pool_supported(C.byref(d)))
        d.epi_pool = int(pooled)
    _vc.check(_vc.lib().vc_conv_gemm(C.byref(d), _vc.current_stream()))
    return (out, pooled) if pool_output == 'auto' else out


def _refuse_cudnn(use_Cudnn, what):
    if use_Cudnn:
        raise NotImplementedError(' - ERROR, {}: use_Cudnn=True (cuDNN parameter blob / cell variant) is not built; '
                                  'only the GRUCell / LSTMCell variable layout of use_Cudnn=False is supported'.format(what))


def gru(inputs, num_units=None, bidirection=False, scope="gru", use_Cudnn=False, reuse=None):
    _refuse_cudnn(use_Cudnn, 'gru')
    torch = _torch()
    store = _store()
    x = _as3(inputs)
    N_, T_, Cin = x.shape
    H = Cin if num_units is None else num_units
    if not bidirection:
        btx, bx, wh = _prep_gru_uni(store, _scope(scope), Cin, H)
        xproj = torch.empty((N_ * T_, 6 * H), dtype=torch.float32, device=x.device)
        gemm_launch(x, N_ * T_, T_, Cin, Cin, 6 * H, [(btx, Cin, 1, 0, 0)], xproj, 6 * H, store.vc_dtype,
                    epi_shift=bx, out_f32=True)
        return _gru_recurrence(xproj, N_, T_, H, wh, wh)[:, :, :H].contiguous()
    btx, bx, wh_fw, wh_bw = _prep_gru(store, _scope(scope), Cin, H)
    xproj = torch.empty((N_ * T_, 6 * H), dtype=torch.float32, device=x.device)
    gemm_launch(x, N_ * T_, T_, Cin, Cin, 6 * H, [(btx, Cin, 1, 0, 0)], xproj, 6 * H, store.vc_dtype,
                epi_shift=bx, out_f32=True)
    return _gru_recurrence(xproj, N_, T_, H, wh_fw, wh_bw)


def _gru_recurrence(xproj, N_, T_, H, wh_fw, wh_bw):
    torch = _torch()
    store = _store()
    x = xproj
    out = torch.empty((N_, T_, 2 * H), dtype=store.dtype, device=x.device)
    if store.dtype == torch.float32 and 128 < H <= 1024 and _vc.get_option('gru_f32_wide') != 0:
        gates = torch.empty((2, N_ * T_, 3 * H), dtype=torch.float32, device=x.device)
        rh = torch.empty((2, N_ * T_, H), dtype=torch.float32, device=x.device)
        _vc.check(_vc.lib().vc_gru_train_forward(xproj.data_ptr(), wh_fw.data_ptr(), wh_bw.data_ptr(), N_, T_, H,
                                                 out.data_ptr(), gates.data_ptr(), rh.data_ptr(), _vc.current_stream()))
        return out
    nws = _vc.lib().vc_gru_workspace_bytes(H, store.vc_dtype)
    ws = torch.empty((max(nws, 16),), dtype=torch.uint8, device=x.device)
    _vc.check(_vc.lib().vc_gru_bidir(xproj.data_ptr(), wh_fw.data_ptr(), wh_bw.data_ptr(), store.vc_dtype,
                                     N_, T_, H, out.data_ptr(), store.vc_dtype, ws.data_ptr(), nws,
                                     _vc.current_stream()))
    return out


def _prep_lstm(store, scope, cin, H, bidirection):
    dirs = ('bidirectional_rnn/fw', 'bidirectional_rnn/bw') if bidirection else ('rnn', 'rnn')
    w = []
    for d in dirs:
        s = '{}/{}/lstm_cell'.format(scope, d)
        w.append((store.get(s + '/kernel', (cin + H, 4 * H), 'glorot'), store.get(s + '/bias', (4 * H,), 0.0)))

    def build():
        torch = _torch()
        btx = torch.cat([k[:cin].t() for k, _ in w], 0).contiguous().to(store.dtype)
        bx = torch.cat([b for _, b in w], 0).contiguous()
        wh = [k[cin:].contiguous().to(store.dtype) for k, _ in w]
        return btx, bx, wh[0], wh[1]
    return store.cached(('lstm', scope, bidirection), build)


def lstm(inputs, num_units=None, bidirection=False, scope="lstm", use_Cudnn=False, reuse=None):
    _refuse_cudnn(use_Cudnn, 'lstm')
    torch = _torch()
    store = _store()
    x = _as3(inputs)
    N_, T_, Cin = x.shape
    H = Cin if num_units is None else num_units
    btx, bx, wh_fw, wh_bw = _prep_lstm(store, _scope(scope), Cin, H, bidirection)
    xproj = torch.empty((N_ * T_, 8 * H), dtype=torch.float32, device=x.device)
    gemm_launch(x, N_ * T_, T_, Cin, Cin, 8 * H, [(btx, Cin, 1, 0, 0)], xproj, 8 * H, store.vc_dtype,
                epi_shift=bx, out_f32=True)
    out = torch.empty((N_, T_, 2 * H), dtype=store.dtype, device=x.device)
    _vc.check(_vc.lib().vc_lstm_bidir(xproj.data_ptr(), wh_fw.data_ptr(), wh_bw.data_ptr(), store.vc_dtype, N_, T_, H,
                                      out.data_ptr(), store.vc_dtype, _vc.current_stream()))
    return out if bidirection else out[:, :, :H].contiguous()


def _dropout(x, rate, is_training):
    if is_training:
        raise NotImplementedError(' - ERROR, dropout in training mode runs through the fused training step')
    return x


def prenet(inputs, num_units=None, embed_size=256, dropout_rate=0.5, is_training=True, scope="prenet", reuse=None,
           in_features=None):
    if num_units is None:
        num_units = [embed_size, embed_size // 2]
    torch = _torch()
    store = _store()
    x = _as3(inputs)
    N_, T_, Cx = x.shape
    if (not is_training and store.dtype == torch.bfloat16 and x.dtype in (torch.bfloat16, torch.float32)
            and OPTIONS['prenet_chain']
            and _vc.lib().vc_prenet_chain_supported(Cx, num_units[0], num_units[1])):
        with variable_scope(scope):
            sc1, sc2 = _scope('dense1'), _scope('dense2')
            cin = Cx if in_features is None else in_features
            if sc1 + '/kernel' in store.vars:
                cin = store.vars[sc1 + '/kernel'].shape[0]
            if Cx != _pad8(cin):
                raise ValueError(' - ERROR, prenet {}: input width {} does not match kernel rows {}'.format(sc1, Cx, cin))
            bt1, b1 = _prep_dense(store, sc1, cin, num_units[0])
            bt2, b2 = _prep_dense(store, sc2, num_units[0], num_units[1])
        pk1, pk2 = store.cached(('prenet_pk', sc1), lambda: (_mfma_pack(bt1, num_units[0], Cx, 0),
                                                               _mfma_pack(bt2, num_units[1], num_units[0], 1)))
        x = x.contiguous()
        out = torch.empty((N_, T_, num_units[1]), dtype=store.dtype, device=x.device)
        _vc.check(_vc.lib().vc_prenet_chain(x.data_ptr(), int(x.dtype == torch.float32), N_ * T_, Cx, Cx, num_units[0], num_units[1], pk1.data_ptr(),
                                            b1.data_ptr(), pk2.data_ptr(), b2.data_ptr(), out.data_ptr(), num_units[1],
                                            _vc.current_stream()))
        return out
    with variable_scope(scope):
        outputs = dense(convert(x, store.dtype), num_units[0], 'relu', name="dense1", in_features=in_features)
        outputs = _dropout(outputs, dropout_rate, is_training)
        outputs = dense(outputs, num_units[1], 'relu', name="dense2")
        outputs = _dropout(outputs, dropout_rate, is_training)
    return outputs


def highwaynet(inputs, num_units=None, scope="highwaynet", reuse=None):
    torch = _torch()
    store = _store()
    x = _as3(inputs)
    N_, T_, Cx = x.shape
    if not num_units:
        num_units = Cx
    if num_units != Cx:
        raise ValueError(' - ERROR, highwaynet: num_units must equal the input width')
    bt, bias = _prep_highway(store, _scope(scope), Cx)
    out = torch.empty_like(x)
    gemm_launch(x, N_ * T_, T_, Cx, Cx, bt.shape[0], [(bt, Cx, 1, 0, 0)], out, Cx, store.vc_dtype,
                mode=_vc.GEMM_HIGHWAY, epi_shift=bias)
    return out


def highway_chain(inputs, num_units, n_layers, scope_fmt='highwaynet_{}', gru_scope=None):
    torch = _torch()
    store = _store()
    x = _as3(inputs)
    N_, T_, Cx = x.shape
    fused = (store.dtype == torch.bfloat16 and Cx == num_units and Cx in (128, 256) and N_ * T_ >= 128
             and 1 <= n_layers <= 8 and OPTIONS['highway_chain'])
    if not fused:
        out = x
        for i in range(n_layers):
            out = highwaynet(out, num_units=num_units, scope=scope_fmt.format(i))
        return out if gru_scope is None else gru(out, num_units=num_units, bidirection=True, scope=gru_scope)
    packed, biases = [], []
    for i in range(n_layers):
        sc = _scope(scope_fmt.format(i))
        bt, bias = _prep_highway(store, sc, Cx)

        def build(bt=bt):
            pk = torch.empty(bt.numel(), dtype=store.dtype, device=store.device)
            _vc.check(_vc.lib().vc_highway_pack(bt.data_ptr(), bt.shape[0], Cx, pk.data_ptr(), _vc.current_stream()))
            return pk
        packed.append(store.cached(('highway_pk', sc), build))
        biases.append(bias)
    x = x.contiguous()
    PA = (C.c_void_p * n_layers)(*[p.data_ptr() for p in packed])
    BA = (C.c_void_p * n_layers)(*[b.data_ptr() for b in biases])
    if gru_scope is None:
        out = torch.empty_like(x)
        _vc.check(_vc.lib().vc_highway_chain(x.data_ptr(), N_ * T_, Cx, Cx, n_layers, PA, BA, out.data_ptr(), Cx,
                                             None, None, 0, None, 0, _vc.current_stream()))
        return out
    H = num_units
    gsc = _scope(gru_scope)
    btx, bx, wh_fw, wh_bw = _prep_gru(store, gsc, Cx, H)

    def build_px():
        pk = torch.empty(btx.numel(), dtype=store.dtype, device=store.device)
        _vc.check(_vc.lib().vc_highway_pack(btx.data_ptr(), btx.shape[0], Cx, pk.data_ptr(), _vc.current_stream()))
        return pk
    px = store.cached(('gru_pk', gsc), build_px)
    xproj = torch.empty((N_ * T_, 6 * H), dtype=torch.float32, device=x.device)
    _vc.check(_vc.lib().vc_highway_chain(x.data_ptr(), N_ * T_, Cx, Cx, n_layers, PA, BA, None, 0,
                                         px.data_ptr(), bx.data_ptr(), 6 * H, xproj.data_ptr(), 6 * H,
                                         _vc.current_stream()))
    return _gru_recurrence(xproj, N_, T_, H, wh_fw, wh_bw)


def CBHG(inputs, embed_size=256, num_conv_banks=16, num_highwaynet_blocks=4, dropout_rate=0.5, is_training=True,
         scope="CBHG", use_Cudnn=False, use_lstm=False, reuse=None):
    _refuse_cudnn(use_Cudnn, 'CBHG')
    if use_lstm and is_training:
        raise NotImplementedError(' - ERROR, CBHG(is_training=True): training runs through exec_train_step (training.py), not through this function')
    with variable_scope(scope):
        enc, pooled = conv1d_banks(inputs, K=num_conv_banks, is_training=is_training, pool_output='auto',
                                   mx8_out=(embed_size // 2) % 128 == 0)
        enc = conv1d(enc, filters=embed_size // 2, size=3, scope="conv1d_1", bn_scope="conv1d_1",
                     activation_fn='relu', pool_input=0 if pooled else 2)
        enc = conv1d(enc, filters=embed_size // 2, size=3, scope="conv1d_2", bn_scope="conv1d_2",
                     residual=inputs)
        if use_lstm:
            enc = highway_chain(enc, embed_size // 2, num_highwaynet_blocks)
            return lstm(enc, num_units=embed_size // 2, bidirection=True)
        output = highway_chain(enc, embed_size // 2, num_highwaynet_blocks, gru_scope='gru')
    return output


def _cbhg_front(x, E, num_conv_banks, num_highwaynet_blocks, prenet_scope, scope):
    torch = _torch()
    store = _store()
    N_, T_, Cx = x.shape
    Cw, H = E // 2, E // 2
    with variable_scope(prenet_scope):
        bt1, b1 = _prep_dense(store, _scope('dense1'), Cx, E)
        bt2, b2 = _prep_dense(store, _scope('dense2'), E, Cw)
        psc = _scope()
    with variable_scope(scope):
        csc = _scope()
        banks = []
        with variable_scope('conv1d_banks'):
            for k in range(1, num_conv_banks + 1):
                with variable_scope('conv1d' if k == 1 else 'num_{}/conv1d'.format(k)):
                    banks.append(_prep_conv(store, _scope(), k, Cw, 128))
            bs, bsh = _prep_bn(store, _scope('bn'), 128 * num_conv_banks)
        with variable_scope('conv1d_1'):
            _prep_conv(store, _scope(), 3, 128 * num_conv_banks, Cw)
            k1 = store.vars[_scope() + '/conv1d/kernel']
        p1s, p1b = _prep_bn(store, _scope('conv1d_1'), Cw)
        with variable_scope('conv1d_2'):
            bt_p2 = _prep_conv(store, _scope(), 3, Cw, Cw)
        p2s, p2b = _prep_bn(store, _scope('conv1d_2'), Cw)
        hws = [_prep_highway(store, _scope('highwaynet_{}'.format(i)), Cw) for i in range(num_highwaynet_blocks)]
        btx, bx, wh_fw, wh_bw = _prep_gru(store, _scope('gru'), Cw, H)

    def build():
        K_ = num_conv_banks
        coef = torch.zeros((_vc.lib().vc_cbhg_front_coef_floats(),), dtype=torch.float32, device=store.device)
        for off, v in ((0, b1), (96, b2), (160, bs), (1184, bsh), (2208, p1s), (2272, p1b), (2336, p2s), (2400, p2b),
                       (2464, bx)) + tuple((2720 + 128 * i, hb) for i, (_, hb) in enumerate(hws)):
            coef[off:off + v.numel()] = v
        w1 = k1.reshape(3, K_, 4, 2, 16, Cw).permute(5, 1, 2, 0, 3, 4).reshape(Cw, 3 * 128 * K_).to(store.dtype)
        return dict(
            d1=_mfma_pack(bt1, E, Cx, 0), d2=_mfma_pack(bt2, Cw, E, 1),
            bank=torch.cat([_mfma_pack(b, 128, (k + 1) * Cw, 0) for k, b in enumerate(banks)]),
            p1=_mfma_pack(w1, Cw, 3 * 128 * K_, 0), p2=_mfma_pack(bt_p2, Cw, 3 * Cw, 0),
            hw=[_mfma_pack(bt, bt.shape[0], Cw, 1) for bt, _ in hws], gx=_mfma_pack(btx, 6 * H, Cw, 1),
            coef=coef)
    pk = store.cached(('cbhg_front', psc, csc), build)
    x = x.contiguous()
    xproj = torch.empty((N_ * T_, 6 * H), dtype=torch.float32, device=x.device)
    d = _vc.CbhgFrontDesc()
    d.d_x, d.x_f32, d.ldx, d.n_windows, d.T = x.data_ptr(), int(x.dtype == torch.float32), Cx, N_, T_
    d.n_features, d.prenet_units, d.width, d.n_banks, d.bank_filters = Cx, E, Cw, num_conv_banks, 128
    d.n_highway, d.gru_units = num_highwaynet_blocks, H
    d.d_pk_dense1, d.d_pk_dense2, d.d_pk_bank = pk['d1'].data_ptr(), pk['d2'].data_ptr(), pk['bank'].data_ptr()
    d.d_pk_proj1, d.d_pk_proj2, d.d_pk_gru = pk['p1'].data_ptr(), pk['p2'].data_ptr(), pk['gx'].data_ptr()
    for i in range(num_highwaynet_blocks):
        d.d_pk_highway[i] = pk['hw'][i].data_ptr()
    d.d_coef = pk['coef'].data_ptr()
    d.d_xproj, d.ldp = xproj.data_ptr(), 6 * H
    _vc.check(_vc.lib().vc_cbhg_front(C.byref(d), _vc.current_stream()))
    return xproj, H, wh_fw, wh_bw


def _mfma_pack(W, rows, K, chained):
    torch = _torch()
    W = W.contiguous()
    out = torch.empty(((rows + 31) // 32) * ((K + 15) // 16) * 512, dtype=torch.bfloat16, device=W.device)
    _vc.check(_vc.lib().vc_mfma_pack(W.data_ptr(), rows, K, W.shape[1], int(chained), out.data_ptr(), _vc.current_stream()))
    return out


def prenet_CBHG(inputs, embed_size=256, num_conv_banks=16, num_highwaynet_blocks=4, dropout_rate=0.5, is_training=True,
                prenet_scope="prenet", scope="CBHG", use_Cudnn=False, use_lstm=False, in_features=None):
    _refuse_cudnn(use_Cudnn, 'CBHG')
    torch = _torch()
    store = _store()
    x = _as3(inputs)
    N_, T_, Cx = x.shape
    cin = Cx if in_features is None else in_features
    E = embed_size
    fused = (not is_training and not use_lstm and store.dtype == torch.bfloat16 and cin == Cx
             and OPTIONS['cbhg_front']
             and bool(_vc.lib().vc_cbhg_front_supported(Cx, E, E // 2, num_conv_banks, 128, num_highwaynet_blocks, E // 2, T_)))
    if not fused:
        pre = prenet(convert(x, store.dtype), None, E, dropout_rate, is_training, scope=prenet_scope, in_features=in_features)
        return CBHG(pre, E, num_conv_banks, num_highwaynet_blocks, dropout_rate, is_training, scope=scope,
                    use_Cudnn=use_Cudnn, use_lstm=use_lstm)
    xproj, H, wh_fw, wh_bw = _cbhg_front(x, E, num_conv_banks, num_highwaynet_blocks, prenet_scope, scope)
    return _gru_recurrence(xproj, N_, T_, H, wh_fw, wh_bw)


def softmax_argmax_dual(logits, pad_to):
    torch = _torch()
    x = _as3(logits)
    N_, T_, W = x.shape
    prob = torch.empty((N_, T_, W), dtype=torch.float32, device=x.device)
    prob16 = torch.empty((N_, T_, pad_to), dtype=torch.bfloat16, device=x.device)
    cls = torch.empty((N_, T_), dtype=torch.int32, device=x.device)
    _vc.check(_vc.lib().vc_softmax_argmax_dual(x.data_ptr(), N_ * T_, W, W, prob.data_ptr(), W, prob16.data_ptr(), pad_to,
                                               cls.data_ptr(), _vc.current_stream()))
    return prob, cls, prob16


def create_stage_variables(store, scope, in_features, embed_size, num_conv_banks, num_highwaynet_blocks, n_output,
                           use_lstm=False):
    E, H = embed_size, embed_size // 2
    store.get(scope + '/prenet/dense1/kernel', (in_features, E), 'glorot')
    store.get(scope + '/prenet/dense1/bias', (E,), 0.0)
    store.get(scope + '/prenet/dense2/kernel', (E, H), 'glorot')
    store.get(scope + '/prenet/dense2/bias', (H,), 0.0)
    b = scope + '/CBHG/conv1d_banks'
    for k in range(1, num_conv_banks + 1):
        sub = b + ('/conv1d' if k == 1 else '/num_{}/conv1d'.format(k))
        store.get(sub + '/conv1d/kernel', (k, H, BANK_FILTERS), 'glorot')
    _bn_vars(store, b + '/bn', BANK_FILTERS * num_conv_banks)
    store.get(scope + '/CBHG/conv1d_1/conv1d/kernel', (3, BANK_FILTERS * num_conv_banks, H), 'glorot')
    _bn_vars(store, scope + '/CBHG/conv1d_1', H)
    store.get(scope + '/CBHG/conv1d_2/conv1d/kernel', (3, H, H), 'glorot')
    _bn_vars(store, scope + '/CBHG/conv1d_2', H)
    for i in range(num_highwaynet_blocks):
        hs = scope + '/CBHG/highwaynet_{}'.format(i)
        store.get(hs + '/dense1/kernel', (H, H), 'glorot')
        store.get(hs + '/dense1/bias', (H,), 0.0)
        store.get(hs + '/dense2/kernel', (H, H), 'glorot')
        store.get(hs + '/dense2/bias', (H,), -1.0)
    for d in ('fw', 'bw'):
        if use_lstm:
            ls = scope + '/CBHG/lstm/bidirectional_rnn/{}/lstm_cell'.format(d)
            store.get(ls + '/kernel', (2 * H, 4 * H), 'glorot')
            store.get(ls + '/bias', (4 * H,), 0.0)
            continue
        gs = scope + '/CBHG/gru/bidirectional_rnn/{}/gru_cell'.format(d)
        store.get(gs + '/gates/kernel', (2 * H, 2 * H), 'glorot')
        store.get(gs + '/gates/bias', (2 * H,), 1.0)
        store.get(gs + '/candidate/kernel', (2 * H, H), 'glorot')
        store.get(gs + '/candidate/bias', (H,), 0.0)
    store.get(scope + '/y_logits/kernel', (E, n_output), 'glorot')
    store.get(scope + '/y_logits/bias', (n_output,), 0.0)


def softmax_argmax(logits, n_valid=None, pad_to=None, out_dtype=None):
    torch = _torch()
    x = _as3(logits)
    if x.dtype != torch.float32:
        raise ValueError(' - ERROR, softmax_argmax wants float32 logits')
    N_, T_, W = x.shape
    n = W if n_valid is None else n_valid
    ldp = n if pad_to is None else pad_to
    out_dtype = out_dtype or torch.float32
    prob = torch.empty((N_, T_, ldp), dtype=out_dtype, device=x.device)
    cls = torch.empty((N_, T_), dtype=torch.int32, device=x.device)
    code = {torch.float32: _vc.VC_F32, torch.bfloat16: _vc.VC_BF16}[out_dtype]
    _vc.check(_vc.lib().vc_softmax_argmax(x.data_ptr(), N_ * T_, n, W, prob.data_ptr(), ldp, code,
                                          cls.data_ptr(), _vc.current_stream()))
    return prob, cls
```

Baseline: 14.03 million frames/s.

## Add FFT-based conv bank path and cache pre-packed GRU recurrent weights

Adds an FFT route for the conv1d bank: per-window 512-point real FFTs of the input, a batched per-bin complex product against the precomputed kernel spectra (run through the conv256 GEMM), then an inverse FFT with fused BN affine, ReLU and optional pooling. That route is gated by per-width minimum-window thresholds that are all None, so it stays off unless the bank_fft option is set explicitly. Separately, the GRU MFMA recurrence now takes recurrent weights pre-packed once into a cached buffer per scope. This is meant to remove the per-call weight repacking inside the kernel, at the cost of extra device memory for the packed copies.

```diff
diff --git a/include/vc_hip.h b/include/vc_hip.h
--- a/include/vc_hip.h
+++ b/include/vc_hip.h
@@ -129,6 +129,11 @@
 int vc_gru_bidir(const float* d_xproj, const void* d_Wh_fw, const void* d_Wh_bw, int32_t w_dtype,
                  int32_t n_seq, int32_t T, int32_t H, void* d_out, int32_t out_dtype,
                  void* d_workspace, size_t workspace_bytes, void* stream);
+int vc_gru_pack(const void* d_Wh_fw, const void* d_Wh_bw, int32_t w_dtype, int32_t H, void* d_packed,
+                size_t packed_bytes, void* stream);
+int vc_gru_bidir_packed(const float* d_xproj, const void* d_Wh_fw, const void* d_Wh_bw, int32_t w_dtype,
+                        int32_t n_seq, int32_t T, int32_t H, void* d_out, int32_t out_dtype,
+                        void* d_workspace, size_t workspace_bytes, const void* d_packed, void* stream);
 
 
 typedef struct vc_wgrad_group {
@@ -373,6 +378,12 @@
 int vc_scale_rows_f32(const float* d_wav, const int32_t* d_lens, int32_t batch, int32_t max_len, int32_t ld, const float* d_gain,
                       float* d_out, void* stream);
 
+int vc_bankfft_forward(const void* d_x, int32_t n_win, int32_t T, int32_t Cin, void* d_A, void* stream);
+int vc_bankfft_product(const void* d_A, const void* d_W, int32_t bins, int32_t rows, int32_t K, int32_t N, void* d_Y,
+                       void* stream);
+int vc_bankfft_inverse(const void* d_Y, int32_t n_win, int32_t T, int32_t N, int32_t ldy, const float* d_scale,
+                       const float* d_shift, int32_t pool, void* d_out, int32_t ldo, void* stream);
+
 #ifdef __cplusplus
 }
 #endif
diff --git a/speech-cloner_amd/_vc.py b/speech-cloner_amd/_vc.py
--- a/speech-cloner_amd/_vc.py
+++ b/speech-cloner_amd/_vc.py
@@ -148,6 +148,9 @@
     'vc_gru_workspace_bytes': (C.c_size_t, [C.c_int32, C.c_int32]),
     'vc_gru_bidir': (C.c_int, [_P, _P, _P, C.c_int32, C.c_int32, C.c_int32, C.c_int32, _P, C.c_int32, _P,
                                C.c_size_t, _P]),
+    'vc_gru_pack': (C.c_int, [_P, _P, C.c_int32, C.c_int32, _P, C.c_size_t, _P]),
+    'vc_gru_bidir_packed': (C.c_int, [_P, _P, _P, C.c_int32, C.c_int32, C.c_int32, C.c_int32, _P, C.c_int32, _P,
+                                      C.c_size_t, _P, _P]),
     'vc_lstm_bidir': (C.c_int, [_P, _P, _P, C.c_int32, C.c_int32, C.c_int32, C.c_int32, _P, C.c_int32, _P]),
     'vc_convert': (C.c_int, [_P, C.c_int32, _P, C.c_int32, C.c_size_t, _P]),
     'vc_conv_wgrad': (C.c_int, [C.POINTER(WgradDesc), _P]),
@@ -226,6 +229,9 @@
     'vc_path_map': (C.c_int, [_P, _P, C.c_int32, C.c_int32, _P, C.c_int32, _P, C.c_int32, _P, _P]),
     'vc_speech_gain_f32': (C.c_int, [_P, _P, C.c_int32, C.c_int32, C.c_int32, C.c_int32, _P, _P, C.c_int32, C.c_float, _P, _P]),
     'vc_scale_rows_f32': (C.c_int, [_P, _P, C.c_int32, C.c_int32, C.c_int32, _P, _P, _P]),
+    'vc_bankfft_forward': (C.c_int, [_P, C.c_int32, C.c_int32, C.c_int32, _P, _P]),
+    'vc_bankfft_product': (C.c_int, [_P, _P, C.c_int32, C.c_int32, C.c_int32, C.c_int32, _P, _P]),
+    'vc_bankfft_inverse': (C.c_int, [_P, C.c_int32, C.c_int32, C.c_int32, C.c_int32, _P, _P, C.c_int32, _P, C.c_int32, _P]),
     'vc_f0_yin_f32': (C.c_int, [_P, _P, C.c_int32, C.c_int32, C.c_int32, C.c_float, C.c_int32, C.c_int32, C.c_int32, C.c_int32,
                                 C.c_float, _P, _P, C.c_int32, _P]),
     'vc_f0_metrics_f32': (C.c_int, [_P, _P, _P, _P, C.c_int32, C.c_int32, C.c_int32, _P, _P, C.c_int32, _P, _P, _P]),
diff --git a/speech-cloner_amd/csrc/vc_api.hip b/speech-cloner_amd/csrc/vc_api.hip
--- a/speech-cloner_amd/csrc/vc_api.hip
+++ b/speech-cloner_amd/csrc/vc_api.hip
@@ -22,7 +22,7 @@
 static const struct { const char* name; Option id; bool ablate; } k_opts[] = {
     {"bank256", OPT_BANK256, false}, {"bank256_xcd", OPT_BANK256_XCD, false}, {"conv256", OPT_CONV256, false},
     {"conv256_min_k", OPT_CONV256_MINK, false}, {"conv256_wm", OPT_CONV256_WM, false}, {"proj256", OPT_PROJ256, false}, {"proj256_split", OPT_PROJ256_SPLIT, false},
-    {"wgrad_xcd", OPT_WGRAD_XCD, false}, {"gru_mfma", OPT_GRU_MFMA, false}, {"gru_mfma4", OPT_GRU_MFMA4, false}, {"gru_small_mfma", OPT_GRU_SMALL_MFMA, false}, {"fe_fused", OPT_FE_FUSED, false}, {"fe_fused_spin", OPT_FE_FUSED_SPIN, false}, {"gru_train_resident", OPT_GRU_TRAIN_RESIDENT, false}, {"prenet_lds", OPT_PRENET_LDS, false}, {"cbhg_front_mi", OPT_CBHG_FRONT_MI, false}, {"gemm16_split", OPT_GEMM16_SPLIT, false}, {"f32_f16x3", OPT_F32_F16X3, false}, {"gru_f32_wide", OPT_GRU_F32_WIDE, false},
+    {"wgrad_xcd", OPT_WGRAD_XCD, false}, {"gru_mfma", OPT_GRU_MFMA, false}, {"gru_mfma4", OPT_GRU_MFMA4, false}, {"gru_small_mfma", OPT_GRU_SMALL_MFMA, false}, {"fe_fused", OPT_FE_FUSED, false}, {"fe_fused_spin", OPT_FE_FUSED_SPIN, false}, {"gru_train_resident", OPT_GRU_TRAIN_RESIDENT, false}, {"prenet_lds", OPT_PRENET_LDS, false}, {"cbhg_front_mi", OPT_CBHG_FRONT_MI, false}, {"gemm16_split", OPT_GEMM16_SPLIT, false}, {"f32_f16x3", OPT_F32_F16X3, false}, {"gru_f32_wide", OPT_GRU_F32_WIDE, false}, {"bank_fft", OPT_BANK_FFT, false},
     {"ablate_bank256", OPT_ABLATE_BANK256, true}, {"ablate_bank256_only", OPT_ABLATE_BANK256_ONLY, true},
     {"ablate_cbhg_front", OPT_ABLATE_CBHG_FRONT, true},
 };
diff --git a/speech-cloner_amd/csrc/vc_bankfft.h b/speech-cloner_amd/csrc/vc_bankfft.h
--- /dev/null
+++ b/speech-cloner_amd/csrc/vc_bankfft.h
@@ -0,0 +1,14 @@
+#pragma once
+
+namespace bankfft {
+
+constexpr int NFFT = 512;
+constexpr int BINS = NFFT / 2 + 1;
+constexpr int SLAB = 64;
+constexpr int PAIRS = SLAB / 2;
+constexpr int NTHR = 512;
+constexpr int NG = NTHR / PAIRS;
+constexpr float Y_SCALE = 1.0f / 32.0f;
+constexpr int LDS_BYTES = NFFT * PAIRS * 8 + NFFT * 8;
+
+}
diff --git a/speech-cloner_amd/csrc/vc_bankfft.hip b/speech-cloner_amd/csrc/vc_bankfft.hip
--- /dev/null
+++ b/speech-cloner_amd/csrc/vc_bankfft.hip
@@ -0,0 +1,236 @@
+#include "vc_common.h"
+#include "vc_bankfft.h"
+#include "vc_conv256.h"
+
+namespace {
+
+using namespace bankfft;
+
+typedef __bf16 bf16x2 __attribute__((ext_vector_type(2)));
+typedef _Float16 f16x2 __attribute__((ext_vector_type(2)));
+
+__device__ __forceinline__ float2 cadd(float2 a, float2 b) { return make_float2(a.x + b.x, a.y + b.y); }
+__device__ __forceinline__ float2 csub(float2 a, float2 b) { return make_float2(a.x - b.x, a.y - b.y); }
+__device__ __forceinline__ float2 cmul(float2 a, float2 b) { return make_float2(a.x * b.x - a.y * b.y, a.x * b.y + a.y * b.x); }
+template <bool INV> __device__ __forceinline__ float2 rot4(float2 a) { return INV ? make_float2(-a.y, a.x) : make_float2(a.y, -a.x); }
+template <bool INV> __device__ __forceinline__ float2 rot8(float2 a) {
+    const float h = 0.70710678118654752f;
+    return INV ? make_float2((a.x - a.y) * h, (a.x + a.y) * h) : make_float2((a.x + a.y) * h, (a.y - a.x) * h);
+}
+template <bool INV> __device__ __forceinline__ float2 rot8_3(float2 a) {
+    const float h = 0.70710678118654752f;
+    return INV ? make_float2((-a.x - a.y) * h, (a.x - a.y) * h) : make_float2((a.y - a.x) * h, (-a.x - a.y) * h);
+}
+
+template <bool INV> __device__ __forceinline__ void dft8(float2 (&a)[8]) {
+    const float2 b0 = cadd(a[0], a[4]), b4 = csub(a[0], a[4]);
+    const float2 b1 = cadd(a[1], a[5]), b5 = rot8<INV>(csub(a[1], a[5]));
+    const float2 b2 = cadd(a[2], a[6]), b6 = rot4<INV>(csub(a[2], a[6]));
+    const float2 b3 = cadd(a[3], a[7]), b7 = rot8_3<INV>(csub(a[3], a[7]));
+    const float2 c0 = cadd(b0, b2), c2 = csub(b0, b2), c1 = cadd(b1, b3), c3 = rot4<INV>(csub(b1, b3));
+    const float2 c4 = cadd(b4, b6), c6 = csub(b4, b6), c5 = cadd(b5, b7), c7 = rot4<INV>(csub(b5, b7));
+    a[0] = cadd(c0, c1); a[4] = csub(c0, c1); a[2] = cadd(c2, c3); a[6] = csub(c2, c3);
+    a[1] = cadd(c4, c5); a[5] = csub(c4, c5); a[3] = cadd(c6, c7); a[7] = csub(c6, c7);
+}
+
+__device__ __forceinline__ int drev(int b) { return ((b & 7) << 6) | (b & 0x38) | (b >> 6); }
+
+__device__ __forceinline__ void fill_twiddles(float2* tw) {
+    for (int m = threadIdx.x; m < NFFT; m += NTHR) {
+        float sn, cs;
+        sincospif((float)m * (2.0f / NFFT), &sn, &cs);
+        tw[m] = make_float2(cs, -sn);
+    }
+}
+
+template <bool INV> __device__ __forceinline__ float2 twiddle(const float2* tw, int m) {
+    const float2 w = tw[m];
+    return INV ? make_float2(w.x, -w.y) : w;
+}
+
+template <bool INV, int STRIDE, typename Load>
+__device__ __forceinline__ void pass8(float2* s, const float2* tw, int p, int g, Load load) {
+    for (int j = g; j < 64; j += NG) {
+        const int base = STRIDE == 64 ? j : STRIDE == 8 ? (j >> 3) * 64 + (j & 7) : 8 * j;
+        const int n = STRIDE == 64 ? j : (j & 7) * 8;
+        float2 a[8];
+#pragma unroll
+        for (int k = 0; k < 8; ++k) a[k] = load(base + STRIDE * k);
+        dft8<INV>(a);
+#pragma unroll
+        for (int q = 0; q < 8; ++q) {
+            float2 v = a[q];
+            if (STRIDE != 1 && q != 0) v = cmul(v, twiddle<INV>(tw, n * q));
+            s[(base + STRIDE * q) * PAIRS + p] = v;
+        }
+    }
+}
+
+template <bool INV, typename Load>
+__device__ __forceinline__ void fft512(float2* s, const float2* tw, int p, int g, Load first) {
+    auto from_lds = [&](int pos) { return s[pos * PAIRS + p]; };
+    pass8<INV, 64>(s, tw, p, g, first);
+    __syncthreads();
+    pass8<INV, 8>(s, tw, p, g, from_lds);
+    __syncthreads();
+    pass8<INV, 1>(s, tw, p, g, from_lds);
+    __syncthreads();
+}
+
+__global__ void __launch_bounds__(NTHR, 1)
+bankfft_forward_kernel(const __bf16* __restrict__ x, int T, int Cin, __bf16* __restrict__ A, int rows) {
+    extern __shared__ __attribute__((aligned(16))) char smem[];
+    float2* const s = reinterpret_cast<float2*>(smem);
+    float2* const tw = s + NFFT * PAIRS;
+    const int p = threadIdx.x & (PAIRS - 1), g = threadIdx.x / PAIRS;
+    const int w = blockIdx.y, c = blockIdx.x * SLAB + 2 * p;
+    fill_twiddles(tw);
+    __syncthreads();
+    const __bf16* xw = x + (size_t)w * T * Cin + c;
+    auto from_global = [&](int t) {
+        if (t >= T) return make_float2(0.0f, 0.0f);
+        const bf16x2 v = *reinterpret_cast<const bf16x2*>(xw + (size_t)t * Cin);
+        return make_float2((float)v[0], (float)v[1]);
+    };
+    fft512<false>(s, tw, p, g, from_global);
+    const int K2 = 2 * Cin;
+    for (int b = g; b < BINS; b += NG) {
+        const float2 zb = s[drev(b) * PAIRS + p], zm = s[drev((NFFT - b) & (NFFT - 1)) * PAIRS + p];
+        const float er = 0.5f * (zb.x + zm.x), ei = 0.5f * (zb.y - zm.y);
+        const float orr = 0.5f * (zb.y + zm.y), oi = -0.5f * (zb.x - zm.x);
+        bf16x2 re, im, nim;
+        re[0] = (__bf16)er; re[1] = (__bf16)orr;
+        im[0] = (__bf16)ei; im[1] = (__bf16)oi;
+        nim[0] = (__bf16)(-ei); nim[1] = (__bf16)(-oi);
+        __bf16* r0 = A + ((size_t)b * rows + 2 * w) * K2 + c;
+        *reinterpret_cast<bf16x2*>(r0) = re;
+        *reinterpret_cast<bf16x2*>(r0 + Cin) = nim;
+        *reinterpret_cast<bf16x2*>(r0 + K2) = im;
+        *reinterpret_cast<bf16x2*>(r0 + K2 + Cin) = re;
+    }
+}
+
+template <bool POOL>
+__global__ void __launch_bounds__(NTHR, 1)
+bankfft_inverse_kernel(const _Float16* __restrict__ Y, int T, int ldy, int rows, const float* __restrict__ scale,
+                       const float* __restrict__ shift, __bf16* __restrict__ out, int ldo) {
+    extern __shared__ __attribute__((aligned(16))) char smem[];
+    float2* const s = reinterpret_cast<float2*>(smem);
+    float2* const tw = s + NFFT * PAIRS;
+    const int p = threadIdx.x & (PAIRS - 1), g = threadIdx.x / PAIRS;
+    const int w = blockIdx.y, c = blockIdx.x * SLAB + 2 * p;
+    fill_twiddles(tw);
+    constexpr int NB = (BINS + NG - 1) / NG;
+    f16x2 re[NB], im[NB];
+#pragma unroll
+    for (int i = 0; i < NB; ++i) {
+        const int b = g + NG * i;
+        re[i] = im[i] = f16x2{};
+        if (b < BINS) {
+            const _Float16* r0 = Y + ((size_t)b * rows + 2 * w) * ldy + c;
+            re[i] = *reinterpret_cast<const f16x2*>(r0);
+            im[i] = *reinterpret_cast<const f16x2*>(r0 + ldy);
+        }
+    }
+#pragma unroll
+    for (int i = 0; i < NB; ++i) {
+        const int b = g + NG * i;
+        if (b >= BINS) break;
+        const float er = (float)re[i][0], orr = (float)re[i][1];
+        const bool edge = b == 0 || b == NFFT / 2;
+        const float ei = edge ? 0.0f : (float)im[i][0], oi = edge ? 0.0f : (float)im[i][1];
+        s[b * PAIRS + p] = make_float2(er - oi, ei + orr);
+        if (!edge) s[(NFFT - b) * PAIRS + p] = make_float2(er + oi, orr - ei);
+    }
+    __syncthreads();
+    fft512<true>(s, tw, p, g, [&](int pos) { return s[pos * PAIRS + p]; });
+    const float2 sc = *reinterpret_cast<const float2*>(scale + c), sh = *reinterpret_cast<const float2*>(shift + c);
+    const float inv_n = 1.0f / (NFFT * Y_SCALE);
+    auto frame = [&](int t) {
+        const float2 v = s[drev(t) * PAIRS + p];
+        return make_float2(fmaxf(v.x * inv_n * sc.x + sh.x, 0.0f), fmaxf(v.y * inv_n * sc.y + sh.y, 0.0f));
+    };
+    __bf16* ow = out + (size_t)w * T * ldo + c;
+    for (int t = g; t < T; t += NG) {
+        float2 v = frame(t);
+        if (POOL) {
+            const float2 n = frame(min(t + 1, T - 1));
+            v = make_float2(fmaxf(v.x, n.x), fmaxf(v.y, n.y));
+        }
+        bf16x2 o;
+        o[0] = (__bf16)v.x; o[1] = (__bf16)v.y;
+        *reinterpret_cast<bf16x2*>(ow + (size_t)t * ldo) = o;
+    }
+}
+
+template <typename Kern> int raise_lds(Kern k) {
+    VC_HIP_CHECK(hipFuncSetAttribute(reinterpret_cast<const void*>(k), hipFuncAttributeMaxDynamicSharedMemorySize, LDS_BYTES));
+    return VC_OK;
+}
+
+bool aligned4(const void* p) { return (reinterpret_cast<uintptr_t>(p) & 3) == 0; }
+
+}
+
+extern "C" {
+
+int vc_bankfft_forward(const void* d_x, int32_t n_win, int32_t T, int32_t Cin, void* d_A, void* stream) {
+    VC_REQUIRE(d_x && d_A, "vc_bankfft_forward: NULL argument");
+    VC_REQUIRE(n_win > 0 && n_win <= 32767 && T > 0 && T <= NFFT && Cin > 0 && Cin % SLAB == 0,
+               "vc_bankfft_forward: bad shape n_win=%d T=%d Cin=%d", n_win, T, Cin);
+    VC_REQUIRE(aligned4(d_x) && aligned4(d_A), "vc_bankfft_forward: unaligned pointer");
+    static bool attr_done = false;
+    if (!attr_done) {
+        const int rc = raise_lds(bankfft_forward_kernel);
+        if (rc != VC_OK) return rc;
+        attr_done = true;
+    }
+    hipLaunchKernelGGL(bankfft_forward_kernel, dim3(Cin / SLAB, n_win), dim3(NTHR), LDS_BYTES, static_cast<hipStream_t>(stream),
+                       static_cast<const __bf16*>(d_x), T, Cin, static_cast<__bf16*>(d_A), 2 * n_win);
+    VC_HIP_CHECK(hipGetLastError());
+    return VC_OK;
+}
+
+int vc_bankfft_product(const void* d_A, const void* d_W, int32_t bins, int32_t rows, int32_t K, int32_t N, void* d_Y,
+                       void* stream) {
+    VC_REQUIRE(d_A && d_W && d_Y, "vc_bankfft_product: NULL argument");
+    VC_REQUIRE(bins > 0 && bins <= 65535 && rows > 0 && K >= 128 && K % 64 == 0 && N > 0 && N % 128 == 0,
+               "vc_bankfft_product: bad shape bins=%d rows=%d K=%d N=%d", bins, rows, K, N);
+    VC_REQUIRE((reinterpret_cast<uintptr_t>(d_A) & 15) == 0 && (reinterpret_cast<uintptr_t>(d_W) & 15) == 0 &&
+               (reinterpret_cast<uintptr_t>(d_Y) & 15) == 0, "vc_bankfft_product: pointers must be 16-byte aligned");
+    Conv256Args c;
+    c.X = d_A; c.M = rows; c.T = rows; c.Cin = K; c.ldx = K; c.N = N;
+    c.Bt = d_W; c.K = K; c.taps = 1; c.pad_l = 0; c.c_off = 0;
+    c.pool = 0;
+    c.epi_scale = nullptr; c.epi_shift = nullptr; c.act = VC_ACT_NONE;
+    c.R = nullptr; c.ldr = 0; c.C = d_Y; c.ldc = N;
+    c.out_f16 = 1; c.out_scale = Y_SCALE;
+    c.batch = bins; c.bs_x = (int64_t)rows * K; c.bs_b = (int64_t)N * K; c.bs_c = (int64_t)rows * N;
+    return vc_launch_conv256(c, static_cast<hipStream_t>(stream));
+}
+
+int vc_bankfft_inverse(const void* d_Y, int32_t n_win, int32_t T, int32_t N, int32_t ldy, const float* d_scale,
+                       const float* d_shift, int32_t pool, void* d_out, int32_t ldo, void* stream) {
+    VC_REQUIRE(d_Y && d_scale && d_shift && d_out, "vc_bankfft_inverse: NULL argument");
+    VC_REQUIRE(n_win > 0 && n_win <= 32767 && T > 0 && T <= NFFT && N > 0 && N % SLAB == 0 && ldy >= N && ldo >= N &&
+               ldy % 2 == 0 && ldo % 2 == 0, "vc_bankfft_inverse: bad shape n_win=%d T=%d N=%d ldy=%d ldo=%d", n_win, T, N, ldy, ldo);
+    VC_REQUIRE(aligned4(d_Y) && aligned4(d_out) && (reinterpret_cast<uintptr_t>(d_scale) & 7) == 0 &&
+               (reinterpret_cast<uintptr_t>(d_shift) & 7) == 0, "vc_bankfft_inverse: unaligned pointer");
+    static bool attr_done = false;
+    if (!attr_done) {
+        int rc = raise_lds(bankfft_inverse_kernel<false>);
+        if (rc == VC_OK) rc = raise_lds(bankfft_inverse_kernel<true>);
+        if (rc != VC_OK) return rc;
+        attr_done = true;
+    }
+    const dim3 grid(N / SLAB, n_win);
+    hipStream_t st = static_cast<hipStream_t>(stream);
+    const _Float16* Y = static_cast<const _Float16*>(d_Y);
+    __bf16* out = static_cast<__bf16*>(d_out);
+    if (pool) hipLaunchKernelGGL(bankfft_inverse_kernel<true>, grid, dim3(NTHR), LDS_BYTES, st, Y, T, ldy, 2 * n_win, d_scale, d_shift, out, ldo);
+    else hipLaunchKernelGGL(bankfft_inverse_kernel<false>, grid, dim3(NTHR), LDS_BYTES, st, Y, T, ldy, 2 * n_win, d_scale, d_shift, out, ldo);
+    VC_HIP_CHECK(hipGetLastError());
+    return VC_OK;
+}
+
+}
diff --git a/speech-cloner_amd/csrc/vc_common.h b/speech-cloner_amd/csrc/vc_common.h
--- a/speech-cloner_amd/csrc/vc_common.h
+++ b/speech-cloner_amd/csrc/vc_common.h
@@ -44,6 +44,7 @@
     OPT_GRU_F32_WIDE,
     OPT_F32_F16X3,
     OPT_GEMM16_SPLIT,
+    OPT_BANK_FFT,
     OPT_ABLATE_BANK256,
     OPT_ABLATE_BANK256_ONLY,
     OPT_ABLATE_CBHG_FRONT,
diff --git a/speech-cloner_amd/csrc/vc_conv256.h b/speech-cloner_amd/csrc/vc_conv256.h
--- a/speech-cloner_amd/csrc/vc_conv256.h
+++ b/speech-cloner_amd/csrc/vc_conv256.h
@@ -15,6 +15,10 @@
     int32_t ldr;
     void* C;
     int32_t ldc;
+    int32_t batch = 1;
+    int64_t bs_x = 0, bs_b = 0, bs_c = 0;
+    int32_t out_f16 = 0;
+    float out_scale = 1.0f;
 };
 
 int vc_launch_conv256(const Conv256Args& a, hipStream_t st);
diff --git a/speech-cloner_amd/csrc/vc_conv256.hip b/speech-cloner_amd/csrc/vc_conv256.hip
--- a/speech-cloner_amd/csrc/vc_conv256.hip
+++ b/speech-cloner_amd/csrc/vc_conv256.hip
@@ -56,8 +56,8 @@
     const int wr = wid / WN, wc = wid % WN;
     const int m0 = blockIdx.x * BM, n0 = blockIdx.y * BN;
     const int ntap = a.taps, nslab = a.Cin >> 6, ntiles = nslab * ntap, pad_l = a.pad_l;
-    const __bf16* X = reinterpret_cast<const __bf16*>(a.X);
-    const __bf16* Bt = reinterpret_cast<const __bf16*>(a.Bt);
+    const __bf16* X = reinterpret_cast<const __bf16*>(a.X) + (size_t)blockIdx.z * a.bs_x;
+    const __bf16* Bt = reinterpret_cast<const __bf16*>(a.Bt) + (size_t)blockIdx.z * a.bs_b;
 
     const int srow = lane >> 3, pslot = lane & 7;
     const __bf16* a_src[AQ];
@@ -260,7 +260,8 @@
                     for (int e = 0; e < 4; ++e) {
                         float val = act_fn(acc[i][c][4 * q + e] * svv[e] + bvv[e], a.act);
                         if (a.R) val += (float)rr[e];
-                        o[e] = (__bf16)val;
+                        if (a.out_f16) o[e] = __builtin_bit_cast(__bf16, (_Float16)fminf(fmaxf(val * a.out_scale, -65504.0f), 65504.0f));
+                        else o[e] = (__bf16)val;
                     }
                     *reinterpret_cast<bf16x4*>(smem + row * EP + col * 2) = o;
                 }
@@ -270,7 +271,7 @@
     __syncthreads();
     {
         constexpr int CPR = BN / 8;
-        __bf16* C = reinterpret_cast<__bf16*>(a.C);
+        __bf16* C = reinterpret_cast<__bf16*>(a.C) + (size_t)blockIdx.z * a.bs_c;
         for (int idx = tid; idx < BM * CPR; idx += NTHR) {
             const int row = idx / CPR, ch = idx - row * CPR;
             const int gm = m0 + row, gn = n0 + ch * 8;
@@ -292,7 +293,7 @@
                                          hipFuncAttributeMaxDynamicSharedMemorySize, LDS));
         attr_done = true;
     }
-    hipLaunchKernelGGL((conv256_kernel<WN, POOL, NBUF, WM>), dim3((a.M + BM - 1) / BM, a.N / (64 * WN)), dim3(64 * WM * WN), LDS, st, a);
+    hipLaunchKernelGGL((conv256_kernel<WN, POOL, NBUF, WM>), dim3((a.M + BM - 1) / BM, a.N / (64 * WN), a.batch), dim3(64 * WM * WN), LDS, st, a);
     VC_HIP_CHECK(hipGetLastError());
     return VC_OK;
 }
diff --git a/speech-cloner_amd/csrc/vc_rnn.hip b/speech-cloner_amd/csrc/vc_rnn.hip
--- a/speech-cloner_amd/csrc/vc_rnn.hip
+++ b/speech-cloner_amd/csrc/vc_rnn.hip
@@ -500,14 +500,17 @@
 }
 
 template <int H>
-int launch_mfma(const GruArgs& a, void* ws, size_t ws_bytes, hipStream_t st) {
+int launch_mfma(const GruArgs& a, void* ws, size_t ws_bytes, hipStream_t st, const void* prepacked) {
     typedef MfGeom<H> G;
     const size_t need = 2 * (size_t)3 * H * H * sizeof(__bf16);
-    if (ws == nullptr || ws_bytes < need)
-        return vc::set_error(VC_ERR_WORKSPACE, "vc_gru_bidir: workspace too small (%zu < %zu)", ws_bytes, need);
-    __bf16* packed = static_cast<__bf16*>(ws);
-    hipLaunchKernelGGL((gru_mfma_pack_kernel<H>), dim3(256), dim3(256), 0, st, static_cast<const __bf16*>(a.Wh[0]),
-                       static_cast<const __bf16*>(a.Wh[1]), packed);
+    const __bf16* packed = static_cast<const __bf16*>(prepacked);
+    if (!packed) {
+        if (ws == nullptr || ws_bytes < need)
+            return vc::set_error(VC_ERR_WORKSPACE, "vc_gru_bidir: workspace too small (%zu < %zu)", ws_bytes, need);
+        hipLaunchKernelGGL((gru_mfma_pack_kernel<H>), dim3(256), dim3(256), 0, st, static_cast<const __bf16*>(a.Wh[0]),
+                           static_cast<const __bf16*>(a.Wh[1]), static_cast<__bf16*>(ws));
+        packed = static_cast<const __bf16*>(ws);
+    }
     const size_t lds = 2 * 16 * (size_t)G::PITCH * 2 + (G::CAND_LDS ? (size_t)G::NW * G::NF_C * 64 * 16 : 0);
     static bool attr_done = false;
     if (!attr_done) {
@@ -515,8 +518,7 @@
                                          hipFuncAttributeMaxDynamicSharedMemorySize, (int)lds));
         attr_done = true;
     }
-    hipLaunchKernelGGL((gru_mfma_kernel<H>), dim3((a.n_seq + 15) / 16, 2), dim3(512), lds, st, a,
-                       static_cast<const __bf16*>(packed));
+    hipLaunchKernelGGL((gru_mfma_kernel<H>), dim3((a.n_seq + 15) / 16, 2), dim3(512), lds, st, a, packed);
     VC_HIP_CHECK(hipGetLastError());
     return VC_OK;
 }
@@ -1027,9 +1029,29 @@
     return 2 * (size_t)3 * H * H * (w_dtype == VC_F32 ? 4 : 2);
 }
 
+int vc_gru_pack(const void* d_Wh_fw, const void* d_Wh_bw, int32_t w_dtype, int32_t H, void* d_packed, size_t packed_bytes,
+                void* stream) {
+    VC_REQUIRE(d_Wh_fw && d_Wh_bw && d_packed, "vc_gru_pack: NULL argument");
+    VC_REQUIRE(w_dtype == VC_BF16 && (H == 128 || H == 256), "vc_gru_pack: bf16 weights of 128 or 256 units only (H=%d)", H);
+    VC_REQUIRE(packed_bytes >= 2 * (size_t)3 * H * H * 2, "vc_gru_pack: buffer too small (%zu)", packed_bytes);
+    hipStream_t st = static_cast<hipStream_t>(stream);
+    const __bf16 *w0 = static_cast<const __bf16*>(d_Wh_fw), *w1 = static_cast<const __bf16*>(d_Wh_bw);
+    if (H == 256) hipLaunchKernelGGL((gru_mfma_pack_kernel<256>), dim3(256), dim3(256), 0, st, w0, w1, static_cast<__bf16*>(d_packed));
+    else hipLaunchKernelGGL((gru_mfma_pack_kernel<128>), dim3(256), dim3(256), 0, st, w0, w1, static_cast<__bf16*>(d_packed));
+    VC_HIP_CHECK(hipGetLastError());
+    return VC_OK;
+}
+
 int vc_gru_bidir(const float* d_xproj, const void* d_Wh_fw, const void* d_Wh_bw, int32_t w_dtype, int32_t n_seq,
                  int32_t T, int32_t H, void* d_out, int32_t out_dtype, void* d_workspace, size_t workspace_bytes,
                  void* stream) {
+    return vc_gru_bidir_packed(d_xproj, d_Wh_fw, d_Wh_bw, w_dtype, n_seq, T, H, d_out, out_dtype, d_workspace, workspace_bytes,
+                               nullptr, stream);
+}
+
+int vc_gru_bidir_packed(const float* d_xproj, const void* d_Wh_fw, const void* d_Wh_bw, int32_t w_dtype, int32_t n_seq,
+                        int32_t T, int32_t H, void* d_out, int32_t out_dtype, void* d_workspace, size_t workspace_bytes,
+                        const void* d_packed, void* stream) {
     VC_REQUIRE(d_xproj && d_Wh_fw && d_Wh_bw && d_out, "NULL argument");
     VC_REQUIRE(n_seq > 0 && T > 0 && H > 0 && H <= 1024, "bad shape n_seq=%d T=%d H=%d", n_seq, T, H);
     VC_REQUIRE(w_dtype == VC_F32 || w_dtype == VC_BF16, "bad w_dtype %d", w_dtype);
@@ -1050,10 +1072,10 @@
     const bool four = vc::opt(vc::OPT_GRU_MFMA4) == 1;
     if (w_dtype == VC_BF16 && H == 256) return use_valu ? launch_resident<256, __bf16, 512>(a, d_workspace, workspace_bytes, st)
                                                : four ? launch_mfma4<256>(a, d_workspace, workspace_bytes, st)
-                                                      : launch_mfma<256>(a, d_workspace, workspace_bytes, st);
+                                                      : launch_mfma<256>(a, d_workspace, workspace_bytes, st, d_packed);
     if (w_dtype == VC_BF16 && H == 128) return use_valu ? launch_resident<128, __bf16, 256>(a, d_workspace, workspace_bytes, st)
                                                : four ? launch_mfma4<128>(a, d_workspace, workspace_bytes, st)
-                                                      : launch_mfma<128>(a, d_workspace, workspace_bytes, st);
+                                                      : launch_mfma<128>(a, d_workspace, workspace_bytes, st, d_packed);
     if (w_dtype == VC_F32 && H == 128) return launch_resident<128, float, 1024>(a, d_workspace, workspace_bytes, st);
     if (H == 40 && w_dtype == VC_BF16) {
         const int sm = vc::opt(vc::OPT_GRU_SMALL_MFMA);
diff --git a/speech-cloner_amd/modules.py b/speech-cloner_amd/modules.py
--- a/speech-cloner_amd/modules.py
+++ b/speech-cloner_amd/modules.py
@@ -435,6 +435,67 @@
     return out
 
 
+BANK_FFT_LEN = 512
+BANK_FFT_MIN_WINDOWS = {256: None, 128: None}
+BANK_FFT_MIN_K = 32
+
+
+def bank_fft_spectrum(kernels, n_fft=BANK_FFT_LEN):
+    torch = _torch()
+    dev = kernels[0].device
+    Cin = kernels[0].shape[1]
+    bins = n_fft // 2 + 1
+    out = torch.empty((bins, sum(int(w.shape[2]) for w in kernels), 2 * Cin), dtype=torch.bfloat16, device=dev)
+    b = torch.arange(bins, dtype=torch.int64, device=dev)
+    o0 = 0
+    for w in kernels:
+        k, cin, F_ = w.shape
+        if cin != Cin:
+            raise ValueError(' - ERROR, bank_fft_spectrum: kernels of different input widths')
+        j = torch.arange(k, dtype=torch.int64, device=dev) - (k - 1) // 2
+        ang = torch.remainder(b[:, None] * j[None, :], n_fft).double() * (2.0 * math.pi / n_fft)
+        w64 = w.double()
+        re = torch.einsum('bj,jcf->bfc', torch.cos(ang), w64)
+        im = torch.einsum('bj,jcf->bfc', torch.sin(ang), w64)
+        im[0] = 0.0
+        im[n_fft // 2] = 0.0
+        out[:, o0:o0 + F_, :Cin] = re.to(torch.bfloat16)
+        out[:, o0:o0 + F_, Cin:] = im.to(torch.bfloat16)
+        o0 += F_
+    return out
+
+
+def _bank_fft_ok(store, N_, T_, K, Cin, F_):
+    if store.dtype != _torch().bfloat16 or _mx8_ok(store):
+        return False
+    if not (T_ + K - 1 <= BANK_FFT_LEN and Cin % 64 == 0 and F_ == BANK_FILTERS == 128):
+        return False
+    o = _vc.get_option('bank_fft')
+    if o >= 0:
+        return o != 0
+    n_min = BANK_FFT_MIN_WINDOWS.get(Cin)
+    return n_min is not None and N_ >= n_min and K >= BANK_FFT_MIN_K
+
+
+def _bank_fft(store, x, K, F_, bscope, s, sh, pool):
+    torch = _torch()
+    N_, T_, Cin = x.shape
+    wspec = store.cached(('fftbank', bscope), lambda: bank_fft_spectrum([store.vars[
+        bscope + ('/conv1d' if k == 1 else '/num_{}/conv1d'.format(k)) + '/conv1d/kernel'] for k in range(1, K + 1)]))
+    bins = BANK_FFT_LEN // 2 + 1
+    x = x.contiguous()
+    A = torch.empty((bins, 2 * N_, 2 * Cin), dtype=torch.bfloat16, device=x.device)
+    Y = torch.empty((bins, 2 * N_, F_ * K), dtype=torch.float16, device=x.device)
+    out = torch.empty((N_, T_, F_ * K), dtype=torch.bfloat16, device=x.device)
+    st = _vc.current_stream()
+    h = _vc.lib()
+    _vc.check(h.vc_bankfft_forward(x.data_ptr(), N_, T_, Cin, A.data_ptr(), st))
+    _vc.check(h.vc_bankfft_product(A.data_ptr(), wspec.data_ptr(), bins, 2 * N_, 2 * Cin, F_ * K, Y.data_ptr(), st))
+    _vc.check(h.vc_bankfft_inverse(Y.data_ptr(), N_, T_, F_ * K, F_ * K, s.data_ptr(), sh.data_ptr(), int(pool),
+                                   out.data_ptr(), F_ * K, st))
+    return out
+
+
 def conv1d_banks(inputs, K=16, embed_size=256, is_training=True, scope="conv1d_banks", reuse=None, pool_output=None,
                  mx8_out=False):
     if is_training:
@@ -447,12 +508,13 @@
     if K > _vc.GEMM_MAX_GROUPS:
         raise ValueError(' - ERROR, conv1d_banks: K={} > {}'.format(K, _vc.GEMM_MAX_GROUPS))
     use_mx8 = mx8_out and pool_output == 'auto' and _mx8_ok(store) and mx8.bank_supported(K, Cin, F_)
+    use_fft = not use_mx8 and _bank_fft_ok(store, N_, T_, K, Cin, F_)
     groups = []
     with variable_scope(scope):
         for k in range(1, K + 1):
             sub = 'conv1d' if k == 1 else 'num_{}/conv1d'.format(k)
             with variable_scope(sub):
-                if use_mx8:
+                if use_mx8 or use_fft:
                     store.get(_scope() + '/conv1d/kernel', (k, Cin, F_), 'glorot')
                 else:
                     bt = _prep_conv(store, _scope(), k, Cin, F_)
@@ -463,6 +525,9 @@
         packed = store.cached(('mx8bank', bscope), lambda: [mx8.pack_kernel(store.vars[
             bscope + ('/conv1d' if k == 1 else '/num_{}/conv1d'.format(k)) + '/conv1d/kernel']) for k in range(1, K + 1)])
         return mx8.bank(x, packed, K, s, sh), True
+    if use_fft:
+        out = _bank_fft(store, x, K, F_, _scope(scope), s, sh, pool_output == 'auto')
+        return (out, True) if pool_output == 'auto' else out
     out = torch.empty((N_, T_, F_ * K), dtype=store.dtype, device=x.device)
     if _f32_split_ok(store) and K % 2 == 0 and K <= 32 and Cin % 64 == 0 and F_ == BANK_FILTERS == 128:
         import gemm16
@@ -512,10 +577,10 @@
     xproj = torch.empty((N_ * T_, 6 * H), dtype=torch.float32, device=x.device)
     gemm_launch(x, N_ * T_, T_, Cin, Cin, 6 * H, [(btx, Cin, 1, 0, 0)], xproj, 6 * H, store.vc_dtype,
                 epi_shift=bx, out_f32=True)
-    return _gru_recurrence(xproj, N_, T_, H, wh_fw, wh_bw)
-
-
-def _gru_recurrence(xproj, N_, T_, H, wh_fw, wh_bw):
+    return _gru_recurrence(xproj, N_, T_, H, wh_fw, wh_bw, pack_scope=_scope(scope))
+
+
+def _gru_recurrence(xproj, N_, T_, H, wh_fw, wh_bw, pack_scope=None):
     torch = _torch()
     store = _store()
     x = xproj
@@ -528,9 +593,17 @@
         return out
     nws = _vc.lib().vc_gru_workspace_bytes(H, store.vc_dtype)
     ws = torch.empty((max(nws, 16),), dtype=torch.uint8, device=x.device)
-    _vc.check(_vc.lib().vc_gru_bidir(xproj.data_ptr(), wh_fw.data_ptr(), wh_bw.data_ptr(), store.vc_dtype,
-                                     N_, T_, H, out.data_ptr(), store.vc_dtype, ws.data_ptr(), nws,
-                                     _vc.current_stream()))
+    packed = None
+    if pack_scope is not None and store.dtype == torch.bfloat16 and H in (128, 256):
+        def build():
+            pk = torch.empty((nws,), dtype=torch.uint8, device=x.device)
+            _vc.check(_vc.lib().vc_gru_pack(wh_fw.data_ptr(), wh_bw.data_ptr(), store.vc_dtype, H, pk.data_ptr(), nws,
+                                            _vc.current_stream()))
+            return pk
+        packed = store.cached(('gru_mfma_pk', pack_scope), build)
+    _vc.check(_vc.lib().vc_gru_bidir_packed(xproj.data_ptr(), wh_fw.data_ptr(), wh_bw.data_ptr(), store.vc_dtype,
+                                            N_, T_, H, out.data_ptr(), store.vc_dtype, ws.data_ptr(), nws,
+                                            packed.data_ptr() if packed is not None else None, _vc.current_stream()))
     return out
 
 
@@ -669,7 +742,7 @@
     _vc.check(_vc.lib().vc_highway_chain(x.data_ptr(), N_ * T_, Cx, Cx, n_layers, PA, BA, None, 0,
                                          px.data_ptr(), bx.data_ptr(), 6 * H, xproj.data_ptr(), 6 * H,
                                          _vc.current_stream()))
-    return _gru_recurrence(xproj, N_, T_, H, wh_fw, wh_bw)
+    return _gru_recurrence(xproj, N_, T_, H, wh_fw, wh_bw, pack_scope=gsc)
 
 
 def CBHG(inputs, embed_size=256, num_conv_banks=16, num_highwaynet_blocks=4, dropout_rate=0.5, is_training=True,
```

Result: no change. 13.96 million frames/s (-0.4%).
